# dsteinberg/libcluster

Hardware: AMD Instinct MI355X
Metric: E-step data-points/sec (full VBEM iteration: suff-stats + M-step + E-step) (higher is better)
Workload: dtype f64

## Files before the change

include/libcluster_hip.h:

```cpp
#ifndef LIBCLUSTER_HIP_H
#define LIBCLUSTER_HIP_H

#include <stdint.h>

#ifdef __cplusplus
extern "C" {
#endif

typedef enum { LC_OK = 0, LC_EINVAL = 1, LC_ERUNTIME = 2, LC_EHIP = 3, LC_EDOMAIN = 4 } lc_status;

typedef enum { LC_W_DIRICHLET = 0, LC_W_STICKBREAK = 1, LC_W_GDIRICHLET = 2 } lc_weight_kind;
typedef enum {
  LC_ALGO_VDP = 0,
  LC_ALGO_BGMM = 1,
  LC_ALGO_GMC = 2,
  LC_ALGO_SGMC = 3,
  LC_ALGO_DGMM = 4,
  LC_ALGO_BEMM = 5,
  LC_ALGO_DGMC = 6,
  LC_ALGO_EGMC = 7
} lc_algo;
typedef enum { LC_C_GAUSSWISH = 0, LC_C_NORMGAMMA = 1, LC_C_EXPGAMMA = 2 } lc_ckind;

typedef struct lc_ctx lc_ctx;
// ... 11 lines not shown
double lc_const_zerocutoff(void);
int lc_const_splititer(void);

int lc_ctx_create(int device, void* stream, lc_ctx** out);
int lc_ctx_destroy(lc_ctx* ctx);
int lc_ctx_set_stream(lc_ctx* ctx, void* stream);
int lc_ctx_synchronize(lc_ctx* ctx);
int lc_ctx_dims(lc_ctx* ctx, int* J, int* D, int64_t* Ntotal, int* K);

int lc_ctx_set_data(lc_ctx* ctx, int J, const double* const* Xj, const int64_t* Nj, int D, int64_t row_stride,
                    int64_t col_stride);
int lc_ctx_synth(lc_ctx* ctx, int64_t N, int D, int K, const double* mu, const double* L, uint64_t seed,
                 int64_t row_offset, double hard);
int lc_ctx_synth_groups(lc_ctx* ctx, int J, const int64_t* Nj, int D, int K, const double* mu, const double* L,
                        const double* cdf, uint64_t seed, const int64_t* group_ids, double hard);
int lc_ctx_get_rows(lc_ctx* ctx, int j, int64_t row0, int64_t n, double* out);

int lc_ctx_set_qz(lc_ctx* ctx, int j, const double* q, int K, int64_t row_stride, int64_t col_stride);
int lc_ctx_get_qz(lc_ctx* ctx, int j, double* q, int64_t row_stride, int64_t col_stride);
int lc_ctx_get_qz_rows(lc_ctx* ctx, int j, int64_t row0, int64_t n, double* q, int64_t row_stride, int64_t col_stride);
int lc_ctx_get_qz_all(lc_ctx* ctx, double* q);
int lc_ctx_get_qz_all_colmajor(lc_ctx* ctx, double* const* q);
int lc_ctx_fill_qz(lc_ctx* ctx, int K, double value);

int lc_estep_posterior(lc_ctx* ctx, int K, const double* nu, const double* beta, const double* m, const double* iW,
                       const double* logdW, const double* Elogpi, const unsigned char* active, double* Fz,
                       double* LLk);
int lc_estep(lc_ctx* ctx, int K, const double* A, const double* m, const double* c, double* Fz, double* LLk);
int lc_eloglike(lc_ctx* ctx, int K, const double* nu, const double* beta, const double* m, const double* iW,
                const double* logdW);
int lc_mahaldist(lc_ctx* ctx, const double* mu, const double* A, double* dist);
int lc_suffstat(lc_ctx* ctx, const unsigned char* smask, double* Nk, double* xs, double* xxs, double* Njk);
int lc_suffstat_diag(lc_ctx* ctx, const unsigned char* smask, double* Nk, double* xs, double* xxs, double* Njk);
int lc_estep_diag(lc_ctx* ctx, int K, const double* a, const double* w2, const double* w1, const double* c, int raw,
                  double* Fz, double* LLk);
int lc_colsums(lc_ctx* ctx, double* Njk);

typedef int (*lc_allreduce_fn)(void* user, void* device_buf, int64_t count, void* stream);
int lc_ctx_set_allreduce(lc_ctx* ctx, lc_allreduce_fn fn, void* user);
#define LC_COMM_ID_BYTES 128
int lc_comm_rccl_available(void);
int lc_comm_unique_id(void* id );
int lc_ctx_comm_init_rccl(lc_ctx* ctx, const void* id, int rank, int world);
int lc_ctx_comm_init_host(lc_ctx* ctx, const char* name, int rank, int world);
int lc_ctx_comm_free(lc_ctx* ctx);
int lc_ctx_comm_info(lc_ctx* ctx, int* rank, int* world, const char** kind);
int lc_ctx_allreduce(lc_ctx* ctx, double* values, int n);
int lc_ctx_set_sharding(lc_ctx* ctx, int whole_groups);
int lc_ctx_set_skip_zero(lc_ctx* ctx, int on);

int lc_ctx_set_speck_skip(lc_ctx* ctx, int on);
int lc_ctx_speck_passes(lc_ctx* ctx, int64_t* skipping, int64_t* dense);
int lc_ctx_speck_list_passes(lc_ctx* ctx, int64_t* lists);

int lc_trim_cache(void);

int lc_ctx_timing_enable(lc_ctx* ctx, int on);
int lc_ctx_timing_reset(lc_ctx* ctx);
int lc_ctx_timing_get(lc_ctx* ctx, double* estep_ms, int64_t* estep_calls, double* suffstat_ms,
                      int64_t* suffstat_calls);
int lc_ctx_timing_get_fused(lc_ctx* ctx, double* fused_ms, int64_t* fused_calls);
#define LC_TIMING_FIELDS 14
int lc_ctx_timing_get_all(lc_ctx* ctx, double* out, int n);

int lc_vbem(lc_ctx* ctx, lc_model** model, int wkind, int ckind, double wprior, double clusterprior, int maxit,
            int sparse, int fixed_iters, int verbose, unsigned nthreads, double* F, int* niter, double* Ftrace,
            int ntrace);

int lc_prune(lc_ctx* ctx, lc_model* model, int verbose, int* removed);

int lc_learn(int algo, int J, const double* const* Xj, const int64_t* Nj, int D, int64_t row_stride,
             int64_t col_stride, double wprior, double clusterprior, int maxclusters, int sparse, int verbose,
             unsigned nthreads, int device, lc_model** out, double* F);

int lc_learn_w(int algo, int J, const double* const* Xj, const int64_t* Nj, int D, int64_t row_stride,
               int64_t col_stride, double wprior, const double* wprior_j, double clusterprior, int maxclusters,
               int sparse, int verbose, unsigned nthreads, int device, lc_model** out, double* F);

int lc_cluster(lc_ctx* ctx, int wkind, int ckind, double wprior, double clusterprior, int maxclusters, int sparse,
               int verbose, unsigned nthreads, lc_model** out, double* F);

int lc_model_free(lc_model* m);
int lc_model_dims(lc_model* m, int* J, int* K, int* D);
int lc_model_rounds(lc_model* m, int* nrounds);
int lc_model_round(lc_model* m, int r, int* K, int* niter, double* F, int nF);
int lc_model_get_qz(lc_model* m, int j, double* q, int64_t row_stride, int64_t col_stride);
int lc_model_get_qz_all(lc_model* m, double* q);
int lc_model_get_qz_all_colmajor(lc_model* m, double* const* q);
int lc_model_weights(lc_model* m, int j, double* Elogweight, double* Nk);
int lc_model_kinds(lc_model* m, int* wkind, int* ckind);
int lc_model_cluster(lc_model* m, int k, double* N, double* mean, double* cov, double* nu, double* beta, double* iW,
                     double* logdW);
int lc_model_fenergy(lc_model* m, double* Fw , double* Fc );

int lc_model_predict(lc_model* m, lc_ctx* ctx, const int* groups , int keep_qz);
int lc_ctx_get_predictions(lc_ctx* ctx, int j, int64_t row0, int64_t n, int32_t* label, double* logZ, double* logp);
int lc_model_predict_conditional(lc_model* m, lc_ctx* ctx, const int* groups , const int* given,
                                 int ngiven, const int* target , int ntarget);
int lc_ctx_get_conditional(lc_ctx* ctx, int j, int64_t row0, int64_t n, double* mean, int64_t row_stride, double* logp);
int lc_model_predict_conditional_var(lc_model* m, lc_ctx* ctx, const int* groups , const int* given,
                                     int ngiven, const int* target , int ntarget);
int lc_ctx_get_conditional_var(lc_ctx* ctx, int j, int64_t row0, int64_t n, double* var, int64_t row_stride);
#define LC_DRAWS_MAX 64
int lc_model_predict_conditional_draws(lc_model* m, lc_ctx* ctx, const int* groups , const int* given,
                                       int ngiven, const int* target , int ntarget, int ndraws, uint64_t seed);
int lc_ctx_get_conditional_draws(lc_ctx* ctx, int j, int64_t row0, int64_t n, double* draws, int32_t* label);
// ... 68 lines not shown
```

libcluster_amd/capi.py:

```python
from __future__ import annotations

import ctypes as C
import re
from pathlib import Path
from typing import NamedTuple, Optional

import numpy as np

PKG = Path(__file__).resolve().parent
LIB_PATH = PKG / "lib" / "libcluster_hip.so"
if __import__("os").environ.get("LC_LIB_PATH"):
    LIB_PATH = Path(__import__("os").environ["LC_LIB_PATH"])
HEADER = PKG.parent / "include" / "libcluster_hip.h"

LC_OK, LC_EINVAL, LC_ERUNTIME, LC_EHIP, LC_EDOMAIN = range(5)
W_DIRICHLET, W_STICKBREAK, W_GDIRICHLET = 0, 1, 2
ALGO_VDP, ALGO_BGMM, ALGO_GMC, ALGO_SGMC, ALGO_DGMM, ALGO_BEMM, ALGO_DGMC, ALGO_EGMC = range(8)
C_GAUSSWISH, C_NORMGAMMA, C_EXPGAMMA = 0, 1, 2
RANK_QZ, RANK_LOGZ, RANK_LOGP = 0, 1, 2

c_double_p = C.POINTER(C.c_double)
c_int64_p = C.POINTER(C.c_int64)
c_int_p = C.POINTER(C.c_int)
c_ubyte_p = C.POINTER(C.c_ubyte)
# ... 152 lines not shown

    tmp = Path(tempfile.mkdtemp(prefix="lc_fresh_")) / LIB_PATH.name
    shutil.copy2(LIB_PATH, tmp)
    L2 = C.CDLL(str(tmp))
    L2.lc_source_hash.restype = C.c_char_p
    if L2.lc_source_hash().decode() != want:
        raise ImportError(f"{LIB_PATH} is stale and the rebuild did not pick up the current sources")
    import sys

    print(f"libcluster_amd: rebuilt a stale {LIB_PATH.name} (was {have}, now {want})", file=sys.stderr)
    return L2


def lib() -> C.CDLL:
    global _lib
    if _lib is not None:
        return _lib
    if not LIB_PATH.exists():
        raise ImportError(
            f"{LIB_PATH} is missing: build it with `python -m libcluster_amd.build` "
            "(hipcc, --offload-arch=gfx950).  There is no Python/CPU fallback for the E-step."
        )
    try:
        import torch
    except ImportError:
        pass
    L = _load_checked()
    L.lc_last_error.restype = C.c_char_p
    L.lc_comm_unique_id.argtypes = [C.c_void_p]
    L.lc_ctx_comm_init_rccl.argtypes = [C.c_void_p, C.c_void_p, C.c_int, C.c_int]
    L.lc_ctx_comm_init_host.argtypes = [C.c_void_p, C.c_char_p, C.c_int, C.c_int]
    L.lc_ctx_comm_free.argtypes = [C.c_void_p]
    L.lc_ctx_comm_info.argtypes = [C.c_void_p, c_int_p, c_int_p, C.POINTER(C.c_char_p)]
    L.lc_ctx_allreduce.argtypes = [C.c_void_p, c_double_p, C.c_int]
    for f in ("lc_const_converge", "lc_const_fengydel", "lc_const_zerocutoff"):
        getattr(L, f).restype = C.c_double
    L.lc_digamma.restype = C.c_double
    L.lc_digamma.argtypes = [C.c_double]
    L.lc_ctx_create.argtypes = [C.c_int, C.c_void_p, C.POINTER(C.c_void_p)]
    L.lc_ctx_destroy.argtypes = [C.c_void_p]
    L.lc_ctx_set_stream.argtypes = [C.c_void_p, C.c_void_p]
    L.lc_ctx_synchronize.argtypes = [C.c_void_p]
    L.lc_ctx_dims.argtypes = [C.c_void_p, c_int_p, c_int_p, c_int64_p, c_int_p]
    L.lc_ctx_set_data.argtypes = [C.c_void_p, C.c_int, C.POINTER(c_double_p), c_int64_p, C.c_int, C.c_int64, C.c_int64]
    L.lc_ctx_synth.argtypes = [C.c_void_p, C.c_int64, C.c_int, C.c_int, c_double_p, c_double_p, C.c_uint64,
                               C.c_int64, C.c_double]
    L.lc_ctx_synth_groups.argtypes = [C.c_void_p, C.c_int, c_int64_p, C.c_int, C.c_int, c_double_p, c_double_p,
                                      c_double_p, C.c_uint64, c_int64_p, C.c_double]
    L.lc_ctx_set_sharding.argtypes = [C.c_void_p, C.c_int]
    L.lc_ctx_set_skip_zero.argtypes = [C.c_void_p, C.c_int]
    L.lc_ctx_set_speck_skip.argtypes = [C.c_void_p, C.c_int]
    L.lc_ctx_speck_passes.argtypes = [C.c_void_p, c_int64_p, c_int64_p]
    L.lc_ctx_speck_list_passes.argtypes = [C.c_void_p, c_int64_p]
    L.lc_ctx_get_rows.argtypes = [C.c_void_p, C.c_int, C.c_int64, C.c_int64, c_double_p]
    L.lc_ctx_set_qz.argtypes = [C.c_void_p, C.c_int, c_double_p, C.c_int, C.c_int64, C.c_int64]
    L.lc_ctx_get_qz.argtypes = [C.c_void_p, C.c_int, c_double_p, C.c_int64, C.c_int64]
    L.lc_ctx_get_qz_rows.argtypes = [C.c_void_p, C.c_int, C.c_int64, C.c_int64, c_double_p, C.c_int64, C.c_int64]
    L.lc_ctx_fill_qz.argtypes = [C.c_void_p, C.c_int, C.c_double]
    L.lc_estep.argtypes = [C.c_void_p, C.c_int, c_double_p, c_double_p, c_double_p, c_double_p, c_double_p]
    L.lc_estep_posterior.argtypes = [C.c_void_p, C.c_int, c_double_p, c_double_p, c_double_p, c_double_p, c_double_p,
                                     c_double_p, c_ubyte_p, c_double_p, c_double_p]
    L.lc_eloglike.argtypes = [C.c_void_p, C.c_int, c_double_p, c_double_p, c_double_p, c_double_p, c_double_p]
    L.lc_mahaldist.argtypes = [C.c_void_p, c_double_p, c_double_p, c_double_p]
    L.lc_suffstat.argtypes = [C.c_void_p, c_ubyte_p, c_double_p, c_double_p, c_double_p, c_double_p]
    L.lc_suffstat_diag.argtypes = [C.c_void_p, c_ubyte_p, c_double_p, c_double_p, c_double_p, c_double_p]
    L.lc_estep_diag.argtypes = [C.c_void_p, C.c_int, c_double_p, c_double_p, c_double_p, c_double_p, C.c_int,
                                c_double_p, c_double_p]
    L.lc_colsums.argtypes = [C.c_void_p, c_double_p]
    L.lc_ctx_set_allreduce.argtypes = [C.c_void_p, ALLREDUCE_FN, C.c_void_p]
    L.lc_ctx_timing_enable.argtypes = [C.c_void_p, C.c_int]
    L.lc_ctx_timing_reset.argtypes = [C.c_void_p]
    L.lc_ctx_timing_get.argtypes = [C.c_void_p, c_double_p, c_int64_p, c_double_p, c_int64_p]
    L.lc_vbem.argtypes = [C.c_void_p, C.POINTER(C.c_void_p), C.c_int, C.c_int, C.c_double, C.c_double, C.c_int,
                          C.c_int, C.c_int, C.c_int, C.c_uint, c_double_p, c_int_p, c_double_p, C.c_int]
    L.lc_learn.argtypes = [C.c_int, C.c_int, C.POINTER(c_double_p), c_int64_p, C.c_int, C.c_int64, C.c_int64,
                           C.c_double, C.c_double, C.c_int, C.c_int, C.c_int, C.c_uint, C.c_int,
                           C.POINTER(C.c_void_p), c_double_p]
    L.lc_learn_w.argtypes = [C.c_int, C.c_int, C.POINTER(c_double_p), c_int64_p, C.c_int, C.c_int64, C.c_int64,
                             C.c_double, c_double_p, C.c_double, C.c_int, C.c_int, C.c_int, C.c_uint, C.c_int,
                             C.POINTER(C.c_void_p), c_double_p]
    L.lc_cluster.argtypes = [C.c_void_p, C.c_int, C.c_int, C.c_double, C.c_double, C.c_int, C.c_int, C.c_int,
                             C.c_uint, C.POINTER(C.c_void_p), c_double_p]
    L.lc_prune.argtypes = [C.c_void_p, C.c_void_p, C.c_int, c_int_p]
    L.lc_model_free.argtypes = [C.c_void_p]
    L.lc_model_dims.argtypes = [C.c_void_p, c_int_p, c_int_p, c_int_p]
    L.lc_model_rounds.argtypes = [C.c_void_p, c_int_p]
    L.lc_model_round.argtypes = [C.c_void_p, C.c_int, c_int_p, c_int_p, c_double_p, C.c_int]
    L.lc_model_get_qz.argtypes = [C.c_void_p, C.c_int, c_double_p, C.c_int64, C.c_int64]
    L.lc_model_weights.argtypes = [C.c_void_p, C.c_int, c_double_p, c_double_p]
    L.lc_model_cluster.argtypes = [C.c_void_p, C.c_int, c_double_p, c_double_p, c_double_p, c_double_p, c_double_p,
                                   c_double_p, c_double_p]
    L.lc_model_kinds.argtypes = [C.c_void_p, c_int_p, c_int_p]
    L.lc_model_fenergy.argtypes = [C.c_void_p, c_double_p, c_double_p]
    L.lc_weights_update.argtypes = [C.c_int, C.c_double, c_double_p, C.c_int, c_double_p, c_double_p]
    L.lc_gw_mstep.argtypes = [C.c_double, C.c_int, C.c_double, c_double_p, c_double_p, c_double_p, c_double_p,
                              c_double_p, c_double_p, c_double_p, c_double_p, c_double_p, c_double_p]
    L.lc_learn_topic.argtypes = [C.c_int, c_int_p, C.POINTER(c_double_p), c_int64_p, C.c_int, C.c_int64, C.c_int64,
                                 C.POINTER(c_double_p), C.c_int, C.POINTER(c_double_p), C.c_double, C.c_double,
                                 C.c_uint, C.c_int, C.c_int, C.c_uint, C.c_int, C.POINTER(C.c_void_p), c_double_p]
    L.lc_learn_topic_dist.argtypes = [C.c_int, c_int_p, C.POINTER(c_double_p), c_int64_p, C.c_int, C.c_int64, C.c_int64,
                                      C.POINTER(c_double_p), C.c_int, C.POINTER(c_double_p), C.c_double, C.c_double,
                                      C.c_uint, C.c_int, C.c_int, C.c_uint, C.c_int, C.c_void_p, ALLREDUCE_FN,
                                      C.c_void_p, C.POINTER(C.c_void_p), c_double_p]
    L.lc_tmodel_free.argtypes = [C.c_void_p]
    L.lc_tmodel_dims.argtypes = [C.c_void_p, c_int_p, c_int_p, c_int_p, c_int_p, c_int_p, c_int_p]
    L.lc_tmodel_get_qy.argtypes = [C.c_void_p, C.c_int, c_double_p]
# ... 117 lines not shown
        Xs = [X] if isinstance(X, np.ndarray) else list(X)
        Xs = [np.asarray(x, dtype=np.float64) for x in Xs]
        D = Xs[0].shape[1]
        for x in Xs:
            if x.ndim != 2 or x.shape[1] != D:
                raise ValueError("X dimensions are inconsistent between groups!")
        st = {_strides(x) for x in Xs}
        if len(st) == 1 and all(x.shape[0] > 1 for x in Xs) and min(next(iter(st))) > 0:
            rs, cs = next(iter(st))
        else:
            Xs = [np.ascontiguousarray(x) for x in Xs]
            rs, cs = D, 1
        J = len(Xs)
        ptrs = (c_double_p * J)(*[dptr(x) for x in Xs])
        Nj = (C.c_int64 * J)(*[x.shape[0] for x in Xs])
        check(lib().lc_ctx_set_data(self._h, J, ptrs, Nj, D, rs, cs))
        self._X = Xs

    def synth(self, N, D, K, mu, L, seed, row_offset=0, hard=0.9):
        mu = np.ascontiguousarray(mu, dtype=np.float64)
        L = np.ascontiguousarray(L, dtype=np.float64)
        assert mu.shape == (K, D) and L.shape == (K, D, D)
        check(lib().lc_ctx_synth(self._h, N, D, K, dptr(mu), dptr(L), seed, row_offset, hard))

    def synth_groups(self, Nj, D, K, mu, L, seed, mix=None, group_ids=None, hard=0.9):
        Nj = np.ascontiguousarray(Nj, dtype=np.int64)
        J = Nj.size
        mu = np.ascontiguousarray(mu, dtype=np.float64)
        L = np.ascontiguousarray(L, dtype=np.float64)
        cdf = None
        if mix is not None:
            cdf = np.ascontiguousarray(np.cumsum(np.asarray(mix, dtype=np.float64), axis=1))
            assert cdf.shape == (J, K)
        gid = None if group_ids is None else np.ascontiguousarray(group_ids, dtype=np.int64)
        check(lib().lc_ctx_synth_groups(self._h, J, Nj.ctypes.data_as(c_int64_p), D, K, dptr(mu), dptr(L), dptr(cdf),
                                        seed, None if gid is None else gid.ctypes.data_as(c_int64_p), hard))

    def set_skip_zero(self, on: bool = True):
        check(lib().lc_ctx_set_skip_zero(self._h, int(on)))

    def set_speck_skip(self, on: bool = True):
        check(lib().lc_ctx_set_speck_skip(self._h, int(on)))

    def speck_passes(self):
        a, b = C.c_int64(), C.c_int64()
        check(lib().lc_ctx_speck_passes(self._h, C.byref(a), C.byref(b)))
        return a.value, b.value

    def speck_list_passes(self):
        a = C.c_int64()
        check(lib().lc_ctx_speck_list_passes(self._h, C.byref(a)))
        return a.value

    def set_sharding(self, whole_groups: bool):
        check(lib().lc_ctx_set_sharding(self._h, int(whole_groups)))

    def dims(self):
        J, D, K, N = C.c_int(), C.c_int(), C.c_int(), C.c_int64()
        check(lib().lc_ctx_dims(self._h, C.byref(J), C.byref(D), C.byref(N), C.byref(K)))
        return J.value, D.value, N.value, K.value

    def get_rows(self, j, row0, n):
        _, D, _, _ = self.dims()
        out = np.empty((n, D))
        check(lib().lc_ctx_get_rows(self._h, j, row0, n, dptr(out)))
        return out

    def set_qz(self, qZ):
        qs = [qZ] if isinstance(qZ, np.ndarray) else list(qZ)
        K = qs[0].shape[1]
        for j, q in enumerate(qs):
            q = np.asarray(q, dtype=np.float64)
            if q.shape[1] != K:
                raise ValueError("qZ groups must have the same number of columns")
            if q.shape[0] == 0:
                q = np.zeros((1, K))[:0]
                check(lib().lc_ctx_set_qz(self._h, j, dptr(np.zeros(1)), K, K, 1))
                continue
            rs, cs = _strides(q)
            check(lib().lc_ctx_set_qz(self._h, j, dptr(q), K, rs, cs))

    def get_qz(self, rows_per_group):
        _, _, _, K = self.dims()
        rows = [int(n) for n in rows_per_group]
        allq = np.zeros((sum(rows), K))
        if allq.size:
            check(lib().lc_ctx_get_qz_all(self._h, dptr(allq)))
        return [allq[o - n:o] for n, o in zip(rows, np.cumsum(rows))]

    def get_qz_colmajor(self, rows_per_group):
        _, _, _, K = self.dims()
        out = [np.zeros((int(n), K), order="F") for n in rows_per_group]
        ptrs = (c_double_p * len(out))(*[dptr(a) if a.size else None for a in out])
        if sum(a.size for a in out):
            fn = lib().lc_ctx_get_qz_all_colmajor
            fn.argtypes = [C.c_void_p, C.POINTER(c_double_p)]
            check(fn(self._h, ptrs))
        return out

    def get_qz_rows(self, j, row0, n):
        _, _, _, K = self.dims()
        q = np.empty((n, K))
        if n:
            check(lib().lc_ctx_get_qz_rows(self._h, j, row0, n, dptr(q), K, 1))
        return q

# ... 818 lines not shown
```

libcluster_amd/csrc/lc_capi.cpp:

```cpp
#include <cmath>
#include <cstring>
#include <iostream>
#include <limits>
#include <memory>
#include <new>
#include <algorithm>
#include <string>
#include <sched.h>
#include <atomic>
#include <thread>

#include "../../include/libcluster_hip.h"
#include "lc_ctx.hpp"
#include <execinfo.h>
#include <signal.h>
#include <unistd.h>

#include <cstdlib>

#include "lc_engine.hpp"
#include "lc_topic.hpp"
#include "lc_host.hpp"
#include "lc_predict.hpp"

// ... 385 lines not shown
    need(L, "L");
    ctx->impl.synth(N, D, K, mu, L, seed, row_offset, hard);
  });
}

int lc_ctx_synth_groups(lc_ctx* ctx, int J, const int64_t* Nj, int D, int K, const double* mu, const double* L,
                        const double* cdf, uint64_t seed, const int64_t* group_ids, double hard) {
  return guarded([&] {
    need(ctx, "ctx");
    need(Nj, "Nj");
    need(mu, "mu");
    need(L, "L");
    ctx->impl.synth_groups(J, Nj, D, K, mu, L, cdf, seed, group_ids, 0, hard);
  });
}

int lc_ctx_set_sharding(lc_ctx* ctx, int whole_groups) {
  return guarded([&] {
    need(ctx, "ctx");
    ctx->impl.set_group_sharded(whole_groups != 0);
  });
}

int lc_ctx_set_skip_zero(lc_ctx* ctx, int on) {
  return guarded([&] {
    need(ctx, "ctx");
    ctx->impl.set_skip_zero(on != 0);
  });
}

int lc_ctx_set_speck_skip(lc_ctx* ctx, int on) {
  return guarded([&] {
    need(ctx, "ctx");
    ctx->impl.set_speck_skip(on != 0);
  });
}

int lc_ctx_speck_passes(lc_ctx* ctx, int64_t* skipping, int64_t* dense) {
  return guarded([&] {
    need(ctx, "ctx");
    if (skipping) *skipping = ctx->impl.speck_passes_skipping();
    if (dense) *dense = ctx->impl.speck_passes_dense();
  });
}

int lc_ctx_speck_list_passes(lc_ctx* ctx, int64_t* lists) {
  return guarded([&] {
    need(ctx, "ctx");
    need(lists, "lists");
    *lists = ctx->impl.speck_passes_lists();
  });
}

int lc_ctx_get_rows(lc_ctx* ctx, int j, int64_t row0, int64_t n, double* out) {
  return guarded([&] {
    need(ctx, "ctx");
    need(out, "out");
    ctx->impl.get_rows(j, row0, n, out);
  });
}

int lc_ctx_set_qz(lc_ctx* ctx, int j, const double* q, int K, int64_t rs, int64_t cs) {
  return guarded([&] {
    need(ctx, "ctx");
    need(q, "q");
    ctx->impl.qz_set(j, q, K, rs, cs);
  });
}

int lc_ctx_get_qz(lc_ctx* ctx, int j, double* q, int64_t rs, int64_t cs) {
  return guarded([&] {
    need(ctx, "ctx");
    need(q, "q");
    ctx->impl.qz_get(j, q, rs, cs);
  });
}

int lc_ctx_get_qz_rows(lc_ctx* ctx, int j, int64_t row0, int64_t n, double* q, int64_t rs, int64_t cs) {
  return guarded([&] {
    need(ctx, "ctx");
    need(q, "q");
    ctx->impl.qz_get_rows(j, row0, n, q, rs, cs);
  });
}

int lc_ctx_fill_qz(lc_ctx* ctx, int K, double value) {
  return guarded([&] {
    need(ctx, "ctx");
    ctx->impl.qz_fill(K, value);
    ctx->impl.synchronize();
  });
}

int lc_estep(lc_ctx* ctx, int K, const double* A, const double* m, const double* c, double* Fz, double* LLk) {
  return guarded([&] {
    need(ctx, "ctx");
    need(A, "A");
    need(m, "m");
    need(c, "c");
    ctx->impl.estep(K, A, m, c, Fz, LLk);
  });
}

int lc_estep_posterior(lc_ctx* ctx, int K, const double* nu, const double* beta, const double* m, const double* iW,
                       const double* logdW, const double* Elogpi, const unsigned char* active, double* Fz,
                       double* LLk) {
// ... 1163 lines not shown
```

libcluster_amd/csrc/lc_ctx.cpp:

```cpp
#include "lc_ctx.hpp"
#include "lc_engine.hpp"

#include <algorithm>
#include <atomic>
#include <chrono>
#include <cmath>
#include <iostream>
#include <cstring>
#include <limits>
#include <mutex>
#include <thread>

namespace lcc {

namespace {
struct BlockCache {
  struct Block {
    void* p;
    size_t bytes;
    int device;
    size_t owner;
  };
  std::mutex m;
  std::vector<Block> dev, pinned;
// ... 111 lines not shown
  if (!q) {
    hipError_t e = hipMalloc(&q, n * sizeof(T));
    if (e != hipSuccess) {
      trim_cache();
      e = hipMalloc(&q, n * sizeof(T));
    }
    if (e != hipSuccess)
      throw AllocFailure(std::string("HIP error: hipMalloc of ") + std::to_string(n * sizeof(T)) +
                       " bytes failed: " + hipGetErrorString(e));
    got = n * sizeof(T);
  }
  p = static_cast<T*>(q);
  cap = got / sizeof(T);
  device = dev;
}

PinnedBuf::~PinnedBuf() {
  if (!p) return;
  BlockCache& c = BlockCache::get();
  std::lock_guard<std::mutex> g(c.m);
  if (c.pinned.size() < 256) c.pinned.push_back({p, cap * sizeof(double), 0, BlockCache::thread_tag()});
  else (void)hipHostFree(p);
}

void PinnedBuf::resize(size_t count) {
  if (count > cap) {
    BlockCache& c = BlockCache::get();
    if (p) {
      std::lock_guard<std::mutex> g(c.m);
      c.pinned.push_back({p, cap * sizeof(double), 0, BlockCache::thread_tag()});
    }
    p = nullptr;
    cap = 0;
    const size_t want = count < 1024 ? 1024 : count + count / 2;
    size_t got = 0;
    void* q = c.take(c.pinned, want * sizeof(double), 0, &got);
    if (!q) {
      hipError_t e = hipHostMalloc(&q, want * sizeof(double), hipHostMallocDefault);
      if (e != hipSuccess)
        throw HipFailure(std::string("HIP error: hipHostMalloc of ") + std::to_string(want * sizeof(double)) +
                         " bytes failed: " + hipGetErrorString(e));
      got = want * sizeof(double);
    }
    p = static_cast<double*>(q);
    cap = got / sizeof(double);
  }
  n = count;
}

template struct DevBuf<double>;
template struct DevBuf<int>;
template struct DevBuf<int64_t>;
template struct DevBuf<unsigned char>;

Context::Context(int device, hipStream_t stream) : device_(device), stream_(stream) {
  static int n = 0;
  static hipError_t e = hipGetDeviceCount(&n);
  if (e != hipSuccess || n <= 0)
    throw HipFailure("libcluster_amd: no HIP device available (the E-step has no CPU fallback): " +
                     std::string(e != hipSuccess ? hipGetErrorString(e) : "device count is 0"));
  if (device < 0 || device >= n) throw std::invalid_argument("device index out of range");
  LC_HIP(hipSetDevice(device_));
}

void Context::use_device() const { LC_HIP(hipSetDevice(device_)); }

Context::~Context() {
  (void)hipSetDevice(device_);
  if (X_.p || qz_[0].buf.p || qz_[1].buf.p) (void)hipStreamSynchronize(stream_);
  for (auto& p : pending_) {
    (void)hipEventDestroy(p.a);
    (void)hipEventDestroy(p.b);
  }
  for (hipEvent_t e : evpool_) (void)hipEventDestroy(e);
}

void Context::synchronize() const {
  use_device();
  LC_HIP(hipStreamSynchronize(stream_));
}

void Context::require_gw_width() const {
  if (DP_ > lck::GW_MAX_DP)
    throw std::invalid_argument("D > 1024 is not supported by the Gauss-Wishart kernels (the diagonal and exponential "
                                "families take any D)");
}

void Context::build_layout(int J, const int64_t* Nj, int D) {
  if (J < 1) throw std::invalid_argument("need at least one group of observations");
  if (D < 1) throw std::invalid_argument("observations must have at least one dimension");
  const int DP = lck::padded_dim_wide(D);
  dcache_release();
  J_ = J;
  D_ = D;
  DP_ = DP;
  DC_ = lck::estep_active_width(D, DP);
  if (lck::test_switch("LC_FULL_WIDTH")) DC_ = DP;
  sspart_clean_ = false;
  Nj_.assign(Nj, Nj + J);
  goff_.assign(J + 1, 0);
  Ntot_ = 0;
  for (int j = 0; j < J; ++j) {
    if (Nj[j] < 0) throw std::invalid_argument("negative group size");
    goff_[j + 1] = goff_[j] + (Nj[j] + lck::RG - 1) / lck::RG * lck::RG;
    Ntot_ += Nj[j];
  }
// ... 113 lines not shown
  if (group_ids) {
    dgid.reserve((size_t)J);
    LC_HIP(hipMemcpyAsync(dgid.p, group_ids, (size_t)J * sizeof(int64_t), hipMemcpyHostToDevice, stream_));
  }
  dmu.reserve((size_t)K * D);
  dL.reserve((size_t)K * D * D);
  LC_HIP(hipMemcpyAsync(dmu.p, mu, (size_t)K * D * sizeof(double), hipMemcpyHostToDevice, stream_));
  LC_HIP(hipMemcpyAsync(dL.p, L, (size_t)K * D * D * sizeof(double), hipMemcpyHostToDevice, stream_));
  if (cdf) {
    dcdf.reserve((size_t)J * K);
    LC_HIP(hipMemcpyAsync(dcdf.p, cdf, (size_t)J * K * sizeof(double), hipMemcpyHostToDevice, stream_));
  }
  ensure_qz(qz_[cur_], K, false);
  qz_[cur_].K = K;
  lck::SynthLaunch a;
  a.DP = DP_;
  a.D = D;
  a.K = K;
  a.X = X_.p;
  a.qZ = qz_[cur_].buf.p;
  a.ldq = NP_;
  a.nrows = Nj[0];
  a.NP = NP_;
  a.row_offset = row_offset;
  a.seed = seed;
  a.mu = dmu.p;
  a.L = dL.p;
  a.hard = hard;
  a.rginfo = J > 1 ? rginfo_.p : nullptr;
  a.goff = J > 1 ? goff_d_.p : nullptr;
  a.cdf = cdf ? dcdf.p : nullptr;
  a.gids = group_ids ? dgid.p : nullptr;
  a.group_base = 0;
  LC_HIP(lck::launch_synth(a, stream_));
  LC_HIP(hipStreamSynchronize(stream_));
}

void Context::get_rows(int j, int64_t row0, int64_t n, double* out) const {
  use_device();
  if (j < 0 || j >= J_ || row0 < 0 || n < 0 || row0 + n > Nj_[j]) throw std::invalid_argument("row range out of bounds");
  if (n == 0) return;
  std::vector<double> tmp((size_t)n * DP_);
  LC_HIP(hipMemcpyAsync(tmp.data(), X_.p + (size_t)(goff_[j] + row0) * DP_, tmp.size() * sizeof(double),
                        hipMemcpyDeviceToHost, stream_));
  LC_HIP(hipStreamSynchronize(stream_));
  for (int64_t r = 0; r < n; ++r) std::memcpy(out + r * D_, tmp.data() + (size_t)r * DP_, D_ * sizeof(double));
}

#ifdef LC_TEST_HOOKS
static bool test_keep_stale() {
  static const bool on = std::getenv("LC_TEST_QHASH_KEEP_STALE") != nullptr;
  return on;
}
#endif
void Context::ensure_qz(QZ& q, int K, bool preserve) {
  use_device();
  q.hash_ok = false;
#ifdef LC_TEST_HOOKS
  if (test_keep_stale() && q.hash.p) q.hash_ok = true;
#endif
  if (K <= q.cap && q.buf.p) return;
  int newcap = std::max(K, q.cap > 0 ? q.cap + std::max(4, q.cap / 2) : K);
  DevBuf<double> nb;
  nb.reserve((size_t)std::max<int64_t>(NP_, 1) * newcap);
  LC_HIP(hipMemsetAsync(nb.p, 0, (size_t)std::max<int64_t>(NP_, 1) * newcap * sizeof(double), stream_));
  if (preserve && q.buf.p && q.K > 0)
    LC_HIP(hipMemcpyAsync(nb.p, q.buf.p, (size_t)NP_ * q.K * sizeof(double), hipMemcpyDeviceToDevice, stream_));
  LC_HIP(hipStreamSynchronize(stream_));
  std::swap(q.buf.p, nb.p);
  std::swap(q.buf.cap, nb.cap);
  std::swap(q.buf.device, nb.device);
  q.cap = newcap;
}

void Context::qz_fill(int K, double value) {
  use_device();
  if (K < 1) throw std::invalid_argument("K must be >= 1");
  ensure_qz(qz_[cur_], K, false);
  qz_[cur_].K = K;
  LC_HIP(lck::launch_fill_qz(qz_[cur_].buf.p, NP_, K, rginfo_.p, Nj_[0], NP_ / lck::RG, value, stream_));
}

void Context::qz_set(int j, const double* q, int K, int64_t rs, int64_t cs) {
  use_device();
  if (j < 0 || j >= J_) throw std::invalid_argument("group index out of range");
  if (K < 1) throw std::invalid_argument("K must be >= 1");
  qz_[cur_].hash_ok = false;
  if (K != qz_[cur_].K) {
    ensure_qz(qz_[cur_], K, false);
    LC_HIP(hipMemsetAsync(qz_[cur_].buf.p, 0, (size_t)NP_ * K * sizeof(double), stream_));
    qz_[cur_].K = K;
  }
  const int64_t n = Nj_[j];
  if (n == 0) return;
  std::vector<double> col((size_t)n);
  for (int k = 0; k < K; ++k) {
    for (int64_t r = 0; r < n; ++r) col[(size_t)r] = q[r * rs + k * cs];
    LC_HIP(hipMemcpyAsync(qz_[cur_].buf.p + (size_t)k * NP_ + goff_[j], col.data(), n * sizeof(double),
                          hipMemcpyHostToDevice, stream_));
    LC_HIP(hipStreamSynchronize(stream_));
  }
}

void Context::qz_get_column(int j, int k, double* out) const {
  use_device();
  if (j < 0 || j >= J_ || k < 0 || k >= qz_[cur_].K) throw std::invalid_argument("qZ column out of range");
  if (Nj_[j] == 0) return;
  LC_HIP(hipMemcpyAsync(out, qz_[cur_].buf.p + (size_t)k * NP_ + goff_[j], Nj_[j] * sizeof(double),
                        hipMemcpyDeviceToHost, stream_));
  LC_HIP(hipStreamSynchronize(stream_));
}

void Context::qz_get_rows(int j, int64_t row0, int64_t n, double* q, int64_t rs, int64_t cs) const {
  use_device();
  if (j < 0 || j >= J_ || row0 < 0 || n < 0 || row0 + n > Nj_[j]) throw std::invalid_argument("row range out of bounds");
  if (n == 0) return;
  std::vector<double> col((size_t)n);
  for (int k = 0; k < qz_[cur_].K; ++k) {
    LC_HIP(hipMemcpyAsync(col.data(), qz_[cur_].buf.p + (size_t)k * NP_ + goff_[j] + row0, n * sizeof(double),
                          hipMemcpyDeviceToHost, stream_));
    LC_HIP(hipStreamSynchronize(stream_));
    for (int64_t r = 0; r < n; ++r) q[r * rs + k * cs] = col[(size_t)r];
  }
}

void Context::qz_get(int j, double* q, int64_t rs, int64_t cs) const {
  if (j < 0 || j >= J_) throw std::invalid_argument("group index out of range");
  const int64_t n = Nj_[j];
  std::vector<double> col((size_t)n);
  for (int k = 0; k < qz_[cur_].K; ++k) {
    qz_get_column(j, k, col.data());
    for (int64_t r = 0; r < n; ++r) q[r * rs + k * cs] = col[(size_t)r];
  }
}

void Context::qz_get_all(double* out) const {
  const int K = qz_[cur_].K;
  if (K < 1 || NP_ == 0) return;
  LC_HIP(hipSetDevice(device_));
  {
// ... 60 lines not shown
      int64_t f = f0 + (int64_t)b * blk;
      const int64_t fe = std::min(f + blk, f0 + n);
      while (f < fe) {
        const int64_t k = f / NP_, p = f - k * NP_;
        const int64_t pe = std::min<int64_t>(NP_, p + (fe - f));
        int jj = (int)(std::upper_bound(goff_.begin(), goff_.end(), p) - goff_.begin()) - 1;
        if (jj < 0) jj = 0;
        for (; jj < J_ && goff_[(size_t)jj] < pe; ++jj) {
          const int64_t g0 = goff_[(size_t)jj], nj = Nj_[(size_t)jj];
          const int64_t lo = std::max(p, g0), hi = std::min(pe, g0 + nj);
          if (lo < hi)
            std::memcpy(out[jj] + (size_t)k * (ld ? ld[jj] : nj) + (lo - g0), base + (f - f0) + (lo - p),
                        (size_t)(hi - lo) * sizeof(double));
        }
        f += pe - p;
      }
    });
  };
  int64_t prev0 = -1, prevn = 0;
  int which = 0;
  for (int64_t f0 = 0; f0 < total; f0 += chunk, which ^= 1) {
    const int64_t n = std::min(chunk, total - f0);
    PinnedBuf& st = stage[which];
    if (st.size() == 0) st.resize((size_t)std::min(chunk, total));
    if (!done[which]) LC_HIP(hipEventCreateWithFlags(&done[which], hipEventDisableTiming));
    LC_HIP(hipMemcpyAsync(st.data(), qz_[cur_].buf.p + f0, (size_t)n * sizeof(double), hipMemcpyDeviceToHost, stream_));
    LC_HIP(hipEventRecord(done[which], stream_));
    if (prev0 >= 0) {
      LC_HIP(hipEventSynchronize(done[which ^ 1]));
      unpack(stage[which ^ 1].data(), prev0, prevn);
    }
    prev0 = f0;
    prevn = n;
  }
  which ^= 1;
  LC_HIP(hipEventSynchronize(done[which]));
  unpack(stage[which].data(), prev0, prevn);
  for (auto& e : done)
    if (e) (void)hipEventDestroy(e);
}

void Context::qz_keep_columns(const std::vector<int>& keep) {
  use_device();
  QZ& q = qz_[cur_];
  for (size_t i = 0; i < keep.size(); ++i) {
    const int src = keep[i];
    if (src < (int)i || src >= q.K) throw std::invalid_argument("bad column list");
    if (src != (int)i)
      LC_HIP(hipMemcpyAsync(q.buf.p + i * (size_t)NP_, q.buf.p + (size_t)src * NP_, NP_ * sizeof(double),
                            hipMemcpyDeviceToDevice, stream_));
  }
  q.K = (int)keep.size();
  q.hash_ok = false;
#ifdef LC_TEST_HOOKS
  if (test_keep_stale() && q.hash.p) q.hash_ok = true;
#endif
}

void Context::qz_clone_to_alt() {
  use_device();
  QZ& a = qz_[cur_ ^ 1];
  const int Ksave = qz_[cur_].K;
  static const bool full_only = lck::test_switch("LC_SPLIT_FULL_CLONE") != nullptr;
  if (!full_only && NP_ > 0 && Ksave >= 1 && qz_[cur_].hash_ok && a.hash_ok && a.buf.p && a.hash.p && qz_[cur_].hash.p &&
      a.cap >= Ksave + 1 && (a.K == Ksave || a.K == Ksave + 1)) {
    LC_HIP(lck::launch_qz_resync(a.buf.p, qz_[cur_].buf.p, NP_, Ksave, Ksave + 1, NP_, a.hash.p, qz_[cur_].hash.p, stream_));
    a.K = Ksave;
    clone_resyncs_ += 1;
    return;
  }
  clone_fulls_ += 1;
  static const bool trace = std::getenv("LC_TRACE_PHASES") != nullptr;
  if (trace) std::cerr << "[clone] full copy at K " << Ksave << " (row-wise so far: " << clone_resyncs_ << ")" << std::endl;
  ensure_qz(a, Ksave + 1, false);
  a.K = Ksave;
  LC_HIP(hipMemcpyAsync(a.buf.p, qz_[cur_].buf.p, (size_t)NP_ * Ksave * sizeof(double), hipMemcpyDeviceToDevice,
                        stream_));
  LC_HIP(hipMemsetAsync(a.buf.p + (size_t)NP_ * Ksave, 0, (size_t)NP_ * sizeof(double), stream_));
  if (qz_[cur_].hash_ok && NP_ > 0) {
    a.hash.reserve((size_t)NP_);
    LC_HIP(hipMemcpyAsync(a.hash.p, qz_[cur_].hash.p, (size_t)NP_ * sizeof(int64_t), hipMemcpyDeviceToDevice, stream_));
    a.hash_ok = true;
  }
}

void Context::qz_swap_alt() { cur_ ^= 1; }

void Context::select_rows(int k, double thresh, RowSelection& sel) {
  const QZ& q = qz_[cur_];
  if (k < 0 || k >= q.K) throw std::invalid_argument("qZ column out of range");
  select_rows_col(q.buf.p + (size_t)k * NP_, thresh, sel);
}

void Context::select_rows_col(const double* col, double thresh, RowSelection& sel) {
  LC_HIP(hipSetDevice(device_));
  sel.M = 0;
  sel.starts.assign((size_t)J_ + 1, 0);
  sel.starts_d.reserve((size_t)J_ + 1);
  if (NP_ == 0) {
    LC_HIP(hipMemsetAsync(sel.starts_d.p, 0, (size_t)(J_ + 1) * sizeof(int64_t), stream_));
    return;
  }
  const int nb = lck::select_blocks(NP_);
  selcnt_.reserve((size_t)nb);
  seloff_.reserve((size_t)nb);
  LC_HIP(lck::launch_select_count(col, NP_, thresh, selcnt_.p, stream_));
  std::vector<int> cnt((size_t)nb);
  LC_HIP(hipMemcpyAsync(cnt.data(), selcnt_.p, (size_t)nb * sizeof(int), hipMemcpyDeviceToHost, stream_));
  LC_HIP(hipStreamSynchronize(stream_));
  std::vector<int64_t> off((size_t)nb);
  int64_t tot = 0;
  for (int b = 0; b < nb; ++b) {
    off[(size_t)b] = tot;
    tot += cnt[(size_t)b];
  }
  sel.M = tot;
  sel.idx.reserve((size_t)std::max<int64_t>(tot, 1));
  LC_HIP(hipMemcpyAsync(seloff_.p, off.data(), (size_t)nb * sizeof(int64_t), hipMemcpyHostToDevice, stream_));
// ... 36 lines not shown
  use_device();
  ensure_qz(qz_[cur_], 2, false);
  qz_[cur_].K = 2;
  if (NP_ == 0) return;
  std::vector<double> mv((size_t)2 * DP_, 0.0);
  std::copy(m, m + D_, mv.begin());
  std::copy(v, v + D_, mv.begin() + DP_);
  mv_.reserve(mv.size());
  LC_HIP(hipMemcpyAsync(mv_.p, mv.data(), mv.size() * sizeof(double), hipMemcpyHostToDevice, stream_));
  LC_HIP(lck::launch_split_init(X_.p, DP_, D_, NP_, J_ > 1 ? rginfo_.p : nullptr, Nj_[0], mv_.p, qz_[cur_].buf.p, NP_,
                                0, nullptr, stream_));
  LC_HIP(hipStreamSynchronize(stream_));
}

void Context::qz_init_split_mean(const double* v) {
  use_device();
  ensure_qz(qz_[cur_], 2, false);
  qz_[cur_].K = 2;
  const bool global_mean = distributed() && !group_sharded_;
  std::vector<double> mv((size_t)2 * DP_, 0.0);
  std::copy(v, v + D_, mv.begin() + DP_);
  std::vector<double> sc((size_t)J_ * 2, 0.0);
  const int* rgi = J_ > 1 ? rginfo_.p : nullptr;
  if (NP_ > 0) {
    mv_.reserve(mv.size() + (size_t)J_);
    LC_HIP(hipMemcpyAsync(mv_.p, mv.data(), mv.size() * sizeof(double), hipMemcpyHostToDevice, stream_));
    LC_HIP(lck::launch_split_init(X_.p, DP_, D_, NP_, rgi, Nj_[0], mv_.p, qz_[cur_].buf.p, NP_, 1, nullptr, stream_));
    std::vector<double> sums((size_t)J_ * 2);
    red_.reserve((size_t)J_ * 2);
    LC_HIP(lck::launch_group_colsum(qz_[cur_].buf.p, NP_, 2, goff_d_.p, J_, red_.p, stream_));
    LC_HIP(hipMemcpyAsync(sums.data(), red_.p, sums.size() * sizeof(double), hipMemcpyDeviceToHost, stream_));
    LC_HIP(hipStreamSynchronize(stream_));
    for (int j = 0; j < J_; ++j) sc[(size_t)j] = sums[(size_t)j * 2];
  }
  for (int j = 0; j < J_; ++j) sc[(size_t)J_ + j] = (double)Nj_[j];
  if (global_mean) allreduce_values(sc.data(), 2 * J_);
  if (NP_ == 0) return;
  std::vector<double> thr((size_t)J_);
  for (int j = 0; j < J_; ++j) thr[(size_t)j] = sc[(size_t)J_ + j] > 0 ? sc[(size_t)j] / sc[(size_t)J_ + j] : 0.0;
  double* thr_d = mv_.p + mv.size();
  LC_HIP(hipMemcpyAsync(thr_d, thr.data(), thr.size() * sizeof(double), hipMemcpyHostToDevice, stream_));
  LC_HIP(lck::launch_split_init(X_.p, DP_, D_, NP_, rgi, Nj_[0], mv_.p, qz_[cur_].buf.p, NP_, 2, thr_d, stream_));
  LC_HIP(hipStreamSynchronize(stream_));
}

void Context::qz_split_from(const Context& sub, const RowSelection& sel, int k) {
  use_device();
  QZ& q = qz_[cur_];
  if (k < 0 || k >= q.K) throw std::invalid_argument("split column out of range");
  if (sub.qz_[sub.cur_].K < 2) throw std::invalid_argument("sub-problem has no second column");
  const bool hashed = q.hash_ok;
  if (q.K + 1 > q.cap) ensure_qz(q, q.K + 1, true);
  q.hash_ok = hashed;
  bool mark = hashed;
#ifdef LC_TEST_HOOKS
  if (test_keep_stale()) mark = false;
#endif
  LC_HIP(hipMemsetAsync(q.buf.p + (size_t)NP_ * q.K, 0, (size_t)NP_ * sizeof(double), stream_));
  LC_HIP(lck::launch_aug_from_sub(q.buf.p, NP_, k, q.K, sel.idx.p, sel.M, sel.starts_d.p, sub.goff_d_.p, J_,
                                  sub.qz_[sub.cur_].buf.p + (size_t)sub.NP_, stream_, mark ? q.hash.p : nullptr));
  q.K += 1;
}

template <class F>
void Context::timed(Timed kind, F&& launch) {
  if (!timing_) return launch();
  EvPair ev{timing_event(), timing_event(), kind};
  LC_HIP(hipEventRecord(ev.a, stream_));
  launch();
  LC_HIP(hipEventRecord(ev.b, stream_));
  pending_.push_back(ev);
}

void Context::allreduce(double* dbuf, int64_t count) {
  if (!comm_ && !ar_fn_) return;
  timed(Timed::Allreduce, [&] {
    if (comm_) {
      comm_->allreduce_sum(dbuf, count, stream_);
    } else {
      const int rc = ar_fn_(ar_user_, dbuf, count, (void*)stream_);
      if (rc != 0) throw std::runtime_error("all-reduce hook failed with status " + std::to_string(rc));
    }
  });
}

void Context::enqueue_sums(int64_t grid, int K, bool want_ll) {
  const size_t n = (size_t)1 + K;
  const bool direct = !distributed() && grid > 0;
  hred_.resize(n);
  if (!direct) red_.reserve(n);
  double* dst = direct ? hred_.data() : red_.p;
  if (grid > 0) {
    redtmp_.reserve((size_t)lck::REDUCE_TMP_ELEMS * 64);
    LC_HIP(lck::launch_reduce_partials(fzpart_.p, (int)grid, 1, dst, stream_, redtmp_.p));
    if (want_ll) LC_HIP(lck::launch_reduce_partials(llpart_.p, (int)grid, K, dst + 1, stream_, redtmp_.p));
    else if (!direct) LC_HIP(hipMemsetAsync(red_.p + 1, 0, (size_t)K * sizeof(double), stream_));
  } else {
    LC_HIP(hipMemsetAsync(red_.p, 0, n * sizeof(double), stream_));
  }
  if (!direct) {
    allreduce(red_.p, (int64_t)n);
    LC_HIP(hipMemcpyAsync(hred_.data(), red_.p, n * sizeof(double), hipMemcpyDeviceToHost, stream_));
  }
}

void Context::read_sums(int K, double* Fz, double* LLk) const {
// ... 80 lines not shown
                }
            }
          std::copy(bneg.begin() + 64 * I, bneg.begin() + 64 * (I + 1), C + 4096);
        }
    }
  }
  std::memcpy(hpack_.data() + (size_t)K * PS, c, (size_t)J_ * K * sizeof(double));
}

lck::EstepLaunch Context::gw_estep_launch(int K, const double* A, const double* m, const double* c, const double* X,
                                          int64_t rows, int64_t nrows, double* out, bool raw, bool want_ll) {
  pack_estep_params(K, A, m, c);
  params_.reserve(hpack_.size());
  LC_HIP(hipMemcpyAsync(params_.p, hpack_.data(), hpack_.size() * sizeof(double), hipMemcpyHostToDevice, stream_));
  lck::EstepLaunch a;
  a.DP = DP_;
  a.DC = DC_;
  a.X = X;
  a.nrg = rows / lck::RG;
  a.rginfo = J_ > 1 ? rginfo_.p : nullptr;
  a.nrows = nrows;
  a.params = params_.p;
  a.ctab = params_.p + (size_t)K * lck::estep_pstride(DP_, DC_);
  a.K = K;
  a.qZ = out;
  a.ldq = rows;
  a.raw = raw ? 1 : 0;
  for (size_t t = 0; t < (size_t)J_ * K && !a.sparse; ++t)
    if (c[t] == -std::numeric_limits<double>::infinity()) a.sparse = 1;
  const int64_t grid = lck::estep_grid(a);
  fzpart_.reserve((size_t)std::max<int64_t>(grid, 1));
  if (want_ll) llpart_.reserve((size_t)std::max<int64_t>(grid, 1) * K);
  a.fz_part = fzpart_.p;
  a.ll_part = want_ll ? llpart_.p : nullptr;
  return a;
}

void Context::estep(int K, const double* A, const double* m, const double* c, double* Fz, double* LLk, bool raw,
                    double* target) {
  if (K < 1) throw std::invalid_argument("K must be >= 1");
  if (target && !raw) throw std::invalid_argument("a target buffer needs raw mode");
  require_gw_width();
  if (NP_ == 0 && !distributed()) {
    if (Fz) *Fz = -0.0;
    if (LLk) std::fill(LLk, LLk + K, 0.0);
    if (!target) qz_[cur_].K = K;
    return;
  }
  LC_HIP(hipSetDevice(device_));
  if (!target) {
    ensure_qz(qz_[cur_], K, false);
    qz_[cur_].K = K;
  }
  const lck::EstepLaunch a =
      gw_estep_launch(K, A, m, c, X_.p, NP_, Nj_[0], target ? target : qz_[cur_].buf.p, raw, LLk != nullptr);
  timed(Timed::Estep, [&] { LC_HIP(lck::launch_estep(a, stream_)); });
  if (raw) {
    LC_HIP(hipStreamSynchronize(stream_));
    return;
  }
  enqueue_sums(lck::estep_grid(a), K, LLk != nullptr);
  run_overlap();
  LC_HIP(hipStreamSynchronize(stream_));
  read_sums(K, Fz, LLk);
}

bool Context::estep_suffstat_fused(int K, const double* A, const double* m, const double* c, double* Fz, double* LLk,
                                   double* Nk, double* xs, double* xxs, double* Njk) {
  if (K < 1) throw std::invalid_argument("K must be >= 1");
  const int D = D_, DP = DP_;
  const int64_t nrg = NP_ / lck::RG;
  if (!lck::fused_eligible(DP, K)) return false;
  const int grid = NP_ > 0 ? lck::fused_plan(DP, nrg, K) : 0;
  LC_HIP(hipSetDevice(device_));
  const int64_t PS = lck::pstride(DP), SS = lck::stat_stride(DP);
  pack_estep_params(K, A, m, c);
  params_.reserve(hpack_.size());
  LC_HIP(hipMemcpyAsync(params_.p, hpack_.data(), hpack_.size() * sizeof(double), hipMemcpyHostToDevice, stream_));
  ensure_qz(qz_[cur_], K, false);
  qz_[cur_].K = K;
  const int64_t W = lck::fused_record(DP, K);
  sspart_reserve((size_t)std::max(grid, 1) * W);
  sspart_clean_ = false;
  const bool counts = own_counts(false);
  const size_t nrec = (size_t)W, nout = nrec + (counts ? (size_t)J_ * K : 0);
  const size_t ofz = (size_t)K * SS, oll = ofz + 1;
  ssout_.reserve(nout);
  double* njk_d = ssout_.p + nrec;
  lck::FusedLaunch a;
  a.DP = DP;
  a.D = D;
  a.X = X_.p;
  a.nrg = nrg;
  a.rginfo = J_ > 1 ? rginfo_.p : nullptr;
  a.nrows = Nj_[0];
  a.params = params_.p;
  a.ctab = params_.p + (size_t)K * PS;
  a.K = K;
  a.qZ = qz_[cur_].buf.p;
  a.ldq = NP_;
  a.partial = sspart_.p;
  a.want_ll = LLk != nullptr;
  a.grid = grid;
  a.ngroups = J_;
  timed(Timed::Fused, [&] {
    if (grid > 0) LC_HIP(lck::launch_fused(a, stream_));
  });
  hss_.resize(nout);
  const bool direct = !distributed() && grid > 0;
  double* dst = direct ? hss_.data() : ssout_.p;
  if (grid > 0) {
    LC_HIP(lck::launch_reduce_partials(sspart_.p, grid, W, dst, stream_));
    if (counts) {
      redtmp_.reserve((size_t)lck::REDUCE_TMP_ELEMS * 64);
      LC_HIP(lck::launch_group_colsum(qz_[cur_].buf.p, NP_, K, goff_d_.p, J_, direct ? dst + nrec : njk_d, stream_,
                                      redtmp_.p, NP_));
// ... 28 lines not shown
    units += (double)(goff_[(size_t)j2 + 1] - goff_[(size_t)j2]) *
                      (double)((kofs[(size_t)j2 + 1] - kofs[(size_t)j2] + cpb - 1) / cpb);
  int64_t rows = (int64_t)(units / 2048.0);
  rows = std::max<int64_t>(256, (rows + 31) / 32 * 32);
  std::vector<lck::SSItem> items;
  std::vector<std::vector<int>> recs((size_t)K);
  for (int j2 = 0; j2 < J_; ++j2) {
    const int na = kofs[(size_t)j2 + 1] - kofs[(size_t)j2];
    if (na == 0) continue;
    for (int64_t b0 = goff_[(size_t)j2]; b0 < goff_[(size_t)j2 + 1]; b0 += rows) {
      const int64_t b1 = std::min<int64_t>(b0 + rows, goff_[(size_t)j2 + 1]);
      for (int s0 = 0; s0 < na; s0 += cpb) {
        lck::SSItem it;
        it.r0 = b0;
        it.r1 = b1;
        it.kofs = kofs[(size_t)j2] + s0;
        it.kcnt = std::min(cpb, na - s0);
        it.rec0 = nrec;
        for (int t = 0; t < it.kcnt; ++t) recs[(size_t)klist[(size_t)it.kofs + t]].push_back(nrec + t);
        nrec += it.kcnt;
        items.push_back(it);
      }
    }
  }
  std::vector<int> kptr((size_t)K + 1, 0), krec;
  krec.reserve((size_t)nrec);
  for (int k2 = 0; k2 < K; ++k2) {
    krec.insert(krec.end(), recs[(size_t)k2].begin(), recs[(size_t)k2].end());
    kptr[(size_t)k2 + 1] = (int)krec.size();
  }
  ssitems_.reserve(items.size() * sizeof(lck::SSItem));
  ssints_.reserve(klist.size() + kptr.size() + krec.size() + 1);
  int* klist_d = ssints_.p;
  int* kptr_d = klist_d + klist.size();
  int* krec_d = kptr_d + kptr.size();
  if (!items.empty()) {
    LC_HIP(hipMemcpyAsync(ssitems_.p, items.data(), items.size() * sizeof(lck::SSItem), hipMemcpyHostToDevice,
                          stream_));
    LC_HIP(hipMemcpyAsync(klist_d, klist.data(), klist.size() * sizeof(int), hipMemcpyHostToDevice, stream_));
    LC_HIP(hipMemcpyAsync(krec_d, krec.data(), krec.size() * sizeof(int), hipMemcpyHostToDevice, stream_));
  }
  LC_HIP(hipMemcpyAsync(kptr_d, kptr.data(), kptr.size() * sizeof(int), hipMemcpyHostToDevice, stream_));
  LC_HIP(hipStreamSynchronize(stream_));
  a.items = reinterpret_cast<const lck::SSItem*>(ssitems_.p);
  a.klist = klist_d;
  a.nitems = (int)items.size();
  a.smask = nullptr;
  a.rginfo = nullptr;
  sskptr_ = kptr_d;
  sskrec_ = krec_d;
  return nrec;
}

void Context::suffstat(const unsigned char* smask, double* Nk, double* xs, double* xxs, double* Njk) {
  const int K = qz_[cur_].K, D = D_, DP = DP_;
  if (K < 1) throw std::invalid_argument("qZ has not been set");
  require_gw_width();
  LC_HIP(hipSetDevice(device_));
  const int64_t SS = lck::stat_stride(DP);
  const size_t nout = (size_t)K * SS + (size_t)J_ * K;
  ssout_.reserve(nout);
  double* njk_d = ssout_.p + (size_t)K * SS;
  const bool counts = own_counts(smask != nullptr);
  const bool direct = !distributed() && !counts && NP_ > 0;
  hss_.resize(nout);
  if (NP_ > 0) {
    lck::SuffstatLaunch a;
    a.DP = DP;
    a.DC = DC_;
    a.X = X_.p;
    a.NP = NP_;
    a.qZ = qz_[cur_].buf.p;
    a.ldq = NP_;
    a.K = K;
    a.rginfo = nullptr;
    a.smask = nullptr;
    a.mode = skip_zero_ ? lck::SS_ZERO_SKIP : lck::SS_DENSE;
    if (smask && J_ > 1) {
      smask_.reserve((size_t)J_ * K);
      LC_HIP(hipMemcpyAsync(smask_.p, smask, (size_t)J_ * K, hipMemcpyHostToDevice, stream_));
      a.rginfo = rginfo_.p;
      a.smask = smask_.p;
      double off = 0.0, tot = 0.0;
      for (int j2 = 0; j2 < J_; ++j2)
        for (int k2 = 0; k2 < K; ++k2) {
          tot += (double)Nj_[j2];
          if (!smask[(size_t)j2 * K + k2]) off += (double)Nj_[j2];
        }
      if (off > 0.3 * tot) a.mode = lck::SS_WORK_LIST;
      else if (!skip_zero_) a.mode = lck::SS_MASKED_DENSE;
    }
    const lck::SuffstatPlan plan = lck::suffstat_plan(DP, DC_, NP_, K, a.mode);
    const bool listed = a.mode == lck::SS_WORK_LIST;
    const int nchunks = plan.nchunks, KR = plan.KR, extra = plan.extra;
    a.skip_listed = listed && skip_zero_;
    bool lists = false;
    if (speck_skip_ && plan.route == lck::SS_FEAT && NP_ >= lck::SPECK_PROBE_MIN_ROWS) {
      speck_active_.reserve(2);
      int64_t pairs = 0, rows = 0;
      int counts2[2] = {0, 0};
      LC_HIP(lck::launch_speck_probe(a.qZ, a.ldq, K, NP_, speck_active_.p, &pairs, stream_, &rows));
      LC_HIP(hipMemcpyAsync(counts2, speck_active_.p, 2 * sizeof(int), hipMemcpyDeviceToHost, stream_));
      LC_HIP(hipStreamSynchronize(stream_));
      const int active = counts2[0];
      const bool sort_pays = 2 * (int64_t)active <= pairs && DP < 128;
      a.speck_skip = !lck::speck_probe_says_skip(active, pairs) ? 0 : sort_pays ? lck::speck_skip_mode() : 1;
      (a.speck_skip ? speck_skipping_ : speck_dense_) += 1;
      lists = a.speck_skip != 0 && a.mode == lck::SS_DENSE && lck::speck_lists_enabled() && lck::suffstat_list_instance(DP, DC_) &&
              lck::speck_probe_says_lists(counts2[1], rows);
      if (lists) speck_lists_ += 1;
    }
    const int nrec = listed ? build_sparse_worklist(smask, K, plan, a) : nchunks * KR;
    sspart_reserve((size_t)std::max(nrec, 1) * SS);
    if (extra > 0) ssext_.reserve((size_t)KR * SS);
    a.KR = KR;
    if (DC_ < DP_ && !sspart_clean_) {
      LC_HIP(hipMemsetAsync(sspart_.p, 0, sspart_.cap * sizeof(double), stream_));
      sspart_clean_ = true;
    }
    a.partial = sspart_.p;
    a.nchunks = nchunks;
    a.chunk_rows = plan.chunk_rows;
    if (lists) {
      const size_t lbytes = lck::ss_list_layout(nchunks, plan.chunk_rows, K).bytes;
      sslists_.reserve(lbytes);
      a.speck_skip = 0;
      timed(Timed::Suffstat, [&] { LC_HIP(lck::launch_suffstat_lists(a, plan, sslists_.p, lbytes, stream_)); });
    } else
      timed(Timed::Suffstat, [&] { LC_HIP(lck::launch_suffstat(a, plan, stream_)); });
    if (listed)
      LC_HIP(lck::launch_reduce_records(sspart_.p, SS, K, sskptr_, sskrec_, ssout_.p, stream_));
    else if (extra > 0) {
      LC_HIP(lck::launch_reduce_partials(sspart_.p, nchunks, (int64_t)KR * SS, ssext_.p, stream_));
      LC_HIP(lck::launch_fold_extra(ssext_.p, SS, K, plan.klast0, extra, stream_));
      LC_HIP(hipMemcpyAsync(direct ? hss_.data() : ssout_.p, ssext_.p, (size_t)K * SS * sizeof(double),
                            direct ? hipMemcpyDeviceToHost : hipMemcpyDeviceToDevice, stream_));
    } else
      LC_HIP(lck::launch_reduce_partials(sspart_.p, nchunks, (int64_t)K * SS, direct ? hss_.data() : ssout_.p, stream_));
    if (counts) {
      redtmp_.reserve((size_t)lck::REDUCE_TMP_ELEMS * 64);
      LC_HIP(lck::launch_group_colsum(qz_[cur_].buf.p, NP_, K, goff_d_.p, J_, njk_d, stream_, redtmp_.p, NP_));
    }
    else if (!direct) LC_HIP(hipMemsetAsync(njk_d, 0, (size_t)K * sizeof(double), stream_));
    if (smask && J_ == 1)
      for (int k = 0; k < K; ++k)
        if (!smask[k]) LC_HIP(hipMemsetAsync(ssout_.p + (size_t)k * SS, 0, (size_t)SS * sizeof(double), stream_));
  } else {
    LC_HIP(hipMemsetAsync(ssout_.p, 0, nout * sizeof(double), stream_));
  }
  if (!direct) {
    allreduce(ssout_.p, group_sharded_ ? (int64_t)K * SS : (int64_t)nout);
    LC_HIP(hipMemcpyAsync(hss_.data(), ssout_.p, nout * sizeof(double), hipMemcpyDeviceToHost, stream_));
  }
  LC_HIP(hipStreamSynchronize(stream_));
  unpack_gw_records(hss_.data(), K, D, DP, Nk, xs, xxs);
  unpack_counts(hss_.data(), SS, K, counts ? hss_.data() + (size_t)K * SS : nullptr, J_, Njk);
}

bool Context::dcache_eligible(int K) const {
  static const bool off = lck::test_switch("LC_SPLIT_NO_DCACHE") != nullptr || lck::test_switch("LC_SPLIT_NO_DELTA") != nullptr;
  return !off && DP_ <= lck::GW_MAX_DP && K >= 1 && K <= lck::softmax_cached_max_k() && !lck::fused_eligible(DP_, K);
}

void Context::dcache_invalidate() {
  dc_K_ = 0;
  rm_valid_ = false;
  dc_ver_.clear();
  dc_slot_.clear();
  std::fill(dc_used_.begin(), dc_used_.end(), (unsigned char)0);
  dc_saved_.clear();
  dc_journal_ = false;
  dq_K_ = 0;
}

void Context::dcache_release() {
  dcache_invalidate();
  dc_cap_ = 0;
  dc_room_K_ = 0;
  dc_used_.clear();
  dc_slab_.release();
// ... 860 lines not shown
```

libcluster_amd/csrc/lc_ctx.hpp:

```cpp
#pragma once
#include <hip/hip_runtime.h>

#include <cstdint>
#include <functional>
#include <stdexcept>
#include <string>
#include <vector>

#include "lc_comm.hpp"
#include "lc_kernels.h"

namespace lck {
struct PredictCondLaunch;
}

namespace lcc {

struct HipFailure : std::runtime_error {
  explicit HipFailure(const std::string& s) : std::runtime_error(s) {}
};
#define LC_HIP(expr)                                                                                          \
  do {                                                                                                        \
    hipError_t e_ = (expr);                                                                                   \
    if (e_ != hipSuccess)                                                                                     \
// ... 56 lines not shown
};
void cache_release_thread();

struct KernelTimes {
  double estep_ms = 0, suffstat_ms = 0, fused_ms = 0;
  int64_t estep_calls = 0, suffstat_calls = 0, fused_calls = 0;
  int64_t estep_diag_mfma_calls = 0;
  double allreduce_ms = 0;
  int64_t allreduce_calls = 0;
  double host_stats_ms = 0, host_mstep_ms = 0, host_estep_ms = 0, host_fenergy_ms = 0;
  int64_t host_iters = 0;
};

class Context {
 public:
  Context(int device, hipStream_t stream);
  ~Context();
  Context(const Context&) = delete;
  Context& operator=(const Context&) = delete;

  void set_data(int J, const double* const* Xj, const int64_t* Nj, int D, int64_t row_stride, int64_t col_stride);
  void synth(int64_t N, int D, int K, const double* mu, const double* L, uint64_t seed, int64_t row_offset,
             double hard);
  void synth_groups(int J, const int64_t* Nj, int D, int K, const double* mu, const double* L, const double* cdf,
                    uint64_t seed, const int64_t* group_ids, int64_t row_offset, double hard);
  void get_rows(int j, int64_t row0, int64_t n, double* out) const;

  int J() const { return J_; }
  int D() const { return D_; }
  int DP() const { return DP_; }
  int K() const { return qz_[cur_].K; }
  int64_t N(int j) const { return Nj_[j]; }
  int64_t Ntotal() const { return Ntot_; }
  int64_t NP() const { return NP_; }
  int device() const { return device_; }
  hipStream_t stream() const { return stream_; }
  void set_stream(hipStream_t s) { stream_ = s; }
  void synchronize() const;
  void set_allreduce(allreduce_fn f, void* user) {
    ar_fn_ = f;
    ar_user_ = user;
  }
  void set_comm(std::shared_ptr<lcm::Comm> c) { comm_ = std::move(c); }
  const std::shared_ptr<lcm::Comm>& comm() const { return comm_; }
  bool distributed() const { return ar_fn_ != nullptr || comm_ != nullptr; }
  double allreduce_value(double v);
  void allreduce_values(double* v, int n);
  void set_group_sharded(bool on) { group_sharded_ = on; }
  void set_skip_zero(bool on) { skip_zero_ = on; }
  void set_speck_skip(bool on) { speck_skip_ = on; }
  int64_t speck_passes_skipping() const { return speck_skipping_; }
  int64_t speck_passes_dense() const { return speck_dense_; }
  int64_t speck_passes_lists() const { return speck_lists_; }
  bool group_sharded() const { return group_sharded_ && distributed(); }
  void inherit_comm(const Context& parent) {
    ar_fn_ = parent.ar_fn_;
    ar_user_ = parent.ar_user_;
    comm_ = parent.comm_;
    group_sharded_ = parent.group_sharded_;
    skip_zero_ = parent.skip_zero_;
    speck_skip_ = parent.speck_skip_;
  }

  void qz_fill(int K, double value);
  void qz_set(int j, const double* q, int K, int64_t row_stride, int64_t col_stride);
  void qz_get(int j, double* q, int64_t row_stride, int64_t col_stride) const;
  void qz_get_all(double* out) const;
  void qz_get_all_colmajor(double* const* out, const int64_t* ld = nullptr) const;
  void qz_get_rows(int j, int64_t row0, int64_t n, double* q, int64_t row_stride, int64_t col_stride) const;
  void qz_get_column(int j, int k, double* out) const;
  void qz_keep_columns(const std::vector<int>& keep);
  void qz_clone_to_alt();
  void qz_swap_alt();
  void select_rows(int k, double thresh, RowSelection& sel);
  void select_rows_col(const double* col, double thresh, RowSelection& sel);
  void set_data_gather(const Context& src, const RowSelection& sel);
  void qz_gather_column(const Context& src, const RowSelection& sel, int col);
  void qz_init_split(const double* m, const double* v);
  void qz_init_split_mean(const double* v);
  void qz_split_from(const Context& sub, const RowSelection& sel, int k);

  void estep(int K, const double* A, const double* m, const double* c, double* Fz, double* LLk, bool raw = false,
             double* target = nullptr);
  bool dcache_eligible(int K) const;
  int estep_cache(int K, const double* A, const double* m, const double* c, double* Fz, double* LLk, double delta_tol,
                  int* stale = nullptr);
  void dcache_journal_begin();
  void dcache_rollback();
  void dcache_journal_end();
  void dcache_invalidate();
  void dcache_release();
  bool delta_suffstat(int K1, double max_frac, double* dNk, double* dxs, double* dxxs, double* dNjk);
  int delta_pending() const { return dq_K_; }
  int64_t delta_rows() const { return delta_rows_; }
  bool estep_suffstat_fused(int K, const double* A, const double* m, const double* c, double* Fz, double* LLk,
                            double* Nk, double* xs, double* xxs, double* Njk);
  void suffstat(const unsigned char* smask, double* Nk, double* xs, double* xxs, double* Njk);
  void colsums(double* Njk);
  void estep_diag(int K, const double* a, const double* w2, const double* w1, const double* c, double* Fz,
                  double* LLk, bool raw = false);
  void suffstat_diag(const unsigned char* smask, double* Nk, double* xs, double* xxs, double* Njk);

  void predict_rows(int K, int Kp, const double* c, const double* pc, const double* ps, const double* pe, bool keep_q);
  bool predict_diag(int mode, int Kp, const double* a, const double* w, const double* pc, const double* pe);
  void get_predictions(int j, int64_t row0, int64_t n, int32_t* label, double* logZ, double* logp) const;
  void predict_clear() {
    pred_vb_ = pred_logp_ = false;
    pred_docs_T_ = 0;
    pred_cond_ = 0;
    pred_cond_var_ = false;
    pred_holes_ = false;
    pred_holes_var_ = false;
    pred_holes_draws_ = 0;
    pred_cond_draws_ = 0;
// ... 6 lines not shown
  void get_conditional_var(int j, int64_t row0, int64_t n, double* var, int64_t row_stride) const;
  void predict_cond_draws(int Kp, int Db, int ndraws, uint64_t seed, const double* L, const double* cq);
  void get_conditional_draws(int j, int64_t row0, int64_t n, double* draws, int32_t* label) const;
  int conditional_draws() const { return pred_cond_draws_; }
  void sample(int mode, int J, const int64_t* Nj, int D, int Kp, const double* cdf, const int* klast, const double* loc,
              const double* fac, const double* shape, uint64_t seed, int64_t row_offset);
  void get_sample_labels(int j, int64_t row0, int64_t n, int32_t* label) const;
  void holes_scan(int64_t* holed_rows, int* max_count, int* bad_block, int64_t* bad_row, int* bad_count);
  void holes_fill(const double* fill);
  void predict_holes(int Kp, const double* tt, const double* ps, const double* pe, const double* mean, const double* P,
                     const double* gnu = nullptr, const double* cqnu = nullptr, int ndraws = 0, uint64_t seed = 0);
  void get_completed(int j, int64_t row0, int64_t n, double* rows, int64_t row_stride, double* logp, int32_t* count,
                     int32_t* cols) const;
  void get_completed_var(int j, int64_t row0, int64_t n, double* var, int64_t row_stride) const;
  void get_completed_draws(int j, int64_t row0, int64_t n, double* draws, int32_t* label) const;
  int completed_draws() const { return pred_holes_ ? pred_holes_draws_ : 0; }
  void top_rows(int what, int ncols, int m, bool largest, bool by_label, int32_t* count, int32_t* group, int64_t* row,
                double* score);
  void topic_infer(int K, int T, const double* a, const double* E, int max_sweeps, double tol, bool keep_q);
  void get_doc_predictions(int doc0, int n, double* qY, int32_t* label_t, double* Fyz, double* Fz, int32_t* sweeps) const;

  void set_overlap(std::function<void()> f) { overlap_ = std::move(f); }
  bool overlap_pending() const { return (bool)overlap_; }
  void run_overlap() {
    if (!overlap_) return;
    std::function<void()> f = std::move(overlap_);
    overlap_ = nullptr;
    f();
  }

  void timing_enable(bool on) {
    timing_ = on;
    if (on) timing_prepare(1024);
  }
  bool timing_enabled() const { return timing_; }
  void timing_host_phases(double stats_ms, double mstep_ms, double estep_ms, double fenergy_ms) {
    times_.host_stats_ms += stats_ms;
    times_.host_mstep_ms += mstep_ms;
    times_.host_estep_ms += estep_ms;
    times_.host_fenergy_ms += fenergy_ms;
    times_.host_iters += 1;
  }
  KernelTimes timing_get();
  void timing_prepare(int events);
  void timing_reset();

 private:
  struct QZ {
    DevBuf<double> buf;
    int cap = 0;
    int K = 0;
    DevBuf<int64_t> hash;
    bool hash_ok = false;
  };
  void ensure_qz(QZ& q, int K, bool preserve);
  void build_layout(int J, const int64_t* Nj, int D);
  void allreduce(double* dbuf, int64_t count);
  void pack_estep_params(int K, const double* A, const double* m, const double* c);
  lck::EstepLaunch gw_estep_launch(int K, const double* A, const double* m, const double* c, const double* X, int64_t rows,
                                   int64_t nrows, double* out, bool raw, bool want_ll);
  enum class Timed { Estep, Suffstat, Fused, Allreduce };
  template <class F>
  void timed(Timed kind, F&& launch);
  void enqueue_sums(int64_t grid, int K, bool want_ll);
  void read_sums(int K, double* Fz, double* LLk) const;
  bool own_counts(bool masked) const { return J_ > 1 || group_sharded() || masked; }
  void use_device() const;
  void require_gw_width() const;
  int build_sparse_worklist(const unsigned char* smask, int K, const lck::SuffstatPlan& plan, lck::SuffstatLaunch& a);

  int device_;
  hipStream_t stream_;
  allreduce_fn ar_fn_ = nullptr;
  void* ar_user_ = nullptr;
  std::shared_ptr<lcm::Comm> comm_;
  bool group_sharded_ = false;
  bool skip_zero_ = false;
  bool speck_skip_ = true;
  int64_t speck_skipping_ = 0, speck_dense_ = 0, speck_lists_ = 0;
  DevBuf<int> speck_active_;
  DevBuf<unsigned char> sslists_;

  int J_ = 0, D_ = 0, DP_ = 0;
  int DC_ = 0;
  std::vector<int64_t> Nj_, goff_;
  int64_t Ntot_ = 0, NP_ = 0;
  DevBuf<double> X_;
  DevBuf<int> rginfo_;
  DevBuf<int64_t> goff_d_;
  DevBuf<unsigned char> ssitems_;
  DevBuf<int> ssints_;
  const int* sskptr_ = nullptr;
  const int* sskrec_ = nullptr;
  QZ qz_[2];
  DevBuf<double> dc_slab_, dfresh_;
  int dc_cap_ = 0, dc_K_ = 0;
  int dc_room_K_ = 0;
  std::vector<int> dc_slot_;
  std::vector<unsigned char> dc_used_;
  std::vector<std::vector<double>> dc_tagA_, dc_tagm_;
  struct SavedColumn {
    int col = -1;
    int slot = -1;
    uint64_t ver = 0;
    std::vector<double> A, m;
  };
  std::vector<uint64_t> dc_ver_;
  uint64_t dc_vernext_ = 0;
  DevBuf<double> rm_max_, bs_need_, bs_x_, bs_out_;
  DevBuf<int> rm_arg_;
  bool rm_valid_ = false;
  int rm_K_ = 0;
  std::vector<uint64_t> rm_ver_;
  std::vector<double> rm_c_;
  int64_t clone_resyncs_ = 0, clone_fulls_ = 0;
  int64_t bound_rows_ = 0, bound_passes_ = 0;
  bool bound_static_ok() const;
  bool recompute_bounded(int K, const std::vector<int>& changed, const std::vector<int>& oldslot,
                         const std::vector<std::vector<double>>& oldA, const std::vector<std::vector<double>>& oldm,
                         const std::vector<int>& dest, const double* A, const double* m, const double* c, bool delta);
  int dc_find_run(int n) const;
  std::vector<std::unique_ptr<SavedColumn>> dc_saved_;
  bool dc_journal_ = false;
  int dc_jK0_ = 0;
  DevBuf<double> sink_;
  DevBuf<double> dq_, amax_;
  DevBuf<int64_t> dq_maskd_;
  DevBuf<int> dq_colsd_;
  uint64_t dq_mask_[2] = {0, 0};
  bool dq_mask_ok_ = false;
  double dq_tol_ = 0.0;
  int dq_K_ = 0;
  int64_t dq_ld_ = 0;
// ... 59 lines not shown
```

libcluster_amd/csrc/lc_device.hpp:

```cpp
#pragma once
#include <hip/hip_runtime.h>

#include <atomic>
#include <cmath>
#include <cstdlib>
#include <type_traits>
#include <utility>

#include "lc_kernels.h"

namespace lck {

inline int current_device_cus() {
  static std::atomic<int> cus_of[32];
  int dev = 0;
  if (hipGetDevice(&dev) != hipSuccess || dev < 0 || dev >= 32) dev = -1;
  int cus = dev >= 0 ? cus_of[dev].load(std::memory_order_relaxed) : 0;
  if (cus <= 0) {
    hipDeviceProp_t p;
    if (dev >= 0 && hipGetDeviceProperties(&p, dev) == hipSuccess) cus = p.multiProcessorCount;
    if (cus <= 0) cus = 256;
    if (dev >= 0) cus_of[dev].store(cus, std::memory_order_relaxed);
  }
  return cus;
}

__device__ __forceinline__ double mfma4(double a, double b, double c) {
  return __builtin_amdgcn_mfma_f64_4x4x4f64(a, b, c, 0, 0, 0);
}

__device__ __forceinline__ double max_raw(double a, double b) {
  asm("v_max_f64 %0, %0, %1" : "+v"(a) : "v"(b));
  return a;
}

static __constant__ double LC_EXP2_TAB[64] = {
    0x1.0000000000000p+0, 0x1.02c9a3e778061p+0, 0x1.059b0d3158574p+0, 0x1.0874518759bc8p+0,
    0x1.0b5586cf9890fp+0, 0x1.0e3ec32d3d1a2p+0, 0x1.11301d0125b51p+0, 0x1.1429aaea92de0p+0,
    0x1.172b83c7d517bp+0, 0x1.1a35beb6fcb75p+0, 0x1.1d4873168b9aap+0, 0x1.2063b88628cd6p+0,
    0x1.2387a6e756238p+0, 0x1.26b4565e27cddp+0, 0x1.29e9df51fdee1p+0, 0x1.2d285a6e4030bp+0,
    0x1.306fe0a31b715p+0, 0x1.33c08b26416ffp+0, 0x1.371a7373aa9cbp+0, 0x1.3a7db34e59ff7p+0,
    0x1.3dea64c123422p+0, 0x1.4160a21f72e2ap+0, 0x1.44e086061892dp+0, 0x1.486a2b5c13cd0p+0,
    0x1.4bfdad5362a27p+0, 0x1.4f9b2769d2ca7p+0, 0x1.5342b569d4f82p+0, 0x1.56f4736b527dap+0,
    0x1.5ab07dd485429p+0, 0x1.5e76f15ad2148p+0, 0x1.6247eb03a5585p+0, 0x1.6623882552225p+0,
    0x1.6a09e667f3bcdp+0, 0x1.6dfb23c651a2fp+0, 0x1.71f75e8ec5f74p+0, 0x1.75feb564267c9p+0,
    0x1.7a11473eb0187p+0, 0x1.7e2f336cf4e62p+0, 0x1.82589994cce13p+0, 0x1.868d99b4492edp+0,
    0x1.8ace5422aa0dbp+0, 0x1.8f1ae99157736p+0, 0x1.93737b0cdc5e5p+0, 0x1.97d829fde4e50p+0,
    0x1.9c49182a3f090p+0, 0x1.a0c667b5de565p+0, 0x1.a5503b23e255dp+0, 0x1.a9e6b5579fdbfp+0,
    0x1.ae89f995ad3adp+0, 0x1.b33a2b84f15fbp+0, 0x1.b7f76f2fb5e47p+0, 0x1.bcc1e904bc1d2p+0,
    0x1.c199bdd85529cp+0, 0x1.c67f12e57d14bp+0, 0x1.cb720dcef9069p+0, 0x1.d072d4a07897cp+0,
    0x1.d5818dcfba487p+0, 0x1.da9e603db3285p+0, 0x1.dfc97337b9b5fp+0, 0x1.e502ee78b3ff6p+0,
    0x1.ea4afa2a490dap+0, 0x1.efa1bee615a27p+0, 0x1.f50765b6e4540p+0, 0x1.fa7c1819e90d8p+0};
__device__ __forceinline__ void fill_exp_table(double* etab, int tid, int nthreads) {
  for (int i = tid; i < 64; i += nthreads) etab[i] = LC_EXP2_TAB[i];
}
__device__ __forceinline__ double exp_nonpos(double x, const double* etab) {
  x = fmax(x, -750.0);
  const double n = __builtin_rint(x * 0x1.71547652b82fep+6);
  double r = fma(n, -0x1.62e42fef00000p-7, x);
  r = fma(n, -0x1.473de6af278edp-40, r);
  double q = fma(r, 1.0 / 120.0, 1.0 / 24.0);
  q = fma(q, r, 1.0 / 6.0);
  q = fma(q, r, 0.5);
  const double p = fma(q, r * r, r);
  const int ni = (int)n;
  const double T = etab[ni & 63];
  return ldexp(fma(T, p, T), ni >> 6);
}
__device__ __forceinline__ double rcp_pos(double s) {
  double y = __builtin_amdgcn_rcp(s);
  double e = fma(-s, y, 1.0);
  y = fma(y, e, y);
  e = fma(-s, y, 1.0);
  return fma(y, e, y);
}

struct LogEntry {
  double t, hi, lo;
};
static __constant__ LogEntry LC_LOG_TAB[128] = {
    {0x1.0000000000000p+0, 0x0.0p+0, 0x0.0p+0},
    {0x1.fc07f01fc07f0p-1, 0x1.fe02a6b106799p-8, -0x1.e44b7e3711e7fp-67},
// ... 237 lines not shown
```

libcluster_amd/csrc/lc_kernels.h:

```cpp
#pragma once
#include <hip/hip_runtime.h>
#include <cstdint>

namespace lck {

constexpr int RG = 16;

inline int padded_dim(int D) {
  return D <= 16 ? 16 : D <= 32 ? 32 : D <= 48 ? 48 : D <= 64 ? 64 : D <= 80 ? 80 : D <= 96 ? 96 : D <= 112 ? 112 : D <= 128 ? 128 : -1;
}
__host__ __device__ constexpr int lds_row_stride(int DP) { return DP == 16 ? 16 : (DP + 16) % 32 != 16 ? DP + 32 : DP + 16; }
inline int padded_dim_wide(int D) { return D <= 128 ? padded_dim(D) : (D + 63) / 64 * 64; }
constexpr int GW_MAX_DP = 1024;
inline int ntiles(int DP) { int nt = DP / 4; return nt * (nt + 1) / 2; }
inline int pstride(int DP) { return ntiles(DP) * 16 + DP; }
constexpr int WIDE_CHUNK = 256 * 16 + 64;
inline int wide_chunks(int DP) { int np = DP / 64; return np * (np + 1) / 2; }
inline int64_t estep_pstride(int DP, int DC) { return DP > 128 ? (int64_t)wide_chunks(DP) * WIDE_CHUNK : (int64_t)pstride(DC); }
inline int64_t estep_pstride(int DP) { return estep_pstride(DP, DP); }
inline int estep_active_width(int D, int DP) {
  if (DP < 32 || DP > 128) return DP;
  const int g = DP <= 48 ? 4 : 8, lo = DP <= 48 ? DP - 12 : DP - 8;
  const int dc = (D + g - 1) / g * g;
  return dc < DP ? (dc < lo ? lo : dc) : DP;
}
inline int64_t stat_stride(int DP) { return 1 + (int64_t)DP + (int64_t)DP * DP; }

struct LdsGrant {
  size_t granted[16] = {};
};
inline hipError_t grant_dynamic_lds(const void* fn, size_t bytes, LdsGrant& g) {
  if (bytes <= 64 * 1024) return hipSuccess;
  int dev = -1;
  const bool tracked = hipGetDevice(&dev) == hipSuccess && dev >= 0 && dev < 16;
  if (tracked && bytes <= g.granted[dev]) return hipSuccess;
  const hipError_t e = hipFuncSetAttribute(fn, hipFuncAttributeMaxDynamicSharedMemorySize, (int)bytes);
  if (e == hipSuccess && tracked) g.granted[dev] = bytes;
  return e;
}

inline int rginfo_pack(int group, int nvalid) { return (group << 5) | nvalid; }

struct EstepLaunch {
  int DP;
  int DC = 0;
  const double* X;
  int64_t nrg;
  const int* rginfo;
  int64_t nrows;
  const double* params;
  const double* ctab;
  int K;
  double* qZ;
  int64_t ldq;
  double* fz_part;
  double* ll_part;
  int raw = 0;
  int sparse = 0;
  int lq_lds = 0;
};
struct EstepPlan {
  bool ok;
  int rows_per_block;
  int64_t grid;
  bool four_groups;
  int DC, lq_lds;
  size_t lds_bytes;
};
EstepPlan estep_plan(const EstepLaunch& a);
int64_t estep_grid(const EstepLaunch& a);
hipError_t launch_estep(const EstepLaunch& a, hipStream_t stream);

struct FusedLaunch {
  int DP;
  int D = 16;
  const double* X;
  int64_t nrg;
  const int* rginfo;
  int64_t nrows;
  const double* params;
  const double* ctab;
  int K;
  double* qZ;
  int64_t ldq;
  double* partial;
  bool want_ll;
  int grid;
  int ngroups = 1;
  int yshare = 0;
};
constexpr int FUSED_CT_CAP = 1024;
inline int64_t fused_record(int DP, int K) { return (int64_t)K * (1 + DP + (int64_t)DP * DP) + 1 + K; }
bool fused_eligible(int DP, int K);
int fused_plan(int DP, int64_t nrg, int K);
hipError_t launch_fused(const FusedLaunch& a, hipStream_t stream);

struct SSItem {
  int64_t r0, r1;
  int kofs, kcnt;
  int64_t rec0;
};
constexpr int SS_BR = 32;
constexpr double SPECK_TAU = 0x1p-300;
enum SuffstatRoute { SS_PER_CLUSTER = 0, SS_FEAT = 1, SS_QUAD = 2, SS_WIDE = 3 };
enum SuffstatMode { SS_DENSE = 0, SS_MASKED_DENSE = 1, SS_ZERO_SKIP = 2, SS_WORK_LIST = 3 };
struct SuffstatPlan {
  SuffstatRoute route;
  int nchunks;
  int64_t chunk_rows;
  int extra, klast0, KR;
  int clusters_per_block;
  const char* name;
};
SuffstatPlan suffstat_plan(int DP, int DC, int64_t NP, int K, SuffstatMode mode);
struct SuffstatLaunch {
  int DP;
  int DC = 0;
  const double* X;
  int64_t NP;
  const double* qZ;
  int64_t ldq;
  int K;
  SuffstatMode mode = SS_DENSE;
  const int* rginfo;
  const unsigned char* smask;
  double* partial;
  int nchunks = 0, KR = 0;
  int64_t chunk_rows = 0;
  const SSItem* items = nullptr;
  const int* klist = nullptr;
  int nitems = 0, skip_listed = 0;
  int speck_skip = 0;
  int nslice = 1;
  int slice0 = 0, rs = 1, klast0 = 0, nklast = 0;
  int64_t ldx = 0;
  int DPW = 0, colA = 0, colB = 0;
};
hipError_t launch_suffstat(const SuffstatLaunch& a, const SuffstatPlan& p, hipStream_t stream);

constexpr int SPECK_PROBE_STEPS = 4096;
constexpr int64_t SPECK_PROBE_MIN_ROWS = 4096;
hipError_t launch_speck_probe(const double* qZ, int64_t ldq, int K, int64_t NP, int* active, int64_t* pairs, hipStream_t stream,
                              int64_t* rows = nullptr);
inline bool speck_probe_says_skip(int64_t active, int64_t pairs) { return pairs > 0 && 4 * (pairs - active) >= pairs; }
bool speck_probe_says_lists(int64_t single, int64_t rows);

struct SsListLayout {
  int nq;
  bool wide;
  size_t ent_off;
  size_t bytes;
};
inline SsListLayout ss_list_layout(int nchunks, int64_t chunk_rows, int K) {
  SsListLayout l{(K + 3) / 4, chunk_rows > 65536, 0, 0};
  l.ent_off = ((size_t)nchunks * l.nq * sizeof(int) + 15) / 16 * 16;
  l.bytes = l.ent_off + (size_t)nchunks * l.nq * (size_t)chunk_rows * (l.wide ? 4 : 2);
  return l;
}
bool suffstat_list_instance(int DP, int DC);
bool speck_lists_enabled();
hipError_t launch_suffstat_list_build(const SuffstatLaunch& a, const SuffstatPlan& p, void* lists, size_t bytes, hipStream_t stream);
hipError_t launch_suffstat_lists(const SuffstatLaunch& a, const SuffstatPlan& p, void* lists, size_t bytes, hipStream_t stream);
int speck_skip_mode();

__host__ __device__ constexpr int ft_offdiag(int DC) { return (DC / 4) * (DC / 4 - 1) / 2; }
__host__ __device__ constexpr int ft_features(int DC) { return 16 * ft_offdiag(DC) + 10 * (DC / 4) + DC + 1; }
__host__ __device__ constexpr int ft_tiles(int DC) { return (ft_features(DC) + 15) / 16; }
enum FtKind { FT_PRODUCT = 0, FT_LINEAR = 1, FT_COUNT = 2, FT_SPARE = 3 };
struct FtFeature {
  int u, w, kind;
};
__host__ __device__ __attribute__((always_inline)) constexpr FtFeature ft_feature_rest(int DC, int one, int g) {
  const int ndiag = 10 * (DC / 4);
  if (g < ndiag) {
    const int b = 4 * (g / 10), e = g % 10;
    const int i = e < 4 ? 0 : e < 7 ? 1 : e < 9 ? 2 : 3, i0 = e < 4 ? 0 : e < 7 ? 4 : e < 9 ? 7 : 9;
    return {b + i, b + i + (e - i0), FT_PRODUCT};
  }
  g -= ndiag;
  if (g < DC) return {g, one, FT_LINEAR};
  return {one, one, g == DC ? FT_COUNT : FT_SPARE};
}
__host__ __device__ __attribute__((always_inline)) constexpr FtFeature ft_feature(int DC, int one, int f) {
  const int noff = 16 * ft_offdiag(DC);
  if (f < noff) {
    const int p = f / 16, r = f % 16;
    int ja = 1;
    while ((ja + 1) * ja / 2 <= p) ++ja;
    return {4 * (p - ja * (ja - 1) / 2) + (r & 3), 4 * ja + (r >> 2), FT_PRODUCT};
  }
  return ft_feature_rest(DC, one, f - noff);
}
#ifndef LC_FT_WAVES64
#define LC_FT_WAVES64 8
#endif
#ifndef LC_FT_WAVES128
#define LC_FT_WAVES128 8
#endif
__host__ __device__ constexpr int ft_waves(int DP) { return DP == 64 ? LC_FT_WAVES64 : DP == 128 ? LC_FT_WAVES128 : DP > 64 ? 8 : 4; }
__host__ __device__ constexpr int ft_tpw_max(int DP, int NQ) {
  const int t = (NQ >= 8 && DP > 64 && DP < 128 ? 64 : 72) / NQ;
  return t < 14 ? t : 14;
}
__host__ __device__ constexpr int ft_nslice(int DP, int DC, int NQ) {
  return (ft_tiles(DC) + ft_waves(DP) * ft_tpw_max(DP, NQ) - 1) / (ft_waves(DP) * ft_tpw_max(DP, NQ));
}
__host__ __device__ constexpr int ft_tpw(int DP, int DC, int NQ) {
  return (ft_tiles(DC) + ft_waves(DP) * ft_nslice(DP, DC, NQ) - 1) / (ft_waves(DP) * ft_nslice(DP, DC, NQ));
}
__host__ __device__ __attribute__((always_inline)) constexpr void ft_deal(int DP, int DC, int NQ, int slice, int wave, int* t0, int* nt) {
  const int tiles = ft_tiles(DC), nsl = ft_nslice(DP, DC, NQ);
  if (ft_waves(DP) == 8) {
    const int ns = 4 * nsl, s = slice * 4 + (wave & 3), l = tiles / ns, r = tiles % ns;
    const int load = l + (s < r ? 1 : 0), first = s * l + (s < r ? s : r);
    *t0 = first + (wave < 4 ? 0 : (load + 1) / 2);
// ... 295 lines not shown
```

libcluster_amd/csrc/lc_kernels_estep.hip:

```cpp
#include "lc_device.hpp"


namespace lck {

constexpr int ES_PF = 4;

template <int DP, int R>
struct EstepOcc { static constexpr int BLOCKS = DP == 64 && R == 3 ? 3 : 2; };

template <int DP, int DC, int R, int WAVES, bool SPARSE>
__global__ void __launch_bounds__(WAVES * 64, (EstepOcc<DP, R>::BLOCKS)) estep_kernel(EstepLaunch a) {
  static_assert(DC % 4 == 0 && DC <= DP && DC > DP - 16, "active width");
  constexpr int NT = DC / 4;
  constexpr int NTILES = NT * (NT + 1) / 2;
  constexpr int NREAD = NTILES + NT;
  constexpr int PF = ES_PF;
  constexpr int PS = NTILES * 16 + DC;
  constexpr int NTHR = WAVES * 64;
  extern __shared__ __attribute__((aligned(16))) double lds[];
  double* pbuf = lds;
  double* llw = lds + 2 * PS;
  double* fzw = llw + WAVES * a.K;
  double* etab = fzw + WAVES;
  double* lql = etab + 64;
  const bool lqm = R == 4 && a.lq_lds != 0;
  int* klist = reinterpret_cast<int*>(lql + (lqm ? (size_t)a.K * NTHR : 0));
  int* kflag = klist + a.K;
  int* bgrp = kflag + a.K;

  const int tid = threadIdx.x, lane = tid & 63, wave = tid >> 6;
  const int lo4 = lane & 15, hi = lane >> 4;
  const int K = a.K;
  const int64_t rg0 = ((int64_t)blockIdx.x * WAVES + wave) * R;
  fill_exp_table(etab, tid, NTHR);
  constexpr bool ROWLANES = R == 4;

  double xf[R][NT];
  int grp[R];
  bool rowok[R], rgok[R];
#pragma unroll
  for (int r = 0; r < R; ++r) {
    const int64_t rg = rg0 + r;
    rgok[r] = rg < a.nrg;
    int info = 0;
    if (rgok[r]) {
      if (a.rginfo) {
        info = a.rginfo[rg];
      } else {
        const int64_t rem = a.nrows - rg * RG;
        info = rem >= RG ? RG : (rem > 0 ? (int)rem : 0);
      }
    }
    grp[r] = info >> 5;
    rowok[r] = lo4 < (info & 31);
    const double* xr = a.X + ((rgok[r] ? rg : 0) * RG + lo4) * DP + hi;
#pragma unroll
    for (int jt = 0; jt < NT; ++jt) xf[r][jt] = xr[4 * jt];
  }
  bool myok = false;
  int owngrp = 0;
#pragma unroll
  for (int r = 0; r < R; ++r)
    if (hi == r) myok = rgok[r], owngrp = grp[r];
  double selA[R];
#pragma unroll
// ... 160 lines not shown
    double lqsel = 0.0;
    if constexpr (SADDR) {
      if constexpr (R == 3) asm volatile("s_waitcnt vmcnt(0)" : "+v"(cv[0]), "+v"(cv[1]), "+v"(cv[2])::"memory");
      else asm volatile("s_waitcnt vmcnt(0)" : "+v"(cv[0]), "+v"(cv[R > 1 ? 1 : 0])::"memory");
    }
    if constexpr (ROWLANES) {
      double t = mfma4(selA[0], d2[0], 0.0);
#pragma unroll
      for (int r = 1; r < R; ++r) t = mfma4(selA[r], d2[r], t);
      lqsel = cv[0] - 0.5 * t;
      mx[0] = fmax(mx[0], lqsel);
    } else {
#pragma unroll
      for (int r = 0; r < R; ++r) {
        const double dd = mfma4(1.0, d2[r], 0.0);
        const double lq = cv[r] - 0.5 * dd;
        mx[r] = max_raw(mx[r], lq);
        lqprev[r] = lq;
      }
    }
    kprev = k;
    if constexpr (ROWLANES) {
      if (lqm) lql[k * NTHR + tid] = lqsel;
      else lqprev[0] = lqsel;
    }
    asm volatile("s_waitcnt vmcnt(0)" ::: "memory");
    __syncthreads();
  }

  flush_lq();
  if constexpr (SADDR) asm volatile("s_waitcnt vmcnt(0)" ::: "memory");

  if (a.raw) return;

  double fz = 0.0;
  if constexpr (ROWLANES) {
    const double mymx = mx[0];
    int mygrp = grp[0];
    bool myrow = rowok[0];
#pragma unroll
    for (int r = 1; r < R; ++r)
      if (hi == r) mygrp = grp[r], myrow = rowok[r];
    double* qp = a.qZ + (rg0 + hi) * RG + lo4;
    double s = 0.0;
    if (lqm && !a.ll_part) {
      if (myok) {
#pragma unroll 8
        for (int k = 0; k < K; ++k) {
          const double e = exp_nonpos(lql[k * NTHR + tid] - mymx, etab);
          s += e;
          lql[k * NTHR + tid] = e;
        }
        const double inv = rcp_pos(s);
#pragma unroll 8
        for (int k = 0; k < K; ++k) {
          double q = lql[k * NTHR + tid] * inv;
          if (!myrow) q = 0.0;
          qp[(int64_t)k * a.ldq] = q;
        }
      }
      fz = (myok && myrow) ? log(s) + mymx : 0.0;
    } else {
    if (myok) {
#pragma unroll 8
      for (int k = 0; k < K; ++k) s += exp_nonpos((lqm ? lql[k * NTHR + tid] : qp[(int64_t)k * a.ldq]) - mymx, etab);
    }
    const double logZ = log(s) + mymx;
    for (int k = 0; k < K; ++k) {
      double ll = 0.0;
      if (myok) {
        const double lq = lqm ? lql[k * NTHR + tid] : qp[(int64_t)k * a.ldq];
        double q = exp_nonpos(lq - logZ, etab);
        if (!myrow) q = 0.0;
        qp[(int64_t)k * a.ldq] = q;
        if (a.ll_part && q > 0.0) ll = q * (lq - a.ctab[(int64_t)mygrp * K + k]);
      }
      if (a.ll_part) {
        ll = wave_sum(ll);
        if (lane == 0) llw[wave * K + k] = ll;
      }
    }
    fz = (myok && myrow) ? logZ : 0.0;
    }
  } else {
  double logZ[R];
#pragma unroll
  for (int r = 0; r < R; ++r) {
    double s = 0.0;
    if (rgok[r]) {
      const double* qp = a.qZ + (rg0 + r) * RG + lo4;
#pragma unroll 8
      for (int k = hi; k < K; k += 4) s += exp_nonpos(qp[(int64_t)k * a.ldq] - mx[r], etab);
    }
    s = sum_over_hi(s);
    logZ[r] = log(s) + mx[r];
  }
  for (int kb = 0; kb < K; kb += 4) {
    const int k = kb + hi;
    double ll = 0.0;
    if (k < K) {
#pragma unroll
      for (int r = 0; r < R; ++r) {
        if (rgok[r]) {
          double* qp = a.qZ + (int64_t)k * a.ldq + (rg0 + r) * RG + lo4;
          const double lq = *qp;
          double q = exp_nonpos(lq - logZ[r], etab);
          if (!rowok[r]) q = 0.0;
          *qp = q;
          if (a.ll_part && q > 0.0) ll += q * (lq - a.ctab[(int64_t)grp[r] * K + k]);
        }
      }
    }
    if (a.ll_part) {
      ll = sum_over_lo4(ll);
      if (k < K && lo4 == 0) llw[wave * K + k] = ll;
    }
  }
#pragma unroll
  for (int r = 0; r < R; ++r)
    if (rgok[r] && rowok[r] && hi == 0) fz += logZ[r];
  }
  fz = wave_sum(fz);
  if (lane == 0) fzw[wave] = fz;
  __syncthreads();
  if (a.ll_part)
    for (int k = tid; k < K; k += NTHR) {
      double s = 0.0;
      for (int w = 0; w < WAVES; ++w) s += llw[w * K + k];
      a.ll_part[(int64_t)blockIdx.x * K + k] = s;
    }
  if (tid == 0) {
    double s = 0.0;
    for (int w = 0; w < WAVES; ++w) s += fzw[w];
    a.fz_part[blockIdx.x] = -s;
  }
}

__host__ __device__ constexpr int wide_col(int jt, int h) { return 16 * (jt / 4) + 4 * h + (jt % 4); }
__host__ __device__ constexpr bool wide_low(int it, int jt) { return wide_col(jt, 0) <= 4 * it + 3; }
__host__ __device__ constexpr int wide_read(int n) {
  int c = 0;
  for (int part = 0; part < 2; ++part)
    for (int m = 0; m < 256; ++m) {
      const int it = 2 * (m / 32) + (m & 1), jt = (m % 32) / 2;
      if (wide_low(it, jt) == (part == 0)) {
        if (c == n) return it * 16 + jt;
        ++c;
      }
    }
  return -1;
}
__host__ __device__ constexpr int wide_nlow() {
  int c = 0;
  for (int it = 0; it < 16; ++it)
    for (int jt = 0; jt < 16; ++jt) c += wide_low(it, jt) ? 1 : 0;
  return c;
}
constexpr int WIDE_NLOW = wide_nlow();
template <int R, int WAVES, int NPX>
__global__ void __launch_bounds__(WAVES * 64, NPX ? 1 : 2) estep_wide_kernel(EstepLaunch a) {
  constexpr int CHS = WIDE_CHUNK;
// ... 224 lines not shown
  for (int r = 0; r < R; ++r)
    if (rgok[r] && rowok[r] && hi == 0) fz += logZ[r];
  fz = wave_sum(fz);
  if (lane == 0) fzw[wave] = fz;
  __syncthreads();
  if (a.ll_part)
    for (int kk = tid; kk < K; kk += NTHR) {
      double s = 0.0;
      for (int w = 0; w < WAVES; ++w) s += llw[w * K + kk];
      a.ll_part[(int64_t)blockIdx.x * K + kk] = s;
    }
  if (tid == 0) {
    double s = 0.0;
    for (int w = 0; w < WAVES; ++w) s += fzw[w];
    a.fz_part[blockIdx.x] = -s;
  }
}
constexpr int WIDE_R = 2, WIDE_WAVES = 4;

static hipError_t launch_estep_wide(const EstepLaunch& a, const EstepPlan& p, hipStream_t stream) {
  const size_t shmem = p.lds_bytes;
  const int64_t grid = p.grid;
  if (grid <= 0) return hipSuccess;
  static LdsGrant grants[3];
  auto go = [&](auto kern, LdsGrant& grant) {
    if (hipError_t e = grant_dynamic_lds(reinterpret_cast<const void*>(kern), shmem, grant); e != hipSuccess) return e;
    hipLaunchKernelGGL(kern, dim3((unsigned)grid), dim3(WIDE_WAVES * 64), shmem, stream, a);
    return hipGetLastError();
  };
  const char* sw = lck::test_switch("LC_WIDE_STREAM");
#ifdef LC_WIDE_FORCE_STREAM
  const bool stream_only = true;
  (void)sw;
#else
  const bool stream_only = sw && *sw && *sw != '0';
#endif
  if (a.DP == 192 && !stream_only) return go(estep_wide_kernel<WIDE_R, WIDE_WAVES, 3>, grants[1]);
  if (a.DP == 256 && !stream_only) return go(estep_wide_kernel<WIDE_R, WIDE_WAVES, 4>, grants[2]);
  return go(estep_wide_kernel<WIDE_R, WIDE_WAVES, 0>, grants[0]);
}

constexpr int estep_cfg_r(int DP) { return DP <= 48 ? 4 : DP <= 96 ? 3 : 2; }
constexpr int estep_cfg_waves(int DP) { return DP <= 96 ? 4 : 8; }

constexpr size_t ES_LQ_LDS_CAP = 80 * 1024;
static size_t estep_lq_cap() {
  static const size_t cap = test_switch("LC_ES_LQLDS_KB") ? (size_t)atoi(test_switch("LC_ES_LQLDS_KB")) * 1024 : ES_LQ_LDS_CAP;
  return cap;
}
static size_t estep_lds_base(int DC, int K, int R, int WAVES) {
  return (size_t)(2 * pstride(DC) + WAVES * K + WAVES + 64) * sizeof(double) + (size_t)(2 * K + WAVES * R + 2) * sizeof(int);
}
EstepPlan estep_plan(const EstepLaunch& a) {
  EstepPlan p{false, 0, -1, false, a.DC > 0 ? a.DC : a.DP, 0, 0};
  const int DP = a.DP, DC = p.DC;
  auto finish = [&](bool ok, int rows_per_block, size_t lds_bytes) {
    const int64_t rgpb = rows_per_block / RG;
    p.ok = ok, p.rows_per_block = rows_per_block, p.lds_bytes = lds_bytes;
    if (ok) p.grid = (a.nrg + rgpb - 1) / rgpb;
    return p;
  };
  if (DP > 128)
    return finish(DP % 64 == 0, WIDE_R * WIDE_WAVES * RG, (size_t)(2 * WIDE_CHUNK + WIDE_WAVES * a.K + WIDE_WAVES) * sizeof(double));
  if (padded_dim(DP) != DP) return p;
  auto lq_fits = [&](int R, int WAVES) {
    return R == 4 && !a.raw && estep_lds_base(DC, a.K, R, WAVES) + (size_t)a.K * WAVES * 64 * sizeof(double) <= estep_lq_cap();
  };
  static const bool r4_off = test_switch("LC_ES_R4") && atoi(test_switch("LC_ES_R4")) == 0;
  p.four_groups = !r4_off && (DP == 64 || DP == 80) && !a.sparse && a.K >= 6 && lq_fits(4, 4);
  const int R = p.four_groups ? 4 : estep_cfg_r(DP), WAVES = p.four_groups ? 4 : estep_cfg_waves(DP);
  const bool ok = DC == DP || (DP >= 32 && DC == DP - 8) || ((DP == 32 || DP == 48) && (DC == DP - 4 || DC == DP - 12));
  p.lq_lds = lq_fits(R, WAVES) ? 1 : 0;
  return finish(ok, R * WAVES * RG, estep_lds_base(DC, a.K, R, WAVES) + (p.lq_lds ? (size_t)a.K * WAVES * 64 * sizeof(double) : 0));
}
int64_t estep_grid(const EstepLaunch& a) { return estep_plan(a).grid; }

template <int DP, int DC, bool SPARSE, int R = estep_cfg_r(DP), int WAVES = estep_cfg_waves(DP)>
static hipError_t launch_estep_s(const EstepLaunch& a, const EstepPlan& p, hipStream_t stream) {
  if (p.DC != DC || p.rows_per_block != R * WAVES * RG) return hipErrorInvalidValue;
  EstepLaunch b = a;
  b.lq_lds = p.lq_lds;
  auto kern = estep_kernel<DP, DC, R, WAVES, SPARSE>;
  static LdsGrant grant;
  if (hipError_t e = grant_dynamic_lds(reinterpret_cast<const void*>(kern), p.lds_bytes, grant); e != hipSuccess) return e;
  if (p.grid <= 0) return hipSuccess;
  hipLaunchKernelGGL(kern, dim3((unsigned)p.grid), dim3(WAVES * 64), p.lds_bytes, stream, b);
  return hipGetLastError();
}

template <int DP>
static hipError_t launch_estep_t(const EstepLaunch& a, const EstepPlan& p, hipStream_t stream) {
  if constexpr (DP == 64 || DP == 80) {
    if (p.four_groups)
      return p.DC == DP - 8 ? launch_estep_s<DP, DP - 8, false, 4, 4>(a, p, stream) : launch_estep_s<DP, DP, false, 4, 4>(a, p, stream);
  }
  if constexpr (DP >= 32) {
    if (p.DC == DP - 8) return a.sparse ? launch_estep_s<DP, DP - 8, true>(a, p, stream) : launch_estep_s<DP, DP - 8, false>(a, p, stream);
  }
  if constexpr (DP == 32 || DP == 48) {
    if (p.DC == DP - 4) return a.sparse ? launch_estep_s<DP, DP - 4, true>(a, p, stream) : launch_estep_s<DP, DP - 4, false>(a, p, stream);
    if (p.DC == DP - 12) return a.sparse ? launch_estep_s<DP, DP - 12, true>(a, p, stream) : launch_estep_s<DP, DP - 12, false>(a, p, stream);
  }
  return a.sparse ? launch_estep_s<DP, DP, true>(a, p, stream) : launch_estep_s<DP, DP, false>(a, p, stream);
}

hipError_t launch_estep(const EstepLaunch& a, hipStream_t stream) {
  const EstepPlan p = estep_plan(a);
  if (!p.ok) return hipErrorInvalidValue;
  if (a.DP > 128) return launch_estep_wide(a, p, stream);
  switch (a.DP) {
    case 16: return launch_estep_t<16>(a, p, stream);
    case 32: return launch_estep_t<32>(a, p, stream);
    case 48: return launch_estep_t<48>(a, p, stream);
    case 64: return launch_estep_t<64>(a, p, stream);
    case 80: return launch_estep_t<80>(a, p, stream);
    case 96: return launch_estep_t<96>(a, p, stream);
    case 112: return launch_estep_t<112>(a, p, stream);
    case 128: return launch_estep_t<128>(a, p, stream);
  }
  return hipErrorInvalidValue;
}

}
```

libcluster_amd/csrc/lc_kernels_suffstat.hip:

```cpp
#include "lc_device.hpp"

#ifndef LC_SS_FEAT_MINK_ACTIVE
#define LC_SS_FEAT_MINK_ACTIVE 5
#endif
#ifndef LC_SS_FEAT_WIDTHS
#define LC_SS_FEAT_WIDTHS(DP) ((DP) >= 32 && (DP) <= 128)
#endif

namespace lck {

template <int NB>
struct SSAcc { static constexpr int N = NB * 3 + NB * (NB - 1) / 2 * 4; };

template <int NB>
__host__ __device__ constexpr bool ss_in_half(int half, int jbp, int jb) {
  if (half == 0) return true;
  const bool first = NB == 8   ? (jbp < 5 || (jbp == 5 && jb < 3))
                     : NB == 7 ? (jbp < 4 || (jbp == 4 && jb < 4))
                     : NB == 6 ? (jbp < 4 || (jbp == 4 && jb < 1))
                               : (jbp == 1 || jbp == 2);
  return first == (half == 1);
}
template <int PAN>
constexpr int ss_batch_rows() { return PAN == 2 ? 24 : SS_BR; }
// ... 804 lines not shown
          }
        } else {
#pragma unroll
          for (int c = 0; c < NQ; ++c)
            if (on(st, c)) acc[t][c] = mfma4(qa[st & 1][c], p, acc[t][c]);
          __builtin_amdgcn_sched_barrier(0);
        }
      }
    }
  };
  for (int64_t b0 = r0; b0 < r1; b0 += 2 * BR) {
    const bool more1 = b0 + BR < r1, more2 = b0 + 2 * BR < r1;
    if (more1) gload(b0 + BR);
    if (!UNEVEN || nt == TPW) batch(std::integral_constant<int, 0>{}, std::integral_constant<int, TPW>{});
    else batch(std::integral_constant<int, 0>{}, std::integral_constant<int, TPWL>{});
    if (more1) lstore(1);
    __syncthreads();
    if (!more1) break;
    if (more2) gload(b0 + 2 * BR);
    if (!UNEVEN || nt == TPW) batch(std::integral_constant<int, 1>{}, std::integral_constant<int, TPW>{});
    else batch(std::integral_constant<int, 1>{}, std::integral_constant<int, TPWL>{});
    if (more2) lstore(0);
    __syncthreads();
  }

  const int64_t SS = 1 + (int64_t)DP + (int64_t)DP * DP;
  int sle = slice, T0e = 0, nte = 0;
  asm volatile("" : "+v"(sle));
  ft_deal(DP, DC, NQ, sle, wave, &T0e, &nte);
#pragma unroll
  for (int t = 0; t < TPW; ++t) {
    if (t >= nte) continue;
    const FtFeature f = ft_feature(DC, ONE, 16 * (T0e + t) + lo2 + 4 * blk);
    if (f.kind == FT_SPARE) continue;
#pragma unroll
    for (int c = 0; c < NQ; ++c) {
      const int kk = 4 * c + hi;
      if (kk >= KC) continue;
      double* out = a.partial + ((int64_t)chunk * a.KR + k0 + kk) * SS;
      const double v = acc[t][c];
      if (f.kind == FT_PRODUCT) {
        double* S = out + 1 + DP;
        S[(int64_t)f.u * DP + f.w] = v;
        S[(int64_t)f.w * DP + f.u] = v;
      } else if (f.kind == FT_LINEAR) {
        out[1 + f.u] = v;
      } else {
        out[0] = v;
      }
    }
  }
}

__global__ void __launch_bounds__(256) speck_probe_kernel(const double* qZ, int64_t ldq, int K, int64_t stride, int nsteps, int nq,
                                                           int nqp, int* active) {
  const int64_t t = (int64_t)blockIdx.x * 256 + threadIdx.x;
  const int c = (int)(t % nqp);
  unsigned rk = 0;
  if (t / nqp < nsteps && c < nq) {
    const int64_t row = 4 * stride * (t / nqp);
#pragma unroll
    for (int i = 0; i < 4; ++i) {
      const int k = 4 * c + i;
      if (k < K) {
        const double2* qp = reinterpret_cast<const double2*>(qZ + (int64_t)k * ldq + row);
        const double2 v0 = qp[0], v1 = qp[1];
        rk |= (!(v0.x < SPECK_TAU) ? 1u : 0u) | (!(v0.y < SPECK_TAU) ? 2u : 0u) | (!(v1.x < SPECK_TAU) ? 4u : 0u) |
              (!(v1.y < SPECK_TAU) ? 8u : 0u);
      }
    }
  }
  const int lane = threadIdx.x & 63;
  const unsigned long long b = __ballot(rk != 0);
  if (lane == 0 && b != 0) atomicAdd(active, __popcll(b));
  if (nqp <= 64) {
    const unsigned long long grp = (nqp == 64 ? ~0ull : ((1ull << nqp) - 1ull)) << (lane & ~(nqp - 1));
    int single = 0;
#pragma unroll
    for (int i = 0; i < 4; ++i) {
      const unsigned long long br = __ballot((rk >> i) & 1u);
      single += __popcll(__ballot(c == 0 && __popcll(br & grp) == 1));
    }
    if (lane == 0 && single != 0) atomicAdd(active + 1, single);
  }
}
hipError_t launch_speck_probe(const double* qZ, int64_t ldq, int K, int64_t NP, int* active, int64_t* pairs, hipStream_t stream,
                              int64_t* rows) {
  const int64_t steps = NP / 4;
  *pairs = 0;
  if (rows) *rows = 0;
  if (hipError_t e = hipMemsetAsync(active, 0, 2 * sizeof(int), stream); e != hipSuccess) return e;
  if (steps < 1 || K < 1) return hipSuccess;
  const int nsteps = (int)(steps < SPECK_PROBE_STEPS ? steps : SPECK_PROBE_STEPS), nq = (K + 3) / 4;
  const int64_t stride = steps / nsteps;
  int nqp = 1;
  while (nqp < nq) nqp *= 2;
  *pairs = (int64_t)nsteps * nq;
  if (rows && nqp <= 64) *rows = 4 * (int64_t)nsteps;
  hipLaunchKernelGGL(speck_probe_kernel, dim3((unsigned)(((int64_t)nsteps * nqp + 255) / 256)), dim3(256), 0, stream, qZ, ldq, K, stride,
                     nsteps, nq, nqp, active);
  return hipGetLastError();
}

template <int DP, int DC, int NQ, bool SPECK>
static hipError_t launch_ss_feat_i(const SuffstatLaunch& b, hipStream_t stream) {
  constexpr int BR = ft_batch_rows(DP), LD = lds_row_stride(DP);
  const size_t shmem = (size_t)(2 * BR * LD + 2 * BR * ft_qld(NQ)) * sizeof(double);
  auto kern = suffstat_feat_kernel<DP, DC, NQ, SPECK>;
  static LdsGrant grant;
  if (hipError_t e = grant_dynamic_lds(reinterpret_cast<const void*>(kern), shmem, grant); e != hipSuccess) return e;
  hipLaunchKernelGGL(kern, dim3((unsigned)(b.nchunks * ft_nslice(DP, DC, NQ))), dim3(64 * ft_waves(DP)), shmem, stream, b);
  return hipGetLastError();
}
template <int DP, int DC, int NQ>
static hipError_t launch_ss_feat_q(const SuffstatLaunch& b, hipStream_t stream) {
  return b.speck_skip ? launch_ss_feat_i<DP, DC, NQ, true>(b, stream) : launch_ss_feat_i<DP, DC, NQ, false>(b, stream);
}
template <int DP, int DC>
static hipError_t launch_ss_feat_d(const SuffstatLaunch& a, hipStream_t stream) {
  SuffstatLaunch b = a;
  const int range = ft_range(DP, a.K);
  for (int k0 = 0; k0 < a.K; k0 += range) {
    b.klast0 = k0;
    const int nq = ((a.K - k0 < range ? a.K - k0 : range) + 3) / 4;
    hipError_t e = hipErrorInvalidValue;
    switch (ft_instance_quads(nq)) {
      case 2: e = launch_ss_feat_q<DP, DC, 2>(b, stream); break;
      case 4: e = launch_ss_feat_q<DP, DC, 4>(b, stream); break;
      case 5: e = launch_ss_feat_q<DP, DC, 5>(b, stream); break;
      case 6: e = launch_ss_feat_q<DP, DC, 6>(b, stream); break;
      case 7: e = launch_ss_feat_q<DP, DC, 7>(b, stream); break;
      case 8: e = launch_ss_feat_q<DP, DC, 8>(b, stream); break;
      case 16:
        if constexpr (DP == 128) e = launch_ss_feat_q<DP, DC, 16>(b, stream);
        break;
    }
    if (e != hipSuccess) return e;
  }
  return hipSuccess;
}
template <int DP>
static hipError_t launch_ss_feat_w(const SuffstatLaunch& a, hipStream_t stream) {
  if constexpr (DP <= 48) {
    if (a.DC == DP - 4) return launch_ss_feat_d<DP, DP - 4>(a, stream);
    if (a.DC == DP - 12) return launch_ss_feat_d<DP, DP - 12>(a, stream);
  }
  if (a.DC == DP - 8) return launch_ss_feat_d<DP, DP - 8>(a, stream);
  if (a.DC != 0 && a.DC != DP) return hipErrorInvalidValue;
  return launch_ss_feat_d<DP, DP>(a, stream);
}
static hipError_t launch_ss_feat(const SuffstatLaunch& a, hipStream_t stream) {
  switch (a.DP) {
    case 32: return launch_ss_feat_w<32>(a, stream);
// ... 14 lines not shown
#define LC_FTL_BR 48
#endif
#ifndef LC_FTL_SPREAD
#define LC_FTL_SPREAD 12
#endif
__host__ __device__ constexpr int ftl_read(int DC, int r) {
  int n = 0;
  for (int t = 0; t < ftl_tpw(DC); ++t) {
    if (t == 0 || ftl_wi(DC, t) != ftl_wi(DC, t - 1)) {
      if (n == r) return -1 - ftl_wi(DC, t);
      ++n;
    }
    if (n == r) return t;
    ++n;
  }
  return ftl_tpw(DC);
}
bool speck_lists_enabled() { return LC_FT_SPECK_LISTS != 0; }
#ifndef LC_FT_LIST_SHARE64
#define LC_FT_LIST_SHARE64 58
#endif
bool speck_probe_says_lists(int64_t single, int64_t rows) { return rows > 0 && 64 * single >= (int64_t)LC_FT_LIST_SHARE64 * rows; }
bool suffstat_list_instance(int DP, int DC) { return DP == 64 && (DC == 0 || DC == 64 || DC == 56); }

template <typename IT>
__global__ void __launch_bounds__(256) ss_list_build_kernel(const double* __restrict__ qZ, int64_t ldq, int K, int64_t NP,
                                                             int64_t chunk_rows, int nq, int* __restrict__ lens, IT* __restrict__ ent) {
  __shared__ int wcnt[2][32][4];
  const int chunk = blockIdx.x, tid = threadIdx.x, lane = tid & 63, wave = tid >> 6;
  const int64_t r0 = (int64_t)chunk * chunk_rows;
  const int64_t r1 = (r0 + chunk_rows) < NP ? (r0 + chunk_rows) : NP;
  if (r0 >= r1) {
    for (int c = tid; c < nq; c += 256) lens[(int64_t)chunk * nq + c] = 0;
    return;
  }
  for (int q0 = 0; q0 < nq; q0 += 32) {
    const int nqg = nq - q0 < 32 ? nq - q0 : 32;
    int base = 0, par = 0;
    for (int64_t t0 = r0; t0 < r1; t0 += 256, par ^= 1) {
      const int64_t row = t0 + tid;
      const bool valid = row < r1;
      const double* qr = qZ + (valid ? row : r1 - 1);
      unsigned m = 0;
      for (int c8 = 0; c8 < nqg; c8 += 8) {
        double v[32];
#pragma unroll
        for (int i = 0; i < 32; ++i) {
          const int k = 4 * (q0 + c8) + i;
          v[i] = qr[(int64_t)(k < K ? k : K - 1) * ldq];
        }
#pragma unroll
        for (int i = 0; i < 32; ++i) {
          const int k = 4 * (q0 + c8) + i;
          if (valid && k < K && !(v[i] < SPECK_TAU)) m |= 1u << (c8 + i / 4);
        }
      }
      int mycnt = 0;
      for (int c = 0; c < nqg; ++c) {
        const unsigned long long bal = __ballot((m >> c) & 1u);
        if (lane == c) mycnt = __popcll(bal);
      }
      if (lane < nqg) wcnt[par][lane][wave] = mycnt;
      __syncthreads();
      int mybase = 0;
      if (lane < nqg) {
        int tot = 0, before = 0;
#pragma unroll
        for (int w = 0; w < 4; ++w) {
          const int n = wcnt[par][lane][w];
          before += w < wave ? n : 0;
          tot += n;
        }
        mybase = base + before;
        base += tot;
      }
      for (int c = 0; c < nqg; ++c) {
        const unsigned long long bal = __ballot((m >> c) & 1u);
        const int at = __shfl(mybase, c) + (int)__builtin_amdgcn_mbcnt_hi((unsigned)(bal >> 32), __builtin_amdgcn_mbcnt_lo((unsigned)bal, 0u));
        if ((m >> c) & 1u) ent[((int64_t)chunk * nq + q0 + c) * chunk_rows + at] = (IT)(row - r0);
      }
    }
    if (wave == 0 && lane < nqg) lens[(int64_t)chunk * nq + q0 + lane] = base;
    __syncthreads();
  }
}

template <int DP, int DC, typename IT>
__global__ void __launch_bounds__(512, 2) suffstat_list_kernel(SuffstatLaunch a, const int* __restrict__ lens, const IT* __restrict__ ent,
                                                                int nq) {
  static_assert(DC % 4 == 0 && DC <= DP && DC > DP - 16, "active width");
  constexpr int NTHR = 512, BR = LC_FTL_BR, LD = lds_row_stride(DP), QLD = 4, XBUF = BR * LD, QBUF = BR * QLD;
  constexpr int ONE = DP, NT = ftl_tpw(DC);
  constexpr int TPR = DP / 2, RPP = NTHR / TPR, NPRE = BR / RPP;
  static_assert(LD > DP && NTHR % TPR == 0 && BR % RPP == 0 && BR % 4 == 0 && 4 * BR <= NTHR, "staging");
  static_assert((XBUF + (BR - 4) * LD + LD) * 8 <= 65536, "fragment reads: one address register per tile, the rest immediate");
  extern __shared__ __attribute__((aligned(16))) double lds[];
  double* xbuf = lds;
  double* qbuf = lds + 2 * XBUF;
  const int tid = threadIdx.x, lane = tid & 63, wave = tid >> 6;
  const int hi = lane >> 4, blk = (lane >> 2) & 3, lo2 = lane & 3;
  const int chunk = blockIdx.x / nq, quad = blockIdx.x % nq;
  const int64_t r0 = (int64_t)chunk * a.chunk_rows;
  const int len = lens[blockIdx.x];
  const IT* li = ent + (int64_t)blockIdx.x * a.chunk_rows;
  constexpr int NW = ftl_nw(DC);
  constexpr int NRD = NT + NW + 1, SPREAD = LC_FTL_SPREAD < 0 ? 0 : LC_FTL_SPREAD < NT ? LC_FTL_SPREAD : NT;
  const double* pu[NT];
// ... 148 lines not shown
    const FtlFeature f = ftl_feature(DC, ONE, wv, t, lo2 + 4 * blk);
    if (f.kind == FT_SPARE) continue;
    const double v = acc[t];
    if (f.kind == FT_PRODUCT) {
      double* S = out + 1 + DP;
      S[(int64_t)f.u * DP + f.w] = v;
      S[(int64_t)f.w * DP + f.u] = v;
    } else if (f.kind == FT_LINEAR) {
      out[1 + f.u] = v;
    } else {
      out[0] = v;
    }
  }
}

static hipError_t ss_list_check(const SuffstatLaunch& a, const SuffstatPlan& p, const void* lists, size_t bytes, SsListLayout* lay) {
  if (a.K <= 0 || p.nchunks <= 0 || !lists || !a.qZ || !a.X) return hipErrorInvalidValue;
  if (p.route != SS_FEAT || a.mode != SS_DENSE || a.smask || a.items || p.extra != 0) return hipErrorInvalidValue;
  if (a.nchunks != p.nchunks || a.chunk_rows != p.chunk_rows || a.KR != p.KR || a.KR != a.K) return hipErrorInvalidValue;
  if (!suffstat_list_instance(a.DP, a.DC)) return hipErrorInvalidValue;
  if (a.chunk_rows < 4 || a.chunk_rows % 4 || a.chunk_rows > (int64_t)1 << 30 || (int64_t)a.nchunks * a.chunk_rows < a.NP) return hipErrorInvalidValue;
  *lay = ss_list_layout(a.nchunks, a.chunk_rows, a.K);
  if ((int64_t)a.nchunks * lay->nq > (int64_t)1 << 30 || bytes < lay->bytes) return hipErrorInvalidValue;
  return hipSuccess;
}
hipError_t launch_suffstat_list_build(const SuffstatLaunch& a, const SuffstatPlan& p, void* lists, size_t bytes, hipStream_t stream) {
  SsListLayout lay;
  if (hipError_t e = ss_list_check(a, p, lists, bytes, &lay); e != hipSuccess) return e;
  int* lens = static_cast<int*>(lists);
  void* ent = static_cast<char*>(lists) + lay.ent_off;
  if (lay.wide)
    hipLaunchKernelGGL(ss_list_build_kernel<unsigned>, dim3((unsigned)a.nchunks), dim3(256), 0, stream, a.qZ, a.ldq, a.K, a.NP,
                       a.chunk_rows, lay.nq, lens, static_cast<unsigned*>(ent));
  else
    hipLaunchKernelGGL(ss_list_build_kernel<unsigned short>, dim3((unsigned)a.nchunks), dim3(256), 0, stream, a.qZ, a.ldq, a.K, a.NP,
                       a.chunk_rows, lay.nq, lens, static_cast<unsigned short*>(ent));
  return hipGetLastError();
}
template <int DP, int DC, typename IT>
static hipError_t launch_ss_list_i(const SuffstatLaunch& a, const SsListLayout& lay, const void* lists, hipStream_t stream) {
  constexpr int BR = LC_FTL_BR;
  const size_t shmem = (size_t)(2 * BR * lds_row_stride(DP) + 2 * BR * 4) * sizeof(double);
  auto kern = suffstat_list_kernel<DP, DC, IT>;
  static LdsGrant grant;
  if (hipError_t e = grant_dynamic_lds(reinterpret_cast<const void*>(kern), shmem, grant); e != hipSuccess) return e;
  hipLaunchKernelGGL(kern, dim3((unsigned)(a.nchunks * lay.nq)), dim3(512), shmem, stream, a, static_cast<const int*>(lists),
                     reinterpret_cast<const IT*>(static_cast<const char*>(lists) + lay.ent_off), lay.nq);
  return hipGetLastError();
}
hipError_t launch_suffstat_lists(const SuffstatLaunch& a, const SuffstatPlan& p, void* lists, size_t bytes, hipStream_t stream) {
  SsListLayout lay;
  if (hipError_t e = ss_list_check(a, p, lists, bytes, &lay); e != hipSuccess) return e;
  if (hipError_t e = launch_suffstat_list_build(a, p, lists, bytes, stream); e != hipSuccess) return e;
  const bool narrow = a.DC == 56;
  if (lay.wide) return narrow ? launch_ss_list_i<64, 56, unsigned>(a, lay, lists, stream) : launch_ss_list_i<64, 64, unsigned>(a, lay, lists, stream);
  return narrow ? launch_ss_list_i<64, 56, unsigned short>(a, lay, lists, stream)
                : launch_ss_list_i<64, 64, unsigned short>(a, lay, lists, stream);
}

struct SqItem {
  int kind, ia, ja;
};
__host__ __device__ constexpr int sq_items(int DC) { return (DC / 4) * (DC / 4 + 1) / 2 + DC / 4 + 1; }
__host__ __device__ constexpr SqItem sq_item(int DC, int n) {
  for (int ja = 0; ja < DC / 4; ++ja) {
    if (n <= ja) return SqItem{0, n, ja};
    n -= ja + 1;
    if (n == 0) return SqItem{1, 0, ja};
    n -= 1;
  }
  return SqItem{2, 0, 0};
}
__host__ __device__ constexpr int sq_part_lo(int DC, int NPART, int p) { return (sq_items(DC) * p + NPART - 1) / NPART; }
__host__ __device__ constexpr int sq_part_max(int DC, int NPART) {
  int m = 0;
  for (int p = 0; p < NPART; ++p) {
    const int n = sq_part_lo(DC, NPART, p + 1) - sq_part_lo(DC, NPART, p);
    m = n > m ? n : m;
  }
  return m;
}
constexpr int SQ_BR = 32, SQ_QLD = 18;
inline int sq_npart(int DP, int K) {
  const int nq = (K + 3) / 4;
  if (DP > 48) return 4;
  return nq == 2 ? 2 : nq == 4 ? (DP <= 32 ? 1 : 2) : 4;
}
inline int sq_nslice(int DP, int K) { return (((K + 3) / 4) * sq_npart(DP, K) + 3) / 4; }
inline bool ss_quad_eligible(int DP, int K) {
  static const int mode = test_switch("LC_SS_QUAD") ? atoi(test_switch("LC_SS_QUAD")) : -1;
  if (mode == 0 || DP < 32 || DP > 64 || K < 1 || K > 16) return false;
  if (mode == 1) return true;
  return K >= 3;
}
template <int DP, int DC, int NPART>
__global__ void __launch_bounds__(256, 2) suffstat_quad_kernel(SuffstatLaunch a) {
  static_assert(DC % 4 == 0 && DC <= DP && DC > DP - 16, "active width");
  constexpr int NT = DC / 4, BR = SQ_BR, LD = lds_row_stride(DP), QLD = SQ_QLD, XBUF = BR * LD, QBUF = BR * QLD, NTHR = 256;
  constexpr int NACC = sq_part_max(DC, NPART);
  extern __shared__ __attribute__((aligned(16))) double lds[];
  double* xbuf = lds;
  double* qbuf = lds + 2 * XBUF;
  const int tid = threadIdx.x, lane = tid & 63, wave = tid >> 6;
  const int hi = lane >> 4, blk = (lane >> 2) & 3, lo2 = lane & 3;
  const int K = a.K, NQ = (K + 3) / 4;
  int chunk, slice;
// ... 434 lines not shown
```

libcluster_amd/csrc/lc_predict.cpp:

```cpp
#include <algorithm>
#include <cmath>
#include <cstring>
#include <limits>
#include <stdexcept>
#include <string>
#include <vector>

#include "lc_ctx.hpp"
#include "lc_engine.hpp"
#include "lc_host.hpp"
#include "lc_predict.hpp"

namespace lcc {

void Context::predict_rows(int K, int Kp, const double* c, const double* pc, const double* ps, const double* pe,
                           bool keep_q) {
  use_device();
  if (K < 1 || Kp < 0) throw std::invalid_argument("K must be >= 1");
  pred_vb_ = false;
  if (NP_ == 0) {
    qz_[cur_].K = K;
    pred_vb_ = true;
    pred_logp_ = pred_logp_ || Kp > 0;
    return;
  }
  if (qz_[cur_].cap < std::max(K, Kp) || !qz_[cur_].buf.p) throw std::logic_error("predict_rows: no raw E-step columns");
  plabel_.reserve((size_t)NP_);
  plogz_.reserve((size_t)NP_);
  if (Kp > 0) plogp_.reserve((size_t)NP_);
  const size_t nc = (size_t)J_ * K, np = (size_t)J_ * Kp;
  hpack_.resize(nc + np + 2 * (size_t)Kp);
  std::copy(c, c + nc, hpack_.data());
  if (Kp > 0) {
    std::copy(pc, pc + np, hpack_.data() + nc);
    std::copy(ps, ps + Kp, hpack_.data() + nc + np);
    std::copy(pe, pe + Kp, hpack_.data() + nc + np + Kp);
  }
  ptab_.reserve(hpack_.size());
  LC_HIP(hipMemcpyAsync(ptab_.p, hpack_.data(), hpack_.size() * sizeof(double), hipMemcpyHostToDevice, stream_));
  lck::PredictRowsLaunch a;
  a.col = qz_[cur_].buf.p;
  a.qcol = qz_[cur_].buf.p;
  a.ldq = NP_;
  a.K = K;
  a.Kp = Kp;
  a.nrg = NP_ / lck::RG;
  a.rginfo = J_ > 1 ? rginfo_.p : nullptr;
  a.nrows = Nj_[0];
  a.ctab = ptab_.p;
  a.ptab = ptab_.p + nc;
  a.pscale = ptab_.p + nc + np;
  a.pexp = ptab_.p + nc + np + Kp;
  a.keep_q = keep_q ? 1 : 0;
  a.label = plabel_.p;
  a.logZ = plogz_.p;
  a.logp = Kp > 0 ? plogp_.p : nullptr;
  LC_HIP(lck::launch_predict_rows(a, stream_));
  LC_HIP(hipStreamSynchronize(stream_));
  qz_[cur_].K = K;
  qz_[cur_].hash_ok = false;
  pred_vb_ = true;
  pred_logp_ = pred_logp_ || Kp > 0;
}

bool Context::predict_diag(int mode, int Kp, const double* av, const double* w, const double* pc, const double* pe) {
  use_device();
  if (Kp < 1) throw std::invalid_argument("K must be >= 1");
  pred_logp_ = false;
  if (NP_ == 0) {
    pred_logp_ = true;
    return true;
  }
  const int D = D_, DP = DP_;
  plogp_.reserve((size_t)NP_);
  pflag_.reserve(1);
  const size_t nw = (size_t)Kp * DP, np = (size_t)J_ * Kp;
  hpack_.assign(2 * nw + np + (size_t)Kp, 0.0);
  for (int k = 0; k < Kp; ++k) {
    std::copy(av + (size_t)k * D, av + (size_t)(k + 1) * D, hpack_.data() + (size_t)k * DP);
    std::copy(w + (size_t)k * D, w + (size_t)(k + 1) * D, hpack_.data() + nw + (size_t)k * DP);
  }
  std::copy(pc, pc + np, hpack_.data() + 2 * nw);
  std::copy(pe, pe + Kp, hpack_.data() + 2 * nw + np);
  ptab_.reserve(hpack_.size());
  LC_HIP(hipMemcpyAsync(ptab_.p, hpack_.data(), hpack_.size() * sizeof(double), hipMemcpyHostToDevice, stream_));
  LC_HIP(hipMemsetAsync(pflag_.p, 0, sizeof(int), stream_));
  lck::PredictDiagLaunch a;
  a.mode = mode;
  a.X = X_.p;
  a.DP = DP;
  a.nrg = NP_ / lck::RG;
  a.rginfo = J_ > 1 ? rginfo_.p : nullptr;
  a.nrows = Nj_[0];
  a.Kp = Kp;
  a.a = ptab_.p;
  a.w = ptab_.p + nw;
  a.ptab = ptab_.p + 2 * nw;
  a.pexp = ptab_.p + 2 * nw + np;
  a.logp = plogp_.p;
  a.flag = pflag_.p;
  LC_HIP(lck::launch_predict_diag(a, stream_));
  int flag = 0;
  LC_HIP(hipMemcpyAsync(&flag, pflag_.p, sizeof(int), hipMemcpyDeviceToHost, stream_));
  LC_HIP(hipStreamSynchronize(stream_));
  if (flag) return false;
  pred_logp_ = true;
  return true;
}

void Context::get_predictions(int j, int64_t row0, int64_t n, int32_t* label, double* logZ, double* logp) const {
  use_device();
  if (j < 0 || j >= J_ || row0 < 0 || n < 0 || row0 + n > Nj_[j]) throw std::invalid_argument("row range out of bounds");
  if (!pred_vb_) throw std::invalid_argument("the context holds no prediction (lc_model_predict)");
  if (logp && !pred_logp_) throw std::invalid_argument("the context's prediction has no log density");
  if (n == 0) return;
  const size_t at = (size_t)(goff_[j] + row0);
  if (label) LC_HIP(hipMemcpyAsync(label, plabel_.p + at, (size_t)n * sizeof(int), hipMemcpyDeviceToHost, stream_));
  if (logZ) LC_HIP(hipMemcpyAsync(logZ, plogz_.p + at, (size_t)n * sizeof(double), hipMemcpyDeviceToHost, stream_));
  if (logp) LC_HIP(hipMemcpyAsync(logp, plogp_.p + at, (size_t)n * sizeof(double), hipMemcpyDeviceToHost, stream_));
  LC_HIP(hipStreamSynchronize(stream_));
}

void Context::predict_cond(int Kp, int Db, const double* tt, const double* ps, const double* pe, const double* ma,
                           const double* B, const double* mb) {
  use_device();
  if (Kp < 1 || Db < 1) throw std::invalid_argument("K and the number of target columns must be >= 1");
  pred_cond_ = 0;
  if (NP_ == 0) {
    pred_cond_ = Db;
    return;
  }
  if (qz_[cur_].cap < Kp || !qz_[cur_].buf.p) throw std::logic_error("predict_cond: no raw E-step columns");
  const int Da = D_, Dae = (Da + 1 + 3) / 4 * 4, Dbp = (Db + 3) / 4 * 4;
  pcmean_.reserve((size_t)NP_ * Db);
  pclogp_.reserve((size_t)NP_);
  const size_t nt = (size_t)J_ * Kp, nm = (size_t)Kp * Dae, nT = nm * Dbp;
  hpack_.assign(nt + 2 * (size_t)Kp + nm + nT, 0.0);
  double* h = hpack_.data();
  std::copy(tt, tt + nt, h);
  std::copy(ps, ps + Kp, h + nt);
  std::copy(pe, pe + Kp, h + nt + Kp);
  double* hm = h + nt + 2 * (size_t)Kp;
  double* hT = hm + nm;
  for (int k = 0; k < Kp; ++k) {
    std::copy(ma + (size_t)k * Da, ma + (size_t)(k + 1) * Da, hm + (size_t)k * Dae);
    double* Tk = hT + (size_t)k * Dae * Dbp;
    for (int t = 0; t < Db; ++t) {
      for (int c = 0; c < Da; ++c) Tk[(size_t)c * Dbp + t] = B[((size_t)k * Db + t) * Da + c];
      Tk[(size_t)Da * Dbp + t] = mb[(size_t)k * Db + t];
    }
  }
  ptab_.reserve(hpack_.size());
  LC_HIP(hipMemcpyAsync(ptab_.p, hpack_.data(), hpack_.size() * sizeof(double), hipMemcpyHostToDevice, stream_));
  LC_HIP(lck::launch_predict_cond(predict_cond_args(Kp, Db), stream_));
  LC_HIP(hipStreamSynchronize(stream_));
  qz_[cur_].K = Kp;
  qz_[cur_].hash_ok = false;
  pred_cond_ = Db;
}

lck::PredictCondLaunch Context::predict_cond_args(int Kp, int Db) const {
  const int Da = D_, Dae = (Da + 1 + 3) / 4 * 4, Dbp = (Db + 3) / 4 * 4;
  const size_t nt = (size_t)J_ * Kp, nm = (size_t)Kp * Dae;
  lck::PredictCondLaunch a;
  a.X = X_.p;
  a.DP = DP_;
  a.Da = Da;
  a.Dae = Dae;
  a.Db = Db;
  a.Dbp = Dbp;
  a.Kp = Kp;
  a.col = qz_[cur_].buf.p;
  a.ldq = NP_;
  a.nrg = NP_ / lck::RG;
  a.rginfo = J_ > 1 ? rginfo_.p : nullptr;
  a.nrows = Nj_[0];
  a.ttab = ptab_.p;
  a.pscale = ptab_.p + nt;
  a.pexp = ptab_.p + nt + Kp;
  a.mext = ptab_.p + nt + 2 * (size_t)Kp;
  a.T = a.mext + nm;
  a.mean = pcmean_.p;
  a.logp = pclogp_.p;
  return a;
}

void Context::predict_cond_var(int Kp, int Db, const double* S, const double* g) {
  use_device();
  pred_cond_var_ = false;
  if (pred_cond_ != Db || Kp < 1) throw std::logic_error("predict_cond_var: no conditional prediction of this width");
  if (NP_ == 0) {
    pred_cond_var_ = true;
    return;
  }
  if (qz_[cur_].K != Kp) throw std::logic_error("predict_cond_var: the columns of predict_cond are gone");
  const int Dbp = (Db + 3) / 4 * 4;
  pcvar_.reserve((size_t)NP_ * Db);
  hpack_.assign((size_t)Kp + (size_t)Kp * Dbp, 0.0);
  std::copy(g, g + Kp, hpack_.data());
  for (int k = 0; k < Kp; ++k) std::copy(S + (size_t)k * Db, S + (size_t)(k + 1) * Db, hpack_.data() + Kp + (size_t)k * Dbp);
  pvtab_.reserve(hpack_.size());
  LC_HIP(hipMemcpyAsync(pvtab_.p, hpack_.data(), hpack_.size() * sizeof(double), hipMemcpyHostToDevice, stream_));
  lck::PredictCondVarLaunch v;
  v.c = predict_cond_args(Kp, Db);
  v.g = pvtab_.p;
  v.S = pvtab_.p + Kp;
  v.var = pcvar_.p;
  LC_HIP(lck::launch_predict_cond_var(v, stream_));
  LC_HIP(hipStreamSynchronize(stream_));
  pred_cond_var_ = true;
// ... 232 lines not shown
    std::copy(mean + (size_t)k * D, mean + (size_t)(k + 1) * D, hm + (size_t)k * DP);
    for (int r = 0; r < D; ++r)
      std::copy(P + ((size_t)k * D + r) * D, P + ((size_t)k * D + r + 1) * D, hP + ((size_t)k * DP + r) * DP);
  }
  ptab_.reserve(hpack_.size());
  LC_HIP(hipMemcpyAsync(ptab_.p, hpack_.data(), hpack_.size() * sizeof(double), hipMemcpyHostToDevice, stream_));
  lck::PredictHolesLaunch a;
  a.X = X_.p;
  a.DP = DP;
  a.Kp = Kp;
  a.col = qz_[cur_].buf.p;
  a.ldq = NP_;
  a.nrg = NP_ / lck::RG;
  a.rginfo = J_ > 1 ? rginfo_.p : nullptr;
  a.nrows = Nj_[0];
  a.count = hcount_.p;
  a.cols = hcols_.p;
  a.ttab = ptab_.p;
  a.pscale = ptab_.p + nt;
  a.pexp = ptab_.p + nt + Kp;
  a.mean = ptab_.p + nt + Kp + ne;
  a.P = a.mean + nm;
  a.logp = hlogp_.p;
  if (gnu) {
    lck::PredictHolesVarLaunch v;
    v.h = a;
    v.gnu = a.P + nP;
    v.var = hvar_.p;
    LC_HIP(lck::launch_predict_holes_var(v, stream_));
  } else if (ndraws > 0) {
    hdraws_.reserve((size_t)NP_ * ndraws * lck::HOLES_MAX);
    hdlabel_.reserve((size_t)NP_ * ndraws);
    LC_HIP(hipMemsetAsync(hdraws_.p, 0, (size_t)NP_ * ndraws * lck::HOLES_MAX * sizeof(double), stream_));
    LC_HIP(hipMemsetAsync(hdlabel_.p, 0xff, (size_t)NP_ * ndraws * sizeof(int), stream_));
    lck::PredictHolesKeepLaunch kp;
    kp.h = a;
    kp.tcol = qz_[cur_].buf.p;
    LC_HIP(lck::launch_predict_holes_keep(kp, stream_));
    lck::HolesDrawsLaunch v;
    v.h = a;
    v.goff = J_ > 1 ? goff_d_.p : nullptr;
    v.cqnu = a.P + nP;
    v.ndraws = ndraws;
    v.seed = seed;
    v.draws = hdraws_.p;
    v.label = hdlabel_.p;
    LC_HIP(lck::launch_holes_draws(v, stream_));
  } else {
    LC_HIP(lck::launch_predict_holes(a, stream_));
  }
  LC_HIP(hipStreamSynchronize(stream_));
  qz_[cur_].K = Kp;
  qz_[cur_].hash_ok = false;
  dcache_invalidate();
  pred_holes_ = true;
  pred_holes_var_ = gnu != nullptr;
  pred_holes_draws_ = ndraws;
}

void Context::get_completed_draws(int j, int64_t row0, int64_t n, double* draws, int32_t* label) const {
  use_device();
  if (!pred_holes_ || pred_holes_draws_ < 1)
    throw std::invalid_argument("the context holds no draws of completed rows (lc_model_predict_incomplete_draws)");
  if (j < 0 || j >= J_ || row0 < 0 || n < 0 || row0 + n > Nj_[j]) throw std::invalid_argument("row range out of bounds");
  if (n == 0) return;
  const size_t at = (size_t)(goff_[j] + row0) * pred_holes_draws_, cnt = (size_t)n * pred_holes_draws_;
  static_assert(sizeof(int) == sizeof(int32_t), "the components are int32");
  if (draws)
    LC_HIP(hipMemcpyAsync(draws, hdraws_.p + at * lck::HOLES_MAX, cnt * lck::HOLES_MAX * sizeof(double), hipMemcpyDeviceToHost,
                          stream_));
  if (label) LC_HIP(hipMemcpyAsync(label, hdlabel_.p + at, cnt * sizeof(int), hipMemcpyDeviceToHost, stream_));
  LC_HIP(hipStreamSynchronize(stream_));
}

void Context::get_completed_var(int j, int64_t row0, int64_t n, double* var, int64_t row_stride) const {
  use_device();
  if (!pred_holes_) throw std::invalid_argument("the context holds no completed rows (lc_model_predict_incomplete_var)");
  if (!pred_holes_var_)
    throw std::invalid_argument("the context's completed rows have no variance (lc_model_predict_incomplete_var)");
  if (j < 0 || j >= J_ || row0 < 0 || n < 0 || row0 + n > Nj_[j]) throw std::invalid_argument("row range out of bounds");
  if (row_stride < lck::HOLES_MAX) throw std::invalid_argument("row_stride is smaller than LC_HOLES_MAX");
  if (n == 0 || !var) return;
  const size_t at = (size_t)(goff_[j] + row0), w = (size_t)lck::HOLES_MAX * sizeof(double);
  LC_HIP(hipMemcpy2DAsync(var, (size_t)row_stride * sizeof(double), hvar_.p + at * lck::HOLES_MAX, w, w, (size_t)n,
                          hipMemcpyDeviceToHost, stream_));
  LC_HIP(hipStreamSynchronize(stream_));
}

void Context::get_completed(int j, int64_t row0, int64_t n, double* rows, int64_t row_stride, double* logp, int32_t* count,
                            int32_t* cols) const {
  use_device();
  if (!pred_holes_) throw std::invalid_argument("the context holds no completed rows (lc_model_predict_incomplete)");
  if (j < 0 || j >= J_ || row0 < 0 || n < 0 || row0 + n > Nj_[j]) throw std::invalid_argument("row range out of bounds");
  if (rows && row_stride < D_) throw std::invalid_argument("row_stride is smaller than the number of columns");
  if (n == 0) return;
  const size_t at = (size_t)(goff_[j] + row0);
  static_assert(sizeof(int) == sizeof(int32_t), "the hole records are int32");
  if (rows)
    LC_HIP(hipMemcpy2DAsync(rows, (size_t)row_stride * sizeof(double), X_.p + at * DP_, (size_t)DP_ * sizeof(double),
                            (size_t)D_ * sizeof(double), (size_t)n, hipMemcpyDeviceToHost, stream_));
  if (logp) LC_HIP(hipMemcpyAsync(logp, hlogp_.p + at, (size_t)n * sizeof(double), hipMemcpyDeviceToHost, stream_));
  if (count) LC_HIP(hipMemcpyAsync(count, hcount_.p + at, (size_t)n * sizeof(int), hipMemcpyDeviceToHost, stream_));
  if (cols)
    LC_HIP(hipMemcpyAsync(cols, hcols_.p + at * lck::HOLES_MAX, (size_t)n * lck::HOLES_MAX * sizeof(int),
                          hipMemcpyDeviceToHost, stream_));
  LC_HIP(hipStreamSynchronize(stream_));
// ... 633 lines not shown
```

libcluster_amd/csrc/lc_testhooks.hip:

```cpp
#include <algorithm>
#include <cstdio>
#include <vector>

#include "lc_device.hpp"
#include "lc_predict.hpp"

namespace {

using lck::RG;
typedef long long i64;

class Scope {
 public:
  ~Scope() {
    for (auto& b : bufs_)
      if (b.d) (void)hipFree(b.d);
  }
  template <typename T>
  T* in(const T* h, size_t n) { return static_cast<T*>(add(const_cast<T*>(h), n * sizeof(T), false, true)); }
  template <typename T>
  T* io(T* h, size_t n) { return static_cast<T*>(add(h, n * sizeof(T), true, true)); }
  template <typename T>
  T* out(T* h, size_t n) { return static_cast<T*>(add(h, n * sizeof(T), true, false)); }
  template <typename T>
// ... 741 lines not shown
                                i64 nent) {
  if (!X || !qZ || !partial || !plan_out || !lens_out || !ent_out || K < 1 || K > 4096 || !gw_width_ok(DP, DC)) return -1;
  if (NP < RG || NP % RG || NP > HOT_MAX_NRG * RG || ldq < NP || ldq % 2) return -1;
  const i64 SS = lck::stat_stride(DP);
  if (fold && (!sums || !folded || nfolded < (i64)K * SS)) return -1;
  const lck::SuffstatPlan p = lck::suffstat_plan(DP, DC, NP, K, lck::SS_DENSE);
  plan_out[0] = p.route, plan_out[1] = p.nchunks, plan_out[2] = p.chunk_rows, plan_out[3] = p.extra, plan_out[4] = p.klast0;
  plan_out[5] = p.KR, plan_out[6] = p.clusters_per_block;
  if (p.nchunks < 1 || p.chunk_rows < lck::SS_BR || p.chunk_rows % lck::SS_BR || (i64)p.nchunks * p.chunk_rows < NP) return -1;
  const lck::SsListLayout lay = lck::ss_list_layout(p.nchunks, p.chunk_rows, K);
  const i64 nseg = (i64)p.nchunks * lay.nq;
  if (npartial < (i64)p.nchunks * p.KR * SS || nlens < nseg || nent < nseg * p.chunk_rows) return -1;
  Scope s;
  lck::SuffstatLaunch a{};
  a.DP = DP;
  a.DC = DC;
  a.X = s.in(X, (size_t)NP * DP);
  a.NP = NP;
  a.qZ = s.in(qZ, (size_t)K * (size_t)ldq);
  a.ldq = ldq;
  a.K = K;
  a.mode = lck::SS_DENSE;
  a.rginfo = nullptr;
  a.smask = nullptr;
  a.partial = s.io(partial, (size_t)npartial);
  a.nchunks = p.nchunks;
  a.KR = p.KR;
  a.chunk_rows = p.chunk_rows;
  unsigned char* lists = s.scratch<unsigned char>(lay.bytes);
  double* dfold = fold ? s.io(folded, (size_t)nfolded) : nullptr;
  if (!s.ok()) return s.finish(hipSuccess);
  hipError_t e = hipMemset(lists, 0xff, lay.bytes);
  if (e == hipSuccess)
    e = sums ? lck::launch_suffstat_lists(a, p, lists, lay.bytes, nullptr) : lck::launch_suffstat_list_build(a, p, lists, lay.bytes, nullptr);
  if (e == hipSuccess && fold) e = lck::launch_reduce_partials(a.partial, p.nchunks, (i64)K * SS, dfold, nullptr);
  const int rc = s.finish(e);
  if (rc != 0) return rc;
  std::vector<unsigned char> raw(lay.bytes);
  if (hipMemcpy(raw.data(), lists, lay.bytes, hipMemcpyDeviceToHost) != hipSuccess) return -1;
  const int* lens = reinterpret_cast<const int*>(raw.data());
  for (i64 g = 0; g < nseg; ++g)
    if (lens[g] < 0 || lens[g] > p.chunk_rows) return -2;
  for (i64 g = 0; g < nseg; ++g) {
    lens_out[g] = lens[g];
    for (int i = 0; i < lens[g]; ++i) {
      const size_t at = (size_t)g * (size_t)p.chunk_rows + (size_t)i;
      ent_out[at] = lay.wide ? (int)reinterpret_cast<const unsigned*>(raw.data() + lay.ent_off)[at]
                             : (int)reinterpret_cast<const unsigned short*>(raw.data() + lay.ent_off)[at];
    }
  }
  return 0;
}

LC_HOOK lcx_test_suffstat_list_deal(int DP, int DC, i64* info, int* feat, i64 nfeat) {
  if (!info || !feat || !gw_width_ok(DP, DC) || !lck::suffstat_list_instance(DP, DC)) return -1;
  const int dc = DC ? DC : DP, waves = 8, tiles = lck::ftl_tpw(dc);
  if (nfeat < (i64)waves * tiles * 16 * 4) return -1;
  info[0] = lck::ftl_shared(dc) ? 1 : 0, info[1] = waves, info[2] = tiles, info[3] = lck::ftl_paired(dc), info[4] = lck::ftl_split(dc);
  info[5] = DP;
  for (int v = 0; v < waves; ++v)
    for (int t = 0; t < tiles; ++t)
      for (int l = 0; l < 16; ++l) {
        const lck::FtlFeature f = lck::ftl_feature(dc, DP, v, t, l);
        int* o = feat + ((size_t)(v * tiles + t) * 16 + l) * 4;
        o[0] = f.u, o[1] = f.w, o[2] = f.kind, o[3] = f.shared;
      }
  return 0;
}

LC_HOOK lc_test_fused_plan(int DP, i64 nrg, int K, i64* out) {
  if (!out || K < 1 || K > 4096 || nrg < 0 || nrg > HOT_MAX_NRG || DP < 1 || DP > 1024) return -1;
  out[0] = lck::fused_eligible(DP, K) ? 1 : 0;
  out[1] = lck::fused_plan(DP, nrg, K);
  out[2] = lck::current_device_cus();
  out[3] = (i64)lck::fused_record(DP, K);
  return 0;
}
LC_HOOK lc_test_fused(const double* X, int D, i64 nrg, const double* params, const double* ctab, int J, const int* rginfo, i64 nrows,
                      int K, int want_ll, int grid, double* qZ, int Kbuf, i64 ldq, double* partial, i64 npartial, int* grid_used) {
  const int DP = 16;
  if (!X || !params || !ctab || !qZ || !partial || !grid_used || D < 1 || D > DP || K < 1 || Kbuf < K || Kbuf > 8192) return -1;
  if (nrg < 1 || nrg > HOT_MAX_NRG || ldq < nrg * RG || J < 1 || J > (1 << 20) || !lck::fused_eligible(DP, K)) return -1;
  if (rginfo ? !rginfo_ok(rginfo, nrg, J) : (J != 1 || nrows < 0 || nrows > nrg * RG)) return -1;
  const int plan = lck::fused_plan(DP, nrg, K);
  if (plan < 1 || grid < 0 || grid > plan) return -1;
  const int g = grid ? grid : plan;
  if (npartial < (i64)g * lck::fused_record(DP, K)) return -1;
  *grid_used = g;
  Scope s;
  lck::FusedLaunch a{};
  a.DP = DP;
  a.D = D;
  a.X = s.in(X, (size_t)(nrg * RG) * DP);
  a.nrg = nrg;
  a.rginfo = rginfo ? s.in(rginfo, (size_t)nrg) : nullptr;
  a.nrows = nrows;
  a.params = s.in(params, (size_t)K * (size_t)lck::pstride(DP));
  a.ctab = s.in(ctab, (size_t)J * K);
  a.K = K;
  a.qZ = s.io(qZ, (size_t)Kbuf * (size_t)ldq);
  a.ldq = ldq;
  a.partial = s.io(partial, (size_t)npartial);
  a.want_ll = want_ll != 0;
  a.grid = g;
  a.ngroups = J;
  if (!s.ok()) return s.finish(hipSuccess);
// ... 136 lines not shown
```

libcluster_amd/csrc/lc_topic_predict.cpp:

```cpp
#include <algorithm>
#include <stdexcept>
#include <vector>

#include "lc_ctx.hpp"
#include "lc_host.hpp"
#include "lc_topic.hpp"

namespace lcc {

void Context::topic_infer(int K, int T, const double* a, const double* E, int max_sweeps, double tol, bool keep_q) {
  use_device();
  if (K < 1 || T < 1) throw std::invalid_argument("qZ and qY must have at least one column");
  if (max_sweeps < 1) throw std::invalid_argument("max_sweeps must be at least 1");
  predict_clear();
  if (NP_ > 0 && (qz_[cur_].cap < K || !qz_[cur_].buf.p)) throw std::logic_error("topic_infer: no raw E-step columns");
  const int64_t maxN = *std::max_element(Nj_.begin(), Nj_.end());
  lck::TopicInferLaunch l;
  l.threads = maxN <= 64 ? 64 : maxN <= 128 ? 128 : 256;
  const size_t lds = lck::topic_infer_lds(K, T, l.threads, Nj_.data(), J_, &l.tile_cap, &l.e_lds);
  if (lds == 0) throw std::invalid_argument("the model is too large for the inference kernel (K and T against its LDS)");
  plabel_.reserve((size_t)std::max<int64_t>(NP_, 1));
  plogz_.reserve((size_t)std::max<int64_t>(NP_, 1));
  tqy_.reserve((size_t)J_ * T);
  tf_.reserve((size_t)J_ * 2);
  tint_.reserve((size_t)J_ * 2);
  tnrows_.reserve((size_t)J_);
  const size_t na = (size_t)J_ * T, ne = (size_t)T * K;
  hpack_.resize(na + ne);
  std::copy(a, a + na, hpack_.data());
  std::copy(E, E + ne, hpack_.data() + na);
  ptab_.reserve(hpack_.size());
  LC_HIP(hipMemcpyAsync(ptab_.p, hpack_.data(), hpack_.size() * sizeof(double), hipMemcpyHostToDevice, stream_));
  LC_HIP(hipMemcpyAsync(tnrows_.p, Nj_.data(), (size_t)J_ * sizeof(int64_t), hipMemcpyHostToDevice, stream_));
  l.col = qz_[cur_].buf.p;
  l.ldq = NP_;
  l.K = K;
  l.T = T;
  l.docs = J_;
  l.goff = goff_d_.p;
  l.nrows = tnrows_.p;
  l.a = ptab_.p;
  l.E = ptab_.p + na;
  l.max_sweeps = max_sweeps;
  l.tol = tol;
  l.keep_q = keep_q ? 1 : 0;
  l.label = plabel_.p;
  l.logZ = plogz_.p;
  l.qY = tqy_.p;
  l.F = tf_.p;
  l.dint = tint_.p;
  LC_HIP(lck::launch_topic_infer(l, lds, stream_));
  LC_HIP(hipStreamSynchronize(stream_));
  qz_[cur_].K = K;
  qz_[cur_].hash_ok = false;
  pred_vb_ = true;
  pred_docs_T_ = T;
}

void Context::get_doc_predictions(int doc0, int n, double* qY, int32_t* label_t, double* Fyz, double* Fz,
                                  int32_t* sweeps) const {
  use_device();
  if (doc0 < 0 || n < 0 || (int64_t)doc0 + n > J_) throw std::invalid_argument("document range out of bounds");
  if (pred_docs_T_ < 1) throw std::invalid_argument("the context holds no document prediction (lc_tmodel_predict)");
  if (n == 0) return;
  const int T = pred_docs_T_;
  std::vector<double> f((size_t)n * 2);
  std::vector<int> di((size_t)n * 2);
  if (qY)
    LC_HIP(hipMemcpyAsync(qY, tqy_.p + (size_t)doc0 * T, (size_t)n * T * sizeof(double), hipMemcpyDeviceToHost, stream_));
  LC_HIP(hipMemcpyAsync(f.data(), tf_.p + (size_t)doc0 * 2, f.size() * sizeof(double), hipMemcpyDeviceToHost, stream_));
  LC_HIP(hipMemcpyAsync(di.data(), tint_.p + (size_t)doc0 * 2, di.size() * sizeof(int), hipMemcpyDeviceToHost, stream_));
  LC_HIP(hipStreamSynchronize(stream_));
  for (int i = 0; i < n; ++i) {
    if (Fyz) Fyz[i] = f[(size_t)i * 2];
    if (Fz) Fz[i] = f[(size_t)i * 2 + 1];
    if (label_t) label_t[i] = di[(size_t)i * 2];
    if (sweeps) sweeps[i] = di[(size_t)i * 2 + 1];
  }
}

}

namespace lce {

void topic_predict(lcc::Context& ctx, const TopicModel& model, const int* groups, const double* W, int max_sweeps,
                   double tol, bool keep_qz) {
  const int I = ctx.J(), D = ctx.D(), T = model.T, K = (int)model.clusters.size();
  const bool mcm = !model.clusters_t.empty();
  if (K < 1 || T < 1) throw std::invalid_argument("the model has no clusters");
  ctx.predict_clear();

  std::vector<double> a((size_t)I * T), E((size_t)T * K);
  for (int t = 0; t < T; ++t) std::copy(model.weights_t[(size_t)t].Elogpi.begin(), model.weights_t[(size_t)t].Elogpi.end(),
                                        E.begin() + (size_t)t * K);
  std::vector<std::vector<double>> At;
  std::vector<double> ctt;
  const int Dt = mcm ? model.clusters_t[0].D : 0;
  for (int t = 0; mcm && t < T; ++t) {
    At.push_back(model.clusters_t[(size_t)t].whitener());
    ctt.push_back(model.clusters_t[(size_t)t].eloglike_const());
  }
  for (int i = 0; i < I; ++i) {
    const lch::WeightState& wj = model.weights_j[(size_t)(groups ? groups[i] : 0)];
    for (int t = 0; t < T; ++t) {
      double v = wj.Elogpi[(size_t)t];
      if (mcm) {
        const double* w = W + (size_t)i * Dt;
// ... 29 lines not shown
```

Measured before the change: 381.6 million.

## Emit per-row-group responsibility masks from E-step to feed suffstat sparsity lists

The E-step kernel now writes a compact per-row-group bitmask, one 16-bit word per group of four clusters, marking which clusters keep non-negligible responsibilities, using wave ballots. The mask is probed once after the E-step. The next suff-stat pass reuses the cached probe counts and builds its sparse row lists from the masks, instead of rescanning the full qZ matrix with a separate probe kernel plus a host sync. This removes a dense read of qZ and a sync point per iteration. In exchange the E-step gains ballot and store work, and every qZ writer must invalidate the mask cache.

```diff
diff --git a/include/libcluster_hip.h b/include/libcluster_hip.h
--- a/include/libcluster_hip.h
+++ b/include/libcluster_hip.h
@@ -87,6 +87,8 @@
 int lc_ctx_set_speck_skip(lc_ctx* ctx, int on);
 int lc_ctx_speck_passes(lc_ctx* ctx, int64_t* skipping, int64_t* dense);
 int lc_ctx_speck_list_passes(lc_ctx* ctx, int64_t* lists);
+int lc_ctx_set_estep_masks(lc_ctx* ctx, int on);
+int lc_ctx_speck_mask_passes(lc_ctx* ctx, int64_t* masks);
 
 int lc_trim_cache(void);
 
diff --git a/libcluster_amd/capi.py b/libcluster_amd/capi.py
--- a/libcluster_amd/capi.py
+++ b/libcluster_amd/capi.py
@@ -228,6 +228,8 @@
     L.lc_ctx_set_speck_skip.argtypes = [C.c_void_p, C.c_int]
     L.lc_ctx_speck_passes.argtypes = [C.c_void_p, c_int64_p, c_int64_p]
     L.lc_ctx_speck_list_passes.argtypes = [C.c_void_p, c_int64_p]
+    L.lc_ctx_set_estep_masks.argtypes = [C.c_void_p, C.c_int]
+    L.lc_ctx_speck_mask_passes.argtypes = [C.c_void_p, c_int64_p]
     L.lc_ctx_get_rows.argtypes = [C.c_void_p, C.c_int, C.c_int64, C.c_int64, c_double_p]
     L.lc_ctx_set_qz.argtypes = [C.c_void_p, C.c_int, c_double_p, C.c_int, C.c_int64, C.c_int64]
     L.lc_ctx_get_qz.argtypes = [C.c_void_p, C.c_int, c_double_p, C.c_int64, C.c_int64]
@@ -451,6 +453,14 @@
         check(lib().lc_ctx_speck_list_passes(self._h, C.byref(a)))
         return a.value
 
+    def set_estep_masks(self, on: bool = True):
+        check(lib().lc_ctx_set_estep_masks(self._h, int(on)))
+
+    def speck_mask_passes(self):
+        a = C.c_int64()
+        check(lib().lc_ctx_speck_mask_passes(self._h, C.byref(a)))
+        return a.value
+
     def set_sharding(self, whole_groups: bool):
         check(lib().lc_ctx_set_sharding(self._h, int(whole_groups)))
 
diff --git a/libcluster_amd/csrc/lc_capi.cpp b/libcluster_amd/csrc/lc_capi.cpp
--- a/libcluster_amd/csrc/lc_capi.cpp
+++ b/libcluster_amd/csrc/lc_capi.cpp
@@ -461,6 +461,21 @@
   });
 }
 
+int lc_ctx_set_estep_masks(lc_ctx* ctx, int on) {
+  return guarded([&] {
+    need(ctx, "ctx");
+    ctx->impl.set_estep_masks(on != 0);
+  });
+}
+
+int lc_ctx_speck_mask_passes(lc_ctx* ctx, int64_t* masks) {
+  return guarded([&] {
+    need(ctx, "ctx");
+    need(masks, "masks");
+    *masks = ctx->impl.speck_passes_masks();
+  });
+}
+
 int lc_ctx_get_rows(lc_ctx* ctx, int j, int64_t row0, int64_t n, double* out) {
   return guarded([&] {
     need(ctx, "ctx");
diff --git a/libcluster_amd/csrc/lc_ctx.cpp b/libcluster_amd/csrc/lc_ctx.cpp
--- a/libcluster_amd/csrc/lc_ctx.cpp
+++ b/libcluster_amd/csrc/lc_ctx.cpp
@@ -187,6 +187,7 @@
 template struct DevBuf<int>;
 template struct DevBuf<int64_t>;
 template struct DevBuf<unsigned char>;
+template struct DevBuf<unsigned short>;
 
 Context::Context(int device, hipStream_t stream) : device_(device), stream_(stream) {
   static int n = 0;
@@ -406,10 +407,21 @@
   static const bool on = std::getenv("LC_TEST_QHASH_KEEP_STALE") != nullptr;
   return on;
 }
+static bool test_keep_stale_masks() {
+  static const bool on = std::getenv("LC_TEST_QMASK_KEEP_STALE") != nullptr;
+  return on;
+}
 #endif
+void Context::qz_written(QZ& q) {
+#ifdef LC_TEST_HOOKS
+  if (test_keep_stale_masks()) return;
+#endif
+  q.mask_ok = false;
+}
 void Context::ensure_qz(QZ& q, int K, bool preserve) {
   use_device();
   q.hash_ok = false;
+  qz_written(q);
 #ifdef LC_TEST_HOOKS
   if (test_keep_stale() && q.hash.p) q.hash_ok = true;
 #endif
@@ -440,6 +452,7 @@
   if (j < 0 || j >= J_) throw std::invalid_argument("group index out of range");
   if (K < 1) throw std::invalid_argument("K must be >= 1");
   qz_[cur_].hash_ok = false;
+  qz_written(qz_[cur_]);
   if (K != qz_[cur_].K) {
     ensure_qz(qz_[cur_], K, false);
     LC_HIP(hipMemsetAsync(qz_[cur_].buf.p, 0, (size_t)NP_ * K * sizeof(double), stream_));
@@ -606,6 +619,7 @@
   }
   q.K = (int)keep.size();
   q.hash_ok = false;
+  qz_written(q);
 #ifdef LC_TEST_HOOKS
   if (test_keep_stale() && q.hash.p) q.hash_ok = true;
 #endif
@@ -618,6 +632,7 @@
   static const bool full_only = lck::test_switch("LC_SPLIT_FULL_CLONE") != nullptr;
   if (!full_only && NP_ > 0 && Ksave >= 1 && qz_[cur_].hash_ok && a.hash_ok && a.buf.p && a.hash.p && qz_[cur_].hash.p &&
       a.cap >= Ksave + 1 && (a.K == Ksave || a.K == Ksave + 1)) {
+    qz_written(a);
     LC_HIP(lck::launch_qz_resync(a.buf.p, qz_[cur_].buf.p, NP_, Ksave, Ksave + 1, NP_, a.hash.p, qz_[cur_].hash.p, stream_));
     a.K = Ksave;
     clone_resyncs_ += 1;
@@ -760,6 +775,7 @@
   const bool hashed = q.hash_ok;
   if (q.K + 1 > q.cap) ensure_qz(q, q.K + 1, true);
   q.hash_ok = hashed;
+  qz_written(q);
   bool mark = hashed;
 #ifdef LC_TEST_HOOKS
   if (test_keep_stale()) mark = false;
@@ -946,16 +962,42 @@
     ensure_qz(qz_[cur_], K, false);
     qz_[cur_].K = K;
   }
-  const lck::EstepLaunch a =
+  lck::EstepLaunch a =
       gw_estep_launch(K, A, m, c, X_.p, NP_, Nj_[0], target ? target : qz_[cur_].buf.p, raw, LLk != nullptr);
+  QZ& q = qz_[cur_];
+  bool masks = estep_masks_ && !target && !raw && NP_ >= lck::SPECK_PROBE_MIN_ROWS && K <= 256 && speck_skip_ && !skip_zero_ &&
+               lck::speck_lists_enabled() && lck::suffstat_list_instance(DP_, DC_) && lck::estep_plan(a).emits;
+  if (masks) {
+    if (mask_route_K_ != K || mask_route_NP_ != NP_ || mask_route_DC_ != DC_) {
+      mask_route_feat_ = lck::suffstat_plan(DP_, DC_, NP_, K, lck::SS_DENSE).route == lck::SS_FEAT;
+      mask_route_K_ = K, mask_route_NP_ = NP_, mask_route_DC_ = DC_;
+    }
+    masks = mask_route_feat_;
+  }
+  if (masks) {
+    q.qmask.reserve((size_t)((K + 3) / 4) * (size_t)a.nrg);
+    a.qmask = q.qmask.p;
+  }
   timed(Timed::Estep, [&] { LC_HIP(lck::launch_estep(a, stream_)); });
   if (raw) {
     LC_HIP(hipStreamSynchronize(stream_));
     return;
   }
   enqueue_sums(lck::estep_grid(a), K, LLk != nullptr);
+  if (masks) {
+    speck_active_.reserve(2);
+    hprobe_.resize(1);
+    LC_HIP(lck::launch_speck_probe_masks(q.qmask.p, a.nrg, K, NP_, speck_active_.p, &q.mask_pairs, stream_, &q.mask_rows));
+    LC_HIP(hipMemcpyAsync(hprobe_.data(), speck_active_.p, 2 * sizeof(int), hipMemcpyDeviceToHost, stream_));
+  }
   run_overlap();
   LC_HIP(hipStreamSynchronize(stream_));
+  if (masks) {
+    std::memcpy(q.mask_counts, hprobe_.data(), 2 * sizeof(int));
+    q.mask_K = K;
+    q.mask_nrg = a.nrg;
+    q.mask_ok = true;
+  }
   read_sums(K, Fz, LLk);
 }
 
@@ -1090,6 +1132,24 @@
   return nrec;
 }
 
+#ifdef LC_TEST_HOOKS
+void Context::verify_qmask(const QZ& q) {
+  const int64_t nrg = NP_ / lck::RG;
+  const size_t n = (size_t)((q.K + 3) / 4) * (size_t)nrg;
+  DevBuf<unsigned short> ref;
+  ref.reserve(n);
+  LC_HIP(lck::launch_qmask_from_qz(q.buf.p, NP_, q.K, nrg, ref.p, stream_));
+  std::vector<unsigned short> have(n), want(n);
+  LC_HIP(hipMemcpyAsync(want.data(), ref.p, n * sizeof(unsigned short), hipMemcpyDeviceToHost, stream_));
+  LC_HIP(hipMemcpyAsync(have.data(), q.qmask.p, n * sizeof(unsigned short), hipMemcpyDeviceToHost, stream_));
+  LC_HIP(hipStreamSynchronize(stream_));
+  size_t nbad = 0;
+  for (size_t i = 0; i < n; ++i) nbad += have[i] != want[i] ? 1 : 0;
+  if (nbad) throw std::runtime_error("LC_TEST_VERIFY_QMASK: " + std::to_string(nbad) + " mask words are not those of qZ (K = " + std::to_string(q.K) + ")");
+  std::cerr << "[masks] verified, K " << q.K << std::endl;
+}
+#endif
+
 void Context::suffstat(const unsigned char* smask, double* Nk, double* xs, double* xxs, double* Njk) {
   const int K = qz_[cur_].K, D = D_, DP = DP_;
   if (K < 1) throw std::invalid_argument("qZ has not been set");
@@ -1133,13 +1193,27 @@
     const int nchunks = plan.nchunks, KR = plan.KR, extra = plan.extra;
     a.skip_listed = listed && skip_zero_;
     bool lists = false;
+    bool from_masks = false;
     if (speck_skip_ && plan.route == lck::SS_FEAT && NP_ >= lck::SPECK_PROBE_MIN_ROWS) {
       speck_active_.reserve(2);
       int64_t pairs = 0, rows = 0;
       int counts2[2] = {0, 0};
-      LC_HIP(lck::launch_speck_probe(a.qZ, a.ldq, K, NP_, speck_active_.p, &pairs, stream_, &rows));
-      LC_HIP(hipMemcpyAsync(counts2, speck_active_.p, 2 * sizeof(int), hipMemcpyDeviceToHost, stream_));
-      LC_HIP(hipStreamSynchronize(stream_));
+      const QZ& q = qz_[cur_];
+      from_masks = estep_masks_ && q.mask_ok && q.mask_K == K && q.mask_nrg == NP_ / lck::RG && q.qmask.p != nullptr;
+#ifdef LC_TEST_HOOKS
+      if (test_keep_stale_masks() && estep_masks_ && q.mask_ok && q.mask_nrg == NP_ / lck::RG && q.qmask.p != nullptr &&
+          q.qmask.cap >= (size_t)((K + 3) / 4) * (size_t)(NP_ / lck::RG))
+        from_masks = true;
+      if (from_masks && std::getenv("LC_TEST_VERIFY_QMASK") != nullptr) verify_qmask(q);
+#endif
+      if (from_masks) {
+        pairs = q.mask_pairs, rows = q.mask_rows;
+        counts2[0] = q.mask_counts[0], counts2[1] = q.mask_counts[1];
+      } else {
+        LC_HIP(lck::launch_speck_probe(a.qZ, a.ldq, K, NP_, speck_active_.p, &pairs, stream_, &rows));
+        LC_HIP(hipMemcpyAsync(counts2, speck_active_.p, 2 * sizeof(int), hipMemcpyDeviceToHost, stream_));
+        LC_HIP(hipStreamSynchronize(stream_));
+      }
       const int active = counts2[0];
       const bool sort_pays = 2 * (int64_t)active <= pairs && DP < 128;
       a.speck_skip = !lck::speck_probe_says_skip(active, pairs) ? 0 : sort_pays ? lck::speck_skip_mode() : 1;
@@ -1163,7 +1237,12 @@
       const size_t lbytes = lck::ss_list_layout(nchunks, plan.chunk_rows, K).bytes;
       sslists_.reserve(lbytes);
       a.speck_skip = 0;
-      timed(Timed::Suffstat, [&] { LC_HIP(lck::launch_suffstat_lists(a, plan, sslists_.p, lbytes, stream_)); });
+      if (from_masks) {
+        speck_masks_ += 1;
+        timed(Timed::Suffstat,
+              [&] { LC_HIP(lck::launch_suffstat_lists_masks(a, plan, qz_[cur_].qmask.p, NP_ / lck::RG, sslists_.p, lbytes, stream_)); });
+      } else
+        timed(Timed::Suffstat, [&] { LC_HIP(lck::launch_suffstat_lists(a, plan, sslists_.p, lbytes, stream_)); });
     } else
       timed(Timed::Suffstat, [&] { LC_HIP(lck::launch_suffstat(a, plan, stream_)); });
     if (listed)
diff --git a/libcluster_amd/csrc/lc_ctx.hpp b/libcluster_amd/csrc/lc_ctx.hpp
--- a/libcluster_amd/csrc/lc_ctx.hpp
+++ b/libcluster_amd/csrc/lc_ctx.hpp
@@ -132,6 +132,8 @@
   int64_t speck_passes_skipping() const { return speck_skipping_; }
   int64_t speck_passes_dense() const { return speck_dense_; }
   int64_t speck_passes_lists() const { return speck_lists_; }
+  void set_estep_masks(bool on) { estep_masks_ = on; }
+  int64_t speck_passes_masks() const { return speck_masks_; }
   bool group_sharded() const { return group_sharded_ && distributed(); }
   void inherit_comm(const Context& parent) {
     ar_fn_ = parent.ar_fn_;
@@ -140,6 +142,7 @@
     group_sharded_ = parent.group_sharded_;
     skip_zero_ = parent.skip_zero_;
     speck_skip_ = parent.speck_skip_;
+    estep_masks_ = parent.estep_masks_;
   }
 
   void qz_fill(int K, double value);
@@ -252,7 +255,17 @@
     int K = 0;
     DevBuf<int64_t> hash;
     bool hash_ok = false;
+    DevBuf<unsigned short> qmask;
+    bool mask_ok = false;
+    int mask_K = 0;
+    int64_t mask_nrg = 0;
+    int mask_counts[2] = {0, 0};
+    int64_t mask_pairs = 0, mask_rows = 0;
   };
+  void qz_written(QZ& q);
+#ifdef LC_TEST_HOOKS
+  void verify_qmask(const QZ& q);
+#endif
   void ensure_qz(QZ& q, int K, bool preserve);
   void build_layout(int J, const int64_t* Nj, int D);
   void allreduce(double* dbuf, int64_t count);
@@ -279,6 +292,12 @@
   bool speck_skip_ = true;
   int64_t speck_skipping_ = 0, speck_dense_ = 0, speck_lists_ = 0;
   DevBuf<int> speck_active_;
+  bool estep_masks_ = true;
+  int mask_route_K_ = -1, mask_route_DC_ = -1;
+  int64_t mask_route_NP_ = -1;
+  bool mask_route_feat_ = false;
+  int64_t speck_masks_ = 0;
+  PinnedBuf hprobe_;
   DevBuf<unsigned char> sslists_;
 
   int J_ = 0, D_ = 0, DP_ = 0;
diff --git a/libcluster_amd/csrc/lc_device.hpp b/libcluster_amd/csrc/lc_device.hpp
--- a/libcluster_amd/csrc/lc_device.hpp
+++ b/libcluster_amd/csrc/lc_device.hpp
@@ -28,6 +28,8 @@
 __device__ __forceinline__ double mfma4(double a, double b, double c) {
   return __builtin_amdgcn_mfma_f64_4x4x4f64(a, b, c, 0, 0, 0);
 }
+
+__device__ __forceinline__ bool speck_keeps(double q) { return !(q < SPECK_TAU); }
 
 __device__ __forceinline__ double max_raw(double a, double b) {
   asm("v_max_f64 %0, %0, %1" : "+v"(a) : "v"(b));
diff --git a/libcluster_amd/csrc/lc_kernels.h b/libcluster_amd/csrc/lc_kernels.h
--- a/libcluster_amd/csrc/lc_kernels.h
+++ b/libcluster_amd/csrc/lc_kernels.h
@@ -58,6 +58,7 @@
   int raw = 0;
   int sparse = 0;
   int lq_lds = 0;
+  unsigned short* qmask = nullptr;
 };
 struct EstepPlan {
   bool ok;
@@ -66,6 +67,7 @@
   bool four_groups;
   int DC, lq_lds;
   size_t lds_bytes;
+  bool emits = false;
 };
 EstepPlan estep_plan(const EstepLaunch& a);
 int64_t estep_grid(const EstepLaunch& a);
@@ -161,6 +163,13 @@
 bool speck_lists_enabled();
 hipError_t launch_suffstat_list_build(const SuffstatLaunch& a, const SuffstatPlan& p, void* lists, size_t bytes, hipStream_t stream);
 hipError_t launch_suffstat_lists(const SuffstatLaunch& a, const SuffstatPlan& p, void* lists, size_t bytes, hipStream_t stream);
+hipError_t launch_suffstat_list_build_masks(const SuffstatLaunch& a, const SuffstatPlan& p, const unsigned short* qmask, int64_t nrg,
+                                            void* lists, size_t bytes, hipStream_t stream);
+hipError_t launch_suffstat_lists_masks(const SuffstatLaunch& a, const SuffstatPlan& p, const unsigned short* qmask, int64_t nrg,
+                                       void* lists, size_t bytes, hipStream_t stream);
+hipError_t launch_speck_probe_masks(const unsigned short* qmask, int64_t nrg, int K, int64_t NP, int* active, int64_t* pairs,
+                                    hipStream_t stream, int64_t* rows = nullptr);
+hipError_t launch_qmask_from_qz(const double* qZ, int64_t ldq, int K, int64_t nrg, unsigned short* qmask, hipStream_t stream);
 int speck_skip_mode();
 
 __host__ __device__ constexpr int ft_offdiag(int DC) { return (DC / 4) * (DC / 4 - 1) / 2; }
diff --git a/libcluster_amd/csrc/lc_kernels_estep.hip b/libcluster_amd/csrc/lc_kernels_estep.hip
--- a/libcluster_amd/csrc/lc_kernels_estep.hip
+++ b/libcluster_amd/csrc/lc_kernels_estep.hip
@@ -4,13 +4,21 @@
 namespace lck {
 
 constexpr int ES_PF = 4;
-
+#ifndef LC_ESTEP_QMASK
+#define LC_ESTEP_QMASK 1
+#endif
+
+__device__ __forceinline__ void emit_rowlanes(const EstepLaunch& a, bool keep, int quad, int64_t rg0, int lane) {
+  const unsigned long long b = __ballot(keep);
+  if ((lane & 15) == 0) a.qmask[(int64_t)quad * a.nrg + rg0 + (lane >> 4)] = (unsigned short)((b >> (lane & 48)) & 0xffffull);
+}
 template <int DP, int R>
 struct EstepOcc { static constexpr int BLOCKS = DP == 64 && R == 3 ? 3 : 2; };
 
-template <int DP, int DC, int R, int WAVES, bool SPARSE>
+template <int DP, int DC, int R, int WAVES, bool SPARSE, bool EMIT = false>
 __global__ void __launch_bounds__(WAVES * 64, (EstepOcc<DP, R>::BLOCKS)) estep_kernel(EstepLaunch a) {
   static_assert(DC % 4 == 0 && DC <= DP && DC > DP - 16, "active width");
+  static_assert(!EMIT || !SPARSE, "masks: dense launches");
   constexpr int NT = DC / 4;
   constexpr int NTILES = NT * (NT + 1) / 2;
   constexpr int NREAD = NTILES + NT;
@@ -277,12 +285,29 @@
           lql[k * NTHR + tid] = e;
         }
         const double inv = rcp_pos(s);
+        if constexpr (EMIT) {
+          for (int kb = 0; kb < K; kb += 4) {
+            bool kq = false;
+#pragma unroll
+            for (int i = 0; i < 4; ++i) {
+              const int k = kb + i;
+              if (k < K) {
+                double q = lql[k * NTHR + tid] * inv;
+                if (!myrow) q = 0.0;
+                qp[(int64_t)k * a.ldq] = q;
+                kq = kq || speck_keeps(q);
+              }
+            }
+            emit_rowlanes(a, kq, kb >> 2, rg0, lane);
+          }
+        } else {
 #pragma unroll 8
         for (int k = 0; k < K; ++k) {
           double q = lql[k * NTHR + tid] * inv;
           if (!myrow) q = 0.0;
           qp[(int64_t)k * a.ldq] = q;
         }
+        }
       }
       fz = (myok && myrow) ? log(s) + mymx : 0.0;
     } else {
@@ -291,6 +316,7 @@
       for (int k = 0; k < K; ++k) s += exp_nonpos((lqm ? lql[k * NTHR + tid] : qp[(int64_t)k * a.ldq]) - mymx, etab);
     }
     const double logZ = log(s) + mymx;
+    [[maybe_unused]] bool kq = false;
     for (int k = 0; k < K; ++k) {
       double ll = 0.0;
       if (myok) {
@@ -298,6 +324,10 @@
         double q = exp_nonpos(lq - logZ, etab);
         if (!myrow) q = 0.0;
         qp[(int64_t)k * a.ldq] = q;
+        if constexpr (EMIT) {
+          kq = kq || speck_keeps(q);
+          if ((k & 3) == 3 || k == K - 1) emit_rowlanes(a, kq, k >> 2, rg0, lane), kq = false;
+        }
         if (a.ll_part && q > 0.0) ll = q * (lq - a.ctab[(int64_t)mygrp * K + k]);
       }
       if (a.ll_part) {
@@ -332,6 +362,12 @@
           double q = exp_nonpos(lq - logZ[r], etab);
           if (!rowok[r]) q = 0.0;
           *qp = q;
+          if constexpr (EMIT) {
+            const unsigned long long b = __ballot(speck_keeps(q));
+            const unsigned w = (unsigned)(b | (b >> 16) | (b >> 32) | (b >> 48)) & 0xffffu;
+            unsigned short* mw = a.qmask + ((int64_t)blockIdx.x * WAVES + __builtin_amdgcn_readfirstlane(wave)) * R;
+            if (lane == 0) mw[(int64_t)(kb >> 2) * a.nrg + r] = (unsigned short)w;
+          }
           if (a.ll_part && q > 0.0) ll += q * (lq - a.ctab[(int64_t)grp[r] * K + k]);
         }
       }
@@ -662,7 +698,7 @@
   return (size_t)(2 * pstride(DC) + WAVES * K + WAVES + 64) * sizeof(double) + (size_t)(2 * K + WAVES * R + 2) * sizeof(int);
 }
 EstepPlan estep_plan(const EstepLaunch& a) {
-  EstepPlan p{false, 0, -1, false, a.DC > 0 ? a.DC : a.DP, 0, 0};
+  EstepPlan p{false, 0, -1, false, a.DC > 0 ? a.DC : a.DP, 0, 0, false};
   const int DP = a.DP, DC = p.DC;
   auto finish = [&](bool ok, int rows_per_block, size_t lds_bytes) {
     const int64_t rgpb = rows_per_block / RG;
@@ -681,16 +717,18 @@
   const int R = p.four_groups ? 4 : estep_cfg_r(DP), WAVES = p.four_groups ? 4 : estep_cfg_waves(DP);
   const bool ok = DC == DP || (DP >= 32 && DC == DP - 8) || ((DP == 32 || DP == 48) && (DC == DP - 4 || DC == DP - 12));
   p.lq_lds = lq_fits(R, WAVES) ? 1 : 0;
+  p.emits = LC_ESTEP_QMASK != 0 && ok && DP == 64 && (DC == 64 || DC == 56) && !a.sparse && !a.raw;
   return finish(ok, R * WAVES * RG, estep_lds_base(DC, a.K, R, WAVES) + (p.lq_lds ? (size_t)a.K * WAVES * 64 * sizeof(double) : 0));
 }
 int64_t estep_grid(const EstepLaunch& a) { return estep_plan(a).grid; }
 
-template <int DP, int DC, bool SPARSE, int R = estep_cfg_r(DP), int WAVES = estep_cfg_waves(DP)>
+template <int DP, int DC, bool SPARSE, int R = estep_cfg_r(DP), int WAVES = estep_cfg_waves(DP), bool EMIT = false>
 static hipError_t launch_estep_s(const EstepLaunch& a, const EstepPlan& p, hipStream_t stream) {
   if (p.DC != DC || p.rows_per_block != R * WAVES * RG) return hipErrorInvalidValue;
+  if (EMIT != (a.qmask != nullptr) || (EMIT && !p.emits)) return hipErrorInvalidValue;
   EstepLaunch b = a;
   b.lq_lds = p.lq_lds;
-  auto kern = estep_kernel<DP, DC, R, WAVES, SPARSE>;
+  auto kern = estep_kernel<DP, DC, R, WAVES, SPARSE, EMIT>;
   static LdsGrant grant;
   if (hipError_t e = grant_dynamic_lds(reinterpret_cast<const void*>(kern), p.lds_bytes, grant); e != hipSuccess) return e;
   if (p.grid <= 0) return hipSuccess;
@@ -700,6 +738,16 @@
 
 template <int DP>
 static hipError_t launch_estep_t(const EstepLaunch& a, const EstepPlan& p, hipStream_t stream) {
+  if constexpr (DP == 64) {
+    if (a.qmask && p.emits) {
+      if (p.four_groups)
+        return p.DC == DP - 8 ? launch_estep_s<DP, DP - 8, false, 4, 4, true>(a, p, stream)
+                              : launch_estep_s<DP, DP, false, 4, 4, true>(a, p, stream);
+      constexpr int R = estep_cfg_r(DP), WAVES = estep_cfg_waves(DP);
+      return p.DC == DP - 8 ? launch_estep_s<DP, DP - 8, false, R, WAVES, true>(a, p, stream)
+                            : launch_estep_s<DP, DP, false, R, WAVES, true>(a, p, stream);
+    }
+  }
   if constexpr (DP == 64 || DP == 80) {
     if (p.four_groups)
       return p.DC == DP - 8 ? launch_estep_s<DP, DP - 8, false, 4, 4>(a, p, stream) : launch_estep_s<DP, DP, false, 4, 4>(a, p, stream);
@@ -717,6 +765,7 @@
 hipError_t launch_estep(const EstepLaunch& a, hipStream_t stream) {
   const EstepPlan p = estep_plan(a);
   if (!p.ok) return hipErrorInvalidValue;
+  if (a.qmask && !p.emits) return hipErrorInvalidValue;
   if (a.DP > 128) return launch_estep_wide(a, p, stream);
   switch (a.DP) {
     case 16: return launch_estep_t<16>(a, p, stream);
diff --git a/libcluster_amd/csrc/lc_kernels_suffstat.hip b/libcluster_amd/csrc/lc_kernels_suffstat.hip
--- a/libcluster_amd/csrc/lc_kernels_suffstat.hip
+++ b/libcluster_amd/csrc/lc_kernels_suffstat.hip
@@ -880,6 +880,21 @@
   }
 }
 
+__device__ __forceinline__ void speck_probe_count(unsigned rk, int c, int nqp, int* active) {
+  const int lane = threadIdx.x & 63;
+  const unsigned long long b = __ballot(rk != 0);
+  if (lane == 0 && b != 0) atomicAdd(active, __popcll(b));
+  if (nqp <= 64) {
+    const unsigned long long grp = (nqp == 64 ? ~0ull : ((1ull << nqp) - 1ull)) << (lane & ~(nqp - 1));
+    int single = 0;
+#pragma unroll
+    for (int i = 0; i < 4; ++i) {
+      const unsigned long long br = __ballot((rk >> i) & 1u);
+      single += __popcll(__ballot(c == 0 && __popcll(br & grp) == 1));
+    }
+    if (lane == 0 && single != 0) atomicAdd(active + 1, single);
+  }
+}
 __global__ void __launch_bounds__(256) speck_probe_kernel(const double* qZ, int64_t ldq, int K, int64_t stride, int nsteps, int nq,
                                                            int nqp, int* active) {
   const int64_t t = (int64_t)blockIdx.x * 256 + threadIdx.x;
@@ -898,35 +913,53 @@
       }
     }
   }
-  const int lane = threadIdx.x & 63;
-  const unsigned long long b = __ballot(rk != 0);
-  if (lane == 0 && b != 0) atomicAdd(active, __popcll(b));
-  if (nqp <= 64) {
-    const unsigned long long grp = (nqp == 64 ? ~0ull : ((1ull << nqp) - 1ull)) << (lane & ~(nqp - 1));
-    int single = 0;
-#pragma unroll
-    for (int i = 0; i < 4; ++i) {
-      const unsigned long long br = __ballot((rk >> i) & 1u);
-      single += __popcll(__ballot(c == 0 && __popcll(br & grp) == 1));
-    }
-    if (lane == 0 && single != 0) atomicAdd(active + 1, single);
-  }
-}
-hipError_t launch_speck_probe(const double* qZ, int64_t ldq, int K, int64_t NP, int* active, int64_t* pairs, hipStream_t stream,
-                              int64_t* rows) {
+  speck_probe_count(rk, c, nqp, active);
+}
+__global__ void __launch_bounds__(256) speck_probe_masks_kernel(const unsigned short* __restrict__ qmask, int64_t nrg, int64_t stride,
+                                                                 int nsteps, int nq, int nqp, int* active) {
+  const int64_t t = (int64_t)blockIdx.x * 256 + threadIdx.x;
+  const int c = (int)(t % nqp);
+  unsigned rk = 0;
+  if (t / nqp < nsteps && c < nq) {
+    const int64_t row = 4 * stride * (t / nqp);
+    rk = ((unsigned)qmask[(int64_t)c * nrg + (row >> 4)] >> (unsigned)(row & 15)) & 0xfu;
+  }
+  speck_probe_count(rk, c, nqp, active);
+}
+static bool speck_probe_sample(int K, int64_t NP, int64_t* pairs, int64_t* rows, int* nsteps, int64_t* stride, int* nq, int* nqp) {
   const int64_t steps = NP / 4;
   *pairs = 0;
   if (rows) *rows = 0;
+  if (steps < 1 || K < 1) return false;
+  *nsteps = (int)(steps < SPECK_PROBE_STEPS ? steps : SPECK_PROBE_STEPS), *nq = (K + 3) / 4;
+  *stride = steps / *nsteps;
+  *nqp = 1;
+  while (*nqp < *nq) *nqp *= 2;
+  *pairs = (int64_t)*nsteps * *nq;
+  if (rows && *nqp <= 64) *rows = 4 * (int64_t)*nsteps;
+  return true;
+}
+hipError_t launch_speck_probe(const double* qZ, int64_t ldq, int K, int64_t NP, int* active, int64_t* pairs, hipStream_t stream,
+                              int64_t* rows) {
+  int nsteps = 0, nq = 0, nqp = 0;
+  int64_t stride = 0;
+  const bool any = speck_probe_sample(K, NP, pairs, rows, &nsteps, &stride, &nq, &nqp);
   if (hipError_t e = hipMemsetAsync(active, 0, 2 * sizeof(int), stream); e != hipSuccess) return e;
-  if (steps < 1 || K < 1) return hipSuccess;
-  const int nsteps = (int)(steps < SPECK_PROBE_STEPS ? steps : SPECK_PROBE_STEPS), nq = (K + 3) / 4;
-  const int64_t stride = steps / nsteps;
-  int nqp = 1;
-  while (nqp < nq) nqp *= 2;
-  *pairs = (int64_t)nsteps * nq;
-  if (rows && nqp <= 64) *rows = 4 * (int64_t)nsteps;
+  if (!any) return hipSuccess;
   hipLaunchKernelGGL(speck_probe_kernel, dim3((unsigned)(((int64_t)nsteps * nqp + 255) / 256)), dim3(256), 0, stream, qZ, ldq, K, stride,
                      nsteps, nq, nqp, active);
+  return hipGetLastError();
+}
+hipError_t launch_speck_probe_masks(const unsigned short* qmask, int64_t nrg, int K, int64_t NP, int* active, int64_t* pairs,
+                                    hipStream_t stream, int64_t* rows) {
+  int nsteps = 0, nq = 0, nqp = 0;
+  int64_t stride = 0;
+  if (!qmask || !active || !pairs || nrg * RG < NP) return hipErrorInvalidValue;
+  const bool any = speck_probe_sample(K, NP, pairs, rows, &nsteps, &stride, &nq, &nqp);
+  if (hipError_t e = hipMemsetAsync(active, 0, 2 * sizeof(int), stream); e != hipSuccess) return e;
+  if (!any) return hipSuccess;
+  hipLaunchKernelGGL(speck_probe_masks_kernel, dim3((unsigned)(((int64_t)nsteps * nqp + 255) / 256)), dim3(256), 0, stream, qmask, nrg,
+                     stride, nsteps, nq, nqp, active);
   return hipGetLastError();
 }
 
@@ -1047,7 +1080,7 @@
 #pragma unroll
         for (int i = 0; i < 32; ++i) {
           const int k = 4 * (q0 + c8) + i;
-          if (valid && k < K && !(v[i] < SPECK_TAU)) m |= 1u << (c8 + i / 4);
+          if (valid && k < K && speck_keeps(v[i])) m |= 1u << (c8 + i / 4);
         }
       }
       int mycnt = 0;
@@ -1302,6 +1335,104 @@
   SsListLayout lay;
   if (hipError_t e = ss_list_check(a, p, lists, bytes, &lay); e != hipSuccess) return e;
   if (hipError_t e = launch_suffstat_list_build(a, p, lists, bytes, stream); e != hipSuccess) return e;
+  const bool narrow = a.DC == 56;
+  if (lay.wide) return narrow ? launch_ss_list_i<64, 56, unsigned>(a, lay, lists, stream) : launch_ss_list_i<64, 64, unsigned>(a, lay, lists, stream);
+  return narrow ? launch_ss_list_i<64, 56, unsigned short>(a, lay, lists, stream)
+                : launch_ss_list_i<64, 64, unsigned short>(a, lay, lists, stream);
+}
+
+template <typename IT>
+__global__ void __launch_bounds__(256) ss_list_build_masks_kernel(const unsigned short* __restrict__ qmask, int64_t nrg, int64_t NP,
+                                                                   int64_t chunk_rows, int nq, int* __restrict__ lens, IT* __restrict__ ent) {
+  __shared__ int wcnt[2][4];
+  const int chunk = blockIdx.x / nq, c = blockIdx.x % nq, tid = threadIdx.x, lane = tid & 63, wave = tid >> 6;
+  const int64_t r0 = (int64_t)chunk * chunk_rows;
+  const int64_t r1 = (r0 + chunk_rows) < NP ? (r0 + chunk_rows) : NP;
+  if (r0 >= r1) {
+    if (tid == 0) lens[blockIdx.x] = 0;
+    return;
+  }
+  const unsigned short* mq = qmask + (int64_t)c * nrg;
+  IT* seg = ent + (int64_t)blockIdx.x * chunk_rows;
+  int base = 0, par = 0;
+  for (int64_t t0 = r0; t0 < r1; t0 += 4096, par ^= 1) {
+    const int64_t row = t0 + 16 * tid;
+    unsigned m = 0;
+    if (row < r1) {
+      const int64_t w = row >> 4;
+      const unsigned sh = (unsigned)(row & 15);
+      const unsigned lo = mq[w], hi = sh != 0 && w + 1 < nrg ? mq[w + 1] : 0u;
+      m = ((lo | (hi << 16)) >> sh) & 0xffffu;
+      if (r1 - row < 16) m &= (1u << (unsigned)(r1 - row)) - 1u;
+    }
+    const int cnt = __popc(m);
+    int inc = cnt;
+#pragma unroll
+    for (int d = 1; d < 64; d <<= 1) {
+      const int up = __shfl_up(inc, d);
+      if (lane >= d) inc += up;
+    }
+    if (lane == 63) wcnt[par][wave] = inc;
+    __syncthreads();
+    int before = 0, tot = 0;
+#pragma unroll
+    for (int w = 0; w < 4; ++w) {
+      const int n = wcnt[par][w];
+      before += w < wave ? n : 0;
+      tot += n;
+    }
+    int at = base + before + inc - cnt;
+    while (m) {
+      const int i = __ffs((int)m) - 1;
+      m &= m - 1;
+      seg[at++] = (IT)(row - r0 + i);
+    }
+    base += tot;
+  }
+  if (tid == 0) lens[blockIdx.x] = base;
+}
+__global__ void __launch_bounds__(256) qmask_from_qz_kernel(const double* __restrict__ qZ, int64_t ldq, int K, int64_t nrg,
+                                                             unsigned short* __restrict__ qmask) {
+  const int64_t row = (int64_t)blockIdx.x * 256 + threadIdx.x;
+  const int c = blockIdx.y, lane = threadIdx.x & 63;
+  bool keep = false;
+  if (row < nrg * RG) {
+#pragma unroll
+    for (int i = 0; i < 4; ++i) {
+      const int k = 4 * c + i;
+      if (k < K && speck_keeps(qZ[(int64_t)k * ldq + row])) keep = true;
+    }
+  }
+  const unsigned long long b = __ballot(keep);
+  if ((lane & 15) == 0 && row < nrg * RG) qmask[(int64_t)c * nrg + (row >> 4)] = (unsigned short)((b >> lane) & 0xffffull);
+}
+hipError_t launch_qmask_from_qz(const double* qZ, int64_t ldq, int K, int64_t nrg, unsigned short* qmask, hipStream_t stream) {
+  if (!qZ || !qmask || K < 1 || nrg < 1 || ldq < nrg * RG || (K + 3) / 4 > 65535) return hipErrorInvalidValue;
+  hipLaunchKernelGGL(qmask_from_qz_kernel, dim3((unsigned)((nrg * RG + 255) / 256), (unsigned)((K + 3) / 4)), dim3(256), 0, stream, qZ, ldq,
+                     K, nrg, qmask);
+  return hipGetLastError();
+}
+hipError_t launch_suffstat_list_build_masks(const SuffstatLaunch& a, const SuffstatPlan& p, const unsigned short* qmask, int64_t nrg,
+                                            void* lists, size_t bytes, hipStream_t stream) {
+  SsListLayout lay;
+  if (hipError_t e = ss_list_check(a, p, lists, bytes, &lay); e != hipSuccess) return e;
+  if (!qmask || nrg * RG < a.NP) return hipErrorInvalidValue;
+  int* lens = static_cast<int*>(lists);
+  void* ent = static_cast<char*>(lists) + lay.ent_off;
+  const dim3 grid((unsigned)(a.nchunks * lay.nq));
+  if (lay.wide)
+    hipLaunchKernelGGL(ss_list_build_masks_kernel<unsigned>, grid, dim3(256), 0, stream, qmask, nrg, a.NP, a.chunk_rows, lay.nq, lens,
+                       static_cast<unsigned*>(ent));
+  else
+    hipLaunchKernelGGL(ss_list_build_masks_kernel<unsigned short>, grid, dim3(256), 0, stream, qmask, nrg, a.NP, a.chunk_rows, lay.nq, lens,
+                       static_cast<unsigned short*>(ent));
+  return hipGetLastError();
+}
+hipError_t launch_suffstat_lists_masks(const SuffstatLaunch& a, const SuffstatPlan& p, const unsigned short* qmask, int64_t nrg,
+                                       void* lists, size_t bytes, hipStream_t stream) {
+  SsListLayout lay;
+  if (hipError_t e = launch_suffstat_list_build_masks(a, p, qmask, nrg, lists, bytes, stream); e != hipSuccess) return e;
+  if (hipError_t e = ss_list_check(a, p, lists, bytes, &lay); e != hipSuccess) return e;
   const bool narrow = a.DC == 56;
   if (lay.wide) return narrow ? launch_ss_list_i<64, 56, unsigned>(a, lay, lists, stream) : launch_ss_list_i<64, 64, unsigned>(a, lay, lists, stream);
   return narrow ? launch_ss_list_i<64, 56, unsigned short>(a, lay, lists, stream)
diff --git a/libcluster_amd/csrc/lc_predict.cpp b/libcluster_amd/csrc/lc_predict.cpp
--- a/libcluster_amd/csrc/lc_predict.cpp
+++ b/libcluster_amd/csrc/lc_predict.cpp
@@ -59,6 +59,7 @@
   LC_HIP(hipStreamSynchronize(stream_));
   qz_[cur_].K = K;
   qz_[cur_].hash_ok = false;
+  qz_written(qz_[cur_]);
   pred_vb_ = true;
   pred_logp_ = pred_logp_ || Kp > 0;
 }
@@ -156,6 +157,7 @@
   LC_HIP(hipStreamSynchronize(stream_));
   qz_[cur_].K = Kp;
   qz_[cur_].hash_ok = false;
+  qz_written(qz_[cur_]);
   pred_cond_ = Db;
 }
 
@@ -494,6 +496,7 @@
   LC_HIP(hipStreamSynchronize(stream_));
   qz_[cur_].K = Kp;
   qz_[cur_].hash_ok = false;
+  qz_written(qz_[cur_]);
   dcache_invalidate();
   pred_holes_ = true;
   pred_holes_var_ = gnu != nullptr;
diff --git a/libcluster_amd/csrc/lc_testhooks.hip b/libcluster_amd/csrc/lc_testhooks.hip
--- a/libcluster_amd/csrc/lc_testhooks.hip
+++ b/libcluster_amd/csrc/lc_testhooks.hip
@@ -817,6 +817,109 @@
   return 0;
 }
 
+LC_HOOK lcx_test_estep_masks(const double* X, int DP, int DC, i64 nrg, const double* params, const double* ctab, int J, const int* rginfo,
+                             i64 nrows, int K, double* qZ, int Kbuf, i64 ldq, double* fz_part, i64 nfz, double* ll_part, i64 nll,
+                             unsigned short* qmask, i64 nmask, int* emits) {
+  if (!X || !params || !ctab || !qZ || !fz_part || !emits || K < 1 || K > 4096 || Kbuf < K || Kbuf > 8192 || J < 1 || J > (1 << 20)) return -1;
+  if (nrg < 1 || nrg > HOT_MAX_NRG || ldq < nrg * RG || !gw_width_ok(DP, DC)) return -1;
+  if (rginfo ? !rginfo_ok(rginfo, nrg, J) : (J != 1 || nrows < 0 || nrows > nrg * RG)) return -1;
+  if (qmask && nmask < (i64)((K + 3) / 4) * nrg) return -1;
+  lck::EstepLaunch a{};
+  a.DP = DP;
+  a.DC = DC;
+  a.K = K;
+  a.nrg = nrg;
+  a.nrows = nrows;
+  a.ldq = ldq;
+  const lck::EstepPlan p = lck::estep_plan(a);
+  if (!p.ok || p.grid < 1 || p.lds_bytes > HOT_LDS_LIMIT) return -1;
+  if (nfz < p.grid || (ll_part && nll < p.grid * K)) return -1;
+  *emits = p.emits ? 1 : 0;
+  Scope s;
+  a.X = s.in(X, (size_t)(nrg * RG) * DP);
+  a.params = s.in(params, (size_t)K * (size_t)lck::estep_pstride(DP, p.DC));
+  a.ctab = s.in(ctab, (size_t)J * K);
+  a.rginfo = rginfo ? s.in(rginfo, (size_t)nrg) : nullptr;
+  a.qZ = s.io(qZ, (size_t)Kbuf * (size_t)ldq);
+  a.fz_part = s.io(fz_part, (size_t)nfz);
+  a.ll_part = ll_part ? s.io(ll_part, (size_t)nll) : nullptr;
+  a.qmask = qmask ? s.io(qmask, (size_t)nmask) : nullptr;
+  if (!s.ok()) return s.finish(hipSuccess);
+  return s.finish(lck::launch_estep(a, nullptr));
+}
+
+LC_HOOK lcx_test_list_build(int which, const double* qZ, int DC, i64 NP, int K, i64 ldq, const unsigned short* qmask, i64 chunk_rows,
+                            i64* out, int* lens_out, i64 nlens, int* ent_out, i64 nent) {
+  const int DP = 64;
+  if (!qZ || !qmask || !out || !lens_out || !ent_out || K < 1 || K > 4096 || !gw_width_ok(DP, DC)) return -1;
+  if (NP < RG || NP % RG || NP > HOT_MAX_NRG * RG || ldq < NP || chunk_rows < 0 || chunk_rows % 4) return -1;
+  lck::SuffstatPlan p = lck::suffstat_plan(DP, DC, NP, K, lck::SS_DENSE);
+  if (chunk_rows > 0) {
+    p.chunk_rows = chunk_rows;
+    p.nchunks = (int)((NP + chunk_rows - 1) / chunk_rows);
+  }
+  if (p.nchunks < 1 || p.chunk_rows < 4 || (i64)p.nchunks * p.chunk_rows < NP) return -1;
+  out[0] = p.nchunks, out[1] = p.chunk_rows;
+  const lck::SsListLayout lay = lck::ss_list_layout(p.nchunks, p.chunk_rows, K);
+  const i64 nseg = (i64)p.nchunks * lay.nq, nrg = NP / RG;
+  if (nlens < nseg || nent < nseg * p.chunk_rows) return -1;
+  Scope s;
+  lck::SuffstatLaunch a{};
+  a.DP = DP;
+  a.DC = DC;
+  a.X = s.scratch<double>(16);
+  a.NP = NP;
+  a.qZ = s.in(qZ, (size_t)K * (size_t)ldq);
+  a.ldq = ldq;
+  a.K = K;
+  a.mode = lck::SS_DENSE;
+  a.nchunks = p.nchunks;
+  a.KR = p.KR;
+  a.chunk_rows = p.chunk_rows;
+  const unsigned short* dmask = s.in(qmask, (size_t)lay.nq * (size_t)nrg);
+  unsigned char* lists = s.scratch<unsigned char>(lay.bytes);
+  if (!s.ok()) return s.finish(hipSuccess);
+  hipError_t e = hipMemset(lists, 0xff, lay.bytes);
+  if (e == hipSuccess)
+    e = which ? lck::launch_suffstat_list_build_masks(a, p, dmask, nrg, lists, lay.bytes, nullptr)
+              : lck::launch_suffstat_list_build(a, p, lists, lay.bytes, nullptr);
+  const int rc = s.finish(e);
+  if (rc != 0) return rc;
+  std::vector<unsigned char> raw(lay.bytes);
+  if (hipMemcpy(raw.data(), lists, lay.bytes, hipMemcpyDeviceToHost) != hipSuccess) return -1;
+  const int* lens = reinterpret_cast<const int*>(raw.data());
+  for (i64 g = 0; g < nseg; ++g)
+    if (lens[g] < 0 || lens[g] > p.chunk_rows) return -2;
+  for (i64 g = 0; g < nseg; ++g) {
+    lens_out[g] = lens[g];
+    for (int i = 0; i < lens[g]; ++i) {
+      const size_t at = (size_t)g * (size_t)p.chunk_rows + (size_t)i;
+      ent_out[at] = lay.wide ? (int)reinterpret_cast<const unsigned*>(raw.data() + lay.ent_off)[at]
+                             : (int)reinterpret_cast<const unsigned short*>(raw.data() + lay.ent_off)[at];
+    }
+  }
+  return 0;
+}
+
+LC_HOOK lcx_test_speck_probe(int which, const double* qZ, i64 ldq, int K, i64 NP, const unsigned short* qmask, i64* out) {
+  if (!qZ || !qmask || !out || K < 1 || K > 4096 || NP < RG || NP % RG || NP > HOT_MAX_NRG * RG || ldq < NP || ldq % 2) return -1;
+  const i64 nrg = NP / RG;
+  Scope s;
+  const double* dq = s.in(qZ, (size_t)K * (size_t)ldq);
+  const unsigned short* dm = s.in(qmask, (size_t)((K + 3) / 4) * (size_t)nrg);
+  int* act = s.scratch<int>(2);
+  if (!s.ok()) return s.finish(hipSuccess);
+  int64_t pairs = 0, rows = 0;
+  const hipError_t e = which ? lck::launch_speck_probe_masks(dm, nrg, K, NP, act, &pairs, nullptr, &rows)
+                             : lck::launch_speck_probe(dq, ldq, K, NP, act, &pairs, nullptr, &rows);
+  const int rc = s.finish(e);
+  if (rc != 0) return rc;
+  int h[2] = {0, 0};
+  if (hipMemcpy(h, act, sizeof(h), hipMemcpyDeviceToHost) != hipSuccess) return -1;
+  out[0] = h[0], out[1] = h[1], out[2] = pairs, out[3] = rows;
+  return 0;
+}
+
 LC_HOOK lcx_test_suffstat_list_deal(int DP, int DC, i64* info, int* feat, i64 nfeat) {
   if (!info || !feat || !gw_width_ok(DP, DC) || !lck::suffstat_list_instance(DP, DC)) return -1;
   const int dc = DC ? DC : DP, waves = 8, tiles = lck::ftl_tpw(dc);
diff --git a/libcluster_amd/csrc/lc_topic_predict.cpp b/libcluster_amd/csrc/lc_topic_predict.cpp
--- a/libcluster_amd/csrc/lc_topic_predict.cpp
+++ b/libcluster_amd/csrc/lc_topic_predict.cpp
@@ -53,6 +53,7 @@
   LC_HIP(hipStreamSynchronize(stream_));
   qz_[cur_].K = K;
   qz_[cur_].hash_ok = false;
+  qz_written(qz_[cur_]);
   pred_vb_ = true;
   pred_docs_T_ = T;
 }
```

Result: faster. 390.1 million (median of 6 runs) (+2.2%).
